# szpiech/garlic

Hardware: NVIDIA B200
Metric: individual_windows_per_sec (higher is better)
Workload: dtype f64

## Files before the change

garlic_b200/csrc/bound.cuh:

```cuda
#pragma once
#include "common.cuh"
#include "walk.cuh"

namespace garlic {

constexpr int kBoundShift = 8;
constexpr int kBoundStoreShift = 2;
constexpr int kPiece = 256;
constexpr int kBoundMinW = 16;
constexpr int kBoundPartialW = 32;
constexpr int kBoundMaxC2 = 13;
constexpr int kBoundGeomMaxW = 209;
constexpr int kPlanSegMax = 16;

GHD int bound_geom_w(int W) { return W > kBoundGeomMaxW ? kBoundGeomMaxW : W; }
GHD int bound_c2(int W) { return (bound_geom_w(W) + 14) >> 4; }
GHD int bound_c1(int W) { const int c = (bound_geom_w(W) - 16) >> 4; return c > 0 ? c : 0; }
GHD int bound_lag(int W) { return bound_c2(W) - bound_c1(W); }
GHD bool bound_partial(int W) { return W < kBoundPartialW; }
GHD uint32_t bound_low_mask(int W) { const int r = (bound_geom_w(W) - 16) & 15; return r ? ((1u << (2 * r)) - 1u) & 0x55555555u : 0u; }

GHD uint4 bound_hw_entry(const double* lut, long long q, long long L, int* invalid)
{
    const double scale = (double)(1 << kBoundShift);
    double D[16], dmax = 0.0, chet = -1e300;
    uint32_t mo = 0u;
    for (int i = 0; i < 16; ++i) {
        const long long s = q * 16 + i;
        const double* e = lut + s * 4;
        const double base = e[0] < e[2] ? e[0] : e[2];
        D[i] = fabs(e[0] - e[2]);
        if (!(D[i] >= 0.0) || D[i] > 1e6) { D[i] = 0.0; if (s < L) *invalid = 1; }
        if (e[2] > e[0]) mo |= 1u << (2 * i);
        if (D[i] > dmax) dmax = D[i];
        if (s < L) {
            const double dh = e[1] - base;
            if (dh > chet) chet = dh;
            if (e[3] - base > 0.0) *invalid = 1;
            if (!(dh <= 0.0)) *invalid = 1;
        }
    }
    uint32_t step = dmax > 0.0 ? (uint32_t)ceil(dmax / 3.0 * scale) + 1u : 0u;
    if (step > 0xffffu) { step = 0xffffu; *invalid = 1; }
    uint32_t p0 = 0u, p1 = 0u;
    for (int i = 0; i < 16; ++i) {
        int lev = 0;
        if (D[i] > 0.0) {
            lev = (int)ceil(D[i] * scale / (double)step);
            if (lev < 1) lev = 1;
            if (lev > 3) lev = 3;
        }
        if (lev & 1) p0 |= 1u << (2 * i);
        if (lev & 2) p1 |= 1u << (2 * i);
    }
    uint32_t ch = 0u;
    if (chet > -1e299 && chet < 0.0) { const double m = floor(-chet * scale); ch = m > 65535.0 ? 0xffffu : (uint32_t)m; }
    uint4 o;
    o.x = mo | (p0 << 1); o.y = p1; o.z = step | (ch << 16); o.w = 0u;
    return o;
}

GHD int bound_block_max(const double* lut, long long k, int W)
{
    const int Wg = bound_geom_w(W);
    const long long s0 = k * 16;
    double b = 0.0;
    for (int i = 0; i < Wg; ++i) { const double* e = lut + (s0 + i) * 4; b += e[0] < e[2] ? e[0] : e[2]; }
    for (int i = Wg; i < W; ++i) { const double* e = lut + (s0 + i) * 4; b += e[0] < e[2] ? e[2] : e[0]; }
    double bmax = b;
    for (int j = 1; j < 16; ++j) {
        const double* eo = lut + (s0 + j - 1) * 4;
        const double* ei = lut + (s0 + j - 1 + W) * 4;
        b -= (eo[0] < eo[2] ? eo[0] : eo[2]);
        if (W > Wg) {
            const double* em = lut + (s0 + j - 1 + Wg) * 4;
            b -= (em[0] < em[2] ? em[2] : em[0]);
            b += (em[0] < em[2] ? em[0] : em[2]);
            b += (ei[0] < ei[2] ? ei[2] : ei[0]);
        } else {
            b += (ei[0] < ei[2] ? ei[0] : ei[2]);
        }
        if (b > bmax) bmax = b;
    }
    const double v = ceil(bmax * (double)(1 << kBoundShift)) + 2.0;
    return v > 1.0e9 ? 1000000000 : (v < -1.0e9 ? -1000000000 : (int)v);
}

struct BoundState {
    uint32_t PH[16], PR[16];
    uint32_t ph, pr;
    uint32_t top1, top2, low1;
    int pm_all, pm_tail;
};

GHD void bound_reset(BoundState& S)
{
#ifdef __CUDA_ARCH__
#pragma unroll
#endif
    for (int i = 0; i < 16; ++i) { S.PH[i] = 0u; S.PR[i] = 0u; }
    S.ph = 0u; S.pr = 0u;
    S.top1 = 0u; S.top2 = 0u; S.low1 = 0u;
    S.pm_all = -0x40000000; S.pm_tail = -0x40000000;
}

template <int C2, int LAG, bool PARTIAL = false>
GHD void bound_step(BoundState& S, uint32_t h, const uint4& t, const int I, const uint32_t low_mask = 0u)
{
    const uint32_t M = 0x55555555u;
    const uint32_t s = h >> 1;
    const uint32_t het = h & ~s & M;
    const uint32_t x = ~h & ~(s ^ t.x);
    const int n0 = popc32(x & (t.x >> 1) & M), n1 = popc32(x & t.y), nh = popc32(het);
    S.pr += (uint32_t)(n0 + 2 * n1) * (t.z & 0xffffu);
    S.PR[I] = S.pr;
    int ub;
    if (!PARTIAL) {
        S.ph += (uint32_t)nh * (t.z >> 16);
        S.PH[I] = S.ph;
        ub = (int)t.w + (int)(S.pr - S.PR[(I - C2 - 1) & 15]) + (int)(S.PH[(I - C2) & 15] - S.PH[(I - LAG) & 15]);
    } else {
        const uint32_t ch = t.z >> 16;
        const uint32_t top = ((het >> 30) & 1u) * ch, low = (uint32_t)popc32(het & low_mask) * ch;
        S.PH[I] = S.ph + (uint32_t)nh * ch - top;
        S.ph += (uint32_t)nh * ch;
        const uint32_t top_lag = LAG == 1 ? S.top1 : S.top2;
        const uint32_t low_next = LAG == 1 ? low : S.low1;
        const uint32_t core = (S.PH[(I - LAG) & 15] + top_lag) - S.PH[(I - C2) & 15] + low_next;
        ub = (int)t.w + (int)(S.pr - S.PR[(I - C2 - 1) & 15]) - (int)core;
        S.top2 = S.top1; S.top1 = top; S.low1 = low;
    }
    S.pm_all = ub > S.pm_all ? ub : S.pm_all;
    if (((I - C2) & 15) >= 16 - C2) S.pm_tail = ub > S.pm_tail ? ub : S.pm_tail;
}

GHD uint32_t bound_pack(int pm_all, int pm_tail)
{
    int a = (pm_all + (1 << kBoundStoreShift) - 1) >> kBoundStoreShift, b = (pm_tail + (1 << kBoundStoreShift) - 1) >> kBoundStoreShift;
    a = a > 32767 ? 32767 : (a < -32768 ? -32768 : a);
    b = b > 32767 ? 32767 : (b < -32768 ? -32768 : b);
    return ((uint32_t)a & 0xffffu) | ((uint32_t)b << 16);
}

GHD int bound_cut_store(double cutoff, double tol, int* ok)
{
    const double c = floor((cutoff - tol) * (double)(1 << kBoundShift)) - 2.0;
    *ok = (c > -8.0e6 && c < 8.0e6);
    if (!*ok) return 0;
    const int s = (int)c >> kBoundStoreShift;
    if (s > 32000 || s < -32000) *ok = 0;
    return s;
}

GHD bool bound_item_candidate(const uint32_t* pmax, int64_t stride, int ind, const Item& it, int cut_store, int c2)
{
    const int p_own = it.own_lo >> 8, p_hi = (it.own_hi - 1) >> 8, p_w0 = it.w0 >> 8;
    bool c = false;
    for (int p = (p_w0 < p_own ? p_w0 + 1 : p_own); p <= p_hi; ++p) c |= (int)(int16_t)(pmax[(int64_t)p * stride + ind] & 0xffffu) >= cut_store;
    if (p_w0 < p_own) {
        const uint32_t v = pmax[(int64_t)p_w0 * stride + ind];
        const bool tail_covers = it.w0 >= 256 * (p_w0 + 1) - 16 * c2;
        c |= (int)(int16_t)(tail_covers ? (v >> 16) : (v & 0xffffu)) >= cut_store;
    }
    return c;
}

GHD void plan_half(const int* src, long long L, long long q, uint4* head, uint4* segs)
{
    const long long d0 = q * 16;
    int n = 0;
    if (d0 < L) { const long long r = L - d0; n = r < 16 ? (int)r : 16; }
    uint4 hd;
    hd.w = n < 16 ? (0xffffffffu << (2 * n)) : 0u;
    hd.z = 0u;
    if (n == 16) {
        const int d = src[d0 + 15] - src[d0] - 15;
        if (d >= 0 && d <= 3) {
            uint32_t z = (uint32_t)(2 * (src[d0] & 15));
            int k = 0;
            for (int i = 0; i < 15; ++i)
                for (int g = src[d0 + i + 1] - src[d0 + i] - 1; g > 0; --g) z |= (uint32_t)(i + 1) << (8 * ++k);
            hd.x = 0x100u | ((uint32_t)d << 4); hd.y = (uint32_t)(src[d0] >> 4); hd.z = z;
            hd.w = d ? ((1u << (2u * ((z >> 8) & 255u))) - 1u) : 0xffffffffu;
            *head = hd;
            return;
        }
    }
    int ns = 0, i = 0, last = -1;
    while (i < n) {
        const int s0 = src[d0 + i];
        int len = 1;
        while (i + len < n && src[d0 + i + len] == s0 + len && ((s0 + len) >> 4) == (s0 >> 4)) ++len;
        uint4 sg;
        sg.x = (uint32_t)(s0 >> 4); sg.y = (uint32_t)(2 * (s0 & 15));
        sg.z = len >= 16 ? 0xffffffffu : ((1u << (2 * len)) - 1u);
        sg.w = (uint32_t)(2 * i);
        segs[ns++] = sg;
        last = s0 >> 4;
        i += len;
    }
    hd.x = (uint32_t)ns; hd.y = (uint32_t)last;
    *head = hd;
}

GHD uint32_t plan_fast_code(const uint4& hd, int a_base, int I)
{
    if (!(hd.x & 0x100u) || ((hd.x >> 4) & 15u) > 1u) return 0xffffu;
    const int rel = 32 * ((int)hd.y - a_base - I) + (int)(hd.z & 255u);
    if (rel < 0 || rel >= 96) return 0xffffu;
    const uint32_t p = ((hd.x >> 4) & 15u) ? ((hd.z >> 8) & 255u) : 16u;
    return (uint32_t)(rel >> 5) | ((uint32_t)(rel & 31) << 2) | ((2u * p) << 8);
}
GHD uint32_t plan_fast_apply(uint32_t code, uint32_t r0, uint32_t r1, uint32_t r2, uint32_t r3, uint32_t r4)
{
    const uint32_t k = code & 3u, sh = (code >> 2) & 31u, p2 = (code >> 8) & 255u;
    const uint32_t x0 = k == 0u ? r0 : (k == 1u ? r1 : r2), x1 = k == 0u ? r1 : (k == 1u ? r2 : r3), x2 = k == 0u ? r2 : (k == 1u ? r3 : r4);
    const uint32_t lo = sh ? ((x0 >> sh) | (x1 << (32u - sh))) : x0, hi = sh ? ((x1 >> sh) | (x2 << (32u - sh))) : x1;
    const uint32_t m = p2 >= 32u ? 0xffffffffu : ((1u << p2) - 1u);
    return (lo & m) | (((lo >> 2) | (hi << 30)) & ~m);
}
GHD bool plan_need1(const uint4& hd) { return ((hd.z & 255u) != 0u) || ((hd.x >> 4) & 15u); }
GHD bool plan_need2(const uint4& hd) { return ((hd.z & 255u) >> 1) + 15u + ((hd.x >> 4) & 15u) >= 32u; }
GHD uint32_t plan_window(const uint4& hd, uint32_t x0, uint32_t x1, uint32_t x2)
{
    const uint32_t sh = hd.z & 255u;
    uint32_t lo = sh ? ((x0 >> sh) | (x1 << (32u - sh))) : x0;
    uint32_t d = (hd.x >> 4) & 15u;
    if (d) {
        uint32_t hi = sh ? ((x1 >> sh) | (x2 << (32u - sh))) : x1;
        uint32_t z = hd.z >> 8;
        for (; d; --d, z >>= 8) {
            const uint32_t m = (1u << (2u * (z & 255u))) - 1u;
            const uint32_t slo = (lo >> 2) | (hi << 30);
            hi >>= 2;
            lo = (lo & m) | (slo & ~m);
        }
    }
    return lo;
}

}
```

garlic_b200/csrc/capi.cu:

```cuda
#include <cuda_runtime.h>
#include <nccl.h>
#include <algorithm>
#include <chrono>
#include <cmath>
#include <cstdio>
#include <cstring>
#include <map>
#include <unistd.h>
#include <string>
#include <vector>

#include "../../include/garlic_b200.h"
#include "common.cuh"
#include "kernels.h"
#include "wlod.h"
#include "segments.h"
#include "bound.cuh"

using namespace garlic;

namespace {
constexpr int kPad = 4096 + 64;
constexpr int kMaxW = 4096;
constexpr unsigned kBreakCap = 1u << 20, kBreakFirst = 4096;

}

struct garlic_gpu {
    int device = 0;
    cudaStream_t stream = nullptr;
    std::string err;
    uint64_t launches = 0;
    int n_ind = 0, ind_offset = 0, n_chr = 0;
    int64_t L0 = 0, L = 0;
    std::vector<int64_t> chr_off0, chr_off;
    std::vector<int32_t> pos0, pos, src, cen;
    std::vector<double> gpos;
    std::vector<Stretch> stretches;
    bool stretches_pending = false;
    uint8_t* brk_pin = nullptr;
    cudaEvent_t ev_tables = nullptr;
    bool have_geno0 = false, filtered = false, tables = false, have_gl = false, have_ld = false;
    int gl_type = GARLIC_GL_ERROR;
    double error = -1, mu = 1e-9;
    int max_gap = 200000, M = 7, ld_W = 0;
    double amax = 0;
    double fmin = 0.5;
    int* d_corr = nullptr;
    int missing_char = '0';
    uint8_t* d_alleles = nullptr;
    unsigned long long* d_key = nullptr;
    uint64_t *d_geno0 = nullptr, *d_geno = nullptr;
    int64_t row_words0 = 0, row_words = 0;
    int* d_counts = nullptr;
    double *d_gl0 = nullptr, *d_gl = nullptr;
    int64_t gl_stride = 0;
    double *d_freq0 = nullptr, *d_freq = nullptr, *d_lut = nullptr, *d_gpos = nullptr;
    double *d_nomut = nullptr, *d_norec = nullptr, *d_wlut = nullptr, *d_invld = nullptr, *d_homf = nullptr;
    char* d_text = nullptr;
    long long* d_textoff = nullptr;
    int* d_nonblank = nullptr;
    int2* d_hard = nullptr;
    StitchScratch stitch_scratch;
    std::vector<RohRec> recs_buf, ambs_buf, merged_buf, tmp_buf;
    uint64_t* d_ldplanes = nullptr;
    double* d_ldpairs = nullptr;
    uint8_t* d_keep = nullptr;
    int *d_src = nullptr, *d_pos0 = nullptr, *d_chr_of0 = nullptr, *d_pos = nullptr, *d_chr_of = nullptr,
        *d_chr_start = nullptr, *d_chr_param = nullptr;
    RohRec *d_out = nullptr, *d_amb = nullptr, *d_sorted = nullptr;
    unsigned* d_hist = nullptr;
    unsigned* d_kept = nullptr;
    size_t last_final = 0;
    std::vector<Segment> p2_segs;
    std::vector<Item> p2_items;
    Item* d_items_p2 = nullptr;
    int p2_W = 0, p2_tile = 0, p2_chunk = 0;
    uint64_t tables_gen = 0, p2_gen = 0;
    size_t sorted_cap = 0;
    unsigned out_cap = 0, amb_cap = 0;
    unsigned* d_cnt = nullptr;
    Item* d_items = nullptr;
    double* d_dump = nullptr;
    size_t items_cap = 0;
    int* d_indlist = nullptr;
    size_t indlist_cap = 0;
    double stats[8] = {0, 0, 0, 0, 0, 0, 0, 0};
    int64_t stats_items = 0;
    int* d_scan = nullptr;
    int* d_breaks = nullptr;
    uint32_t* d_badbits = nullptr;
    int* d_thin = nullptr;
    bool geno_pending = false;
    uint4 *d_plan_head = nullptr, *d_plan_seg = nullptr;
    int2* d_plan_rng = nullptr;
    uint4* d_bhw = nullptr;
    uint16_t* d_plan_fast = nullptr;
    int* d_bflag = nullptr;
    int bound_tables_W = 0;
    uint32_t* d_pmax = nullptr;
    int64_t pmax_stride = 0;
    int n_pieces = 0, bound_W = 0;
    int* d_cand_list = nullptr;
    unsigned* d_cand_cnt = nullptr;
    int2* d_units = nullptr;
    unsigned* d_nunits = nullptr;
    size_t zero_cap = 0, zero_n = 0;
    cudaEvent_t ev_sq0 = nullptr, ev_sq1 = nullptr;
    bool sq_timed = false;
    int item_pieces = 1;
    bool prune = true;
    bool precounted = false;
    bool phased = false;
    bool wlod_mma = true;
    ncclComm_t comm = nullptr;
    int comm_rank = 0, comm_world = 1;
    bool counts_reduced = false, counts_hi_reduced = false;
    bool counts_nccl_mem = false;
    uint8_t* xslab = nullptr;
    void* xpeer[kXchgMaxRanks] = {nullptr};
    size_t x_off_counts = 0, x_off_freq = 0, x_off_keep = 0;
    bool xchg_tried = false, xchg_ok = false;
    unsigned xchg_seq = 0;
    ncclWindow_t counts_win = nullptr;
    bool counts_win_tried = false;
    double* d_gather = nullptr;
    const double* kde_src = nullptr;
    int64_t kde_src_n = 0;
    double *d_kde = nullptr, *d_kde_in = nullptr;
    cudaEvent_t ev2 = nullptr;
    cudaStream_t copy_stream = nullptr;
    cudaStream_t aux_stream = nullptr;
    cudaEvent_t ev_aux_in = nullptr, ev_aux_out = nullptr;
    cudaEvent_t ev_copy = nullptr;
    bool tl_on = false;
    std::vector<cudaEvent_t> tl_ev;
    std::vector<const char*> tl_name;
    std::vector<double> tl_host;
    bool out_pending = false;
    uint8_t* pin = nullptr;
    size_t pin_cap = 0;
    std::map<void*, size_t> cap;
    cudaEvent_t ev0 = nullptr, ev1 = nullptr;
};

struct Laps {
    bool on;
    int rank = 0;
    const char* name;
    std::chrono::steady_clock::time_point t0;
    std::string out;
    explicit Laps(const char* n) : on(getenv("GARLIC_TIMING") != nullptr), name(n), t0(std::chrono::steady_clock::now()) {}
    void lap(const char* what)
    {
        if (!on) return;
        const auto t1 = std::chrono::steady_clock::now();
        char b[96];
        snprintf(b, sizeof b, " %s=%.3f", what, std::chrono::duration<double, std::milli>(t1 - t0).count());
        out += b;
        t0 = t1;
    }
    ~Laps() { if (on) fprintf(stderr, "[garlic_b200 r%d] %s:%s ms\n", rank, name, out.c_str()); }
};

static void tl_mark(garlic_gpu* h, const char* name)
{
    if (!h->tl_on) return;
    if (h->tl_ev.size() >= 4096) return;
    cudaEvent_t e;
    cudaEventCreate(&e);
    cudaEventRecord(e, h->stream);
    h->tl_ev.push_back(e);
    h->tl_name.push_back(name);
    h->tl_host.push_back(std::chrono::duration<double, std::milli>(std::chrono::steady_clock::now().time_since_epoch()).count());
}
static void tl_dump(garlic_gpu* h)
{
    if (!h->tl_on || h->tl_ev.empty()) return;
    cudaStreamSynchronize(h->stream);
    const size_t n = h->tl_ev.size(), first = n > 120 ? n - 120 : 0;
    for (size_t i = first; i < n; ++i) {
        float g = 0;
        cudaEventElapsedTime(&g, h->tl_ev[first], h->tl_ev[i]);
        fprintf(stderr, "[timeline r%d] %-28s host %9.3f  stream %9.3f ms\n", h->comm_rank, h->tl_name[i], h->tl_host[i] - h->tl_host[first], g);
    }
    for (cudaEvent_t e : h->tl_ev) cudaEventDestroy(e);
    h->tl_ev.clear();
}

#define CK(call)                                                                              \
    do {                                                                                      \
        cudaError_t e_ = (call);                                                              \
        if (e_ != cudaSuccess) {                                                              \
            h->err = std::string(#call) + ": " + cudaGetErrorString(e_);                      \
            return 1;                                                                         \
        }                                                                                     \
    } while (0)
#define LAUNCH(call) do { CK(call); h->launches++; } while (0)
#define FAIL(msg) do { h->err = (msg); return 1; } while (0)

template <typename T>
static int dev_alloc(garlic_gpu* h, T** p, size_t n)
{
    if (n == 0) n = 1;
    const size_t bytes = n * sizeof(T);
    auto it = h->cap.find((void*)p);
    if (*p && it != h->cap.end() && it->second >= bytes) return 0;
    if (*p) { cudaFree(*p); *p = nullptr; }
    CK(cudaMalloc((void**)p, bytes));
    h->cap[(void*)p] = bytes;
    return 0;
}
template <typename T>
static void dev_free(T*& p) { if (p) cudaFree(p); p = nullptr; }

static int pin_alloc(garlic_gpu* h, size_t bytes)
{
    if (h->pin && h->pin_cap >= bytes) return 0;
    if (h->pin) { cudaFreeHost(h->pin); h->pin = nullptr; h->pin_cap = 0; }
    CK(cudaMallocHost((void**)&h->pin, bytes));
    h->pin_cap = bytes;
    return 0;
}

static double lod_bound(const garlic_gpu* h)
{
    const double n_total = 2.0 * ((double)h->n_ind + 1.0) * (double)std::max(1, h->comm_world);
    double fmin = 1.0 / n_total;
    if (h->fmin > 0 && h->fmin < fmin) fmin = h->fmin;
    const double emin = h->have_gl ? 1e-16 : ((h->error > 0 && h->error < 1) ? h->error : 1e-16);
    return std::max(-std::log10(emin), -std::log10(fmin)) + 1.0;
}

#define NCK(call)                                                                             \
    do {                                                                                      \
        ncclResult_t r_ = (call);                                                             \
        if (r_ != ncclSuccess) {                                                              \
            h->err = std::string(#call) + ": " + ncclGetErrorString(r_);                      \
            return 1;                                                                         \
        }                                                                                     \
    } while (0)

static int reduce_counts(garlic_gpu* h, bool hi)
{
    if (!h->comm) return 0;
    if (!h->counts_win_tried && h->counts_nccl_mem) {
        h->counts_win_tried = true;
        if (getenv("GARLIC_NCCL_WINDOW") != nullptr) {
            if (ncclCommWindowRegister(h->comm, h->d_counts, (size_t)4 * h->L0 * sizeof(int), &h->counts_win, NCCL_WIN_COLL_SYMMETRIC) != ncclSuccess)
                h->counts_win = nullptr;
        }
    }
    if (!h->counts_reduced) {
        NCK(ncclAllReduce(h->d_counts, h->d_counts, (size_t)2 * h->L0, ncclInt32, ncclSum, h->comm, h->stream));
        h->counts_reduced = true;
    }
    if (hi && !h->counts_hi_reduced) {
        NCK(ncclAllReduce(h->d_counts + 2 * h->L0, h->d_counts + 2 * h->L0, (size_t)2 * h->L0, ncclInt32, ncclSum, h->comm, h->stream));
        h->counts_hi_reduced = true;
    }
    return 0;
}

static void free_counts(garlic_gpu* h)
{
    if (!h->d_counts) return;
    if (h->xchg_ok) return;
    if (h->counts_win && h->comm) ncclCommWindowDeregister(h->comm, h->counts_win);
    h->counts_win = nullptr; h->counts_win_tried = false;
    if (h->counts_nccl_mem) ncclMemFree(h->d_counts); else cudaFree(h->d_counts);
    h->d_counts = nullptr; h->counts_nccl_mem = false;
    h->cap.erase((void*)&h->d_counts);
}

static int alloc_counts(garlic_gpu* h, size_t n)
{
    const size_t bytes = n * sizeof(int);
    auto it = h->cap.find((void*)&h->d_counts);
    if (h->d_counts && it != h->cap.end() && it->second == bytes) return 0;
    free_counts(h);
    void* p = nullptr;
    if (getenv("GARLIC_NCCL_WINDOW") != nullptr && ncclMemAlloc(&p, bytes) == ncclSuccess && p) {
        h->d_counts = static_cast<int*>(p);
        h->counts_nccl_mem = true;
    } else {
        cudaGetLastError();
        CK(cudaMalloc((void**)&h->d_counts, bytes));
    }
    h->cap[(void*)&h->d_counts] = bytes;
    return 0;
}

static void xchg_teardown(garlic_gpu* h)
{
    if (!h->xslab) { h->xchg_tried = false; h->xchg_ok = false; return; }
    cudaStreamSynchronize(h->stream);
    for (int p = 0; p < kXchgMaxRanks; ++p) {
        if (h->xpeer[p] && h->xpeer[p] != (void*)h->xslab) cudaIpcCloseMemHandle(h->xpeer[p]);
        h->xpeer[p] = nullptr;
    }
    if (h->xchg_ok) {
        h->d_counts = nullptr; h->d_freq0 = nullptr; h->d_keep = nullptr;
        h->cap.erase((void*)&h->d_counts); h->cap.erase((void*)&h->d_freq0); h->cap.erase((void*)&h->d_keep);
    }
    cudaFree(h->xslab);
    h->xslab = nullptr;
    h->xchg_tried = false; h->xchg_ok = false; h->xchg_seq = 0;
}

static int ensure_xchg(garlic_gpu* h)
{
    if (h->xchg_tried) return 0;
    h->xchg_tried = true;
    h->xchg_ok = false;
    if (!h->comm || h->comm_world < 2 || h->comm_world > kXchgMaxRanks || h->counts_nccl_mem) return 0;
    if (getenv("GARLIC_NO_XCHG") != nullptr) return 0;
    const int N = h->comm_world;
    const size_t L0 = (size_t)h->L0;
    h->x_off_counts = 256;
    h->x_off_freq = (h->x_off_counts + 16 * L0 + 255) & ~(size_t)255;
    h->x_off_keep = h->x_off_freq + 8 * L0;
    const size_t total = ((h->x_off_keep + L0 + 255) & ~(size_t)255);
    struct Rec { cudaIpcMemHandle_t hdl; int pid; int ok; long long L0; char pad[128 - sizeof(cudaIpcMemHandle_t) - 16]; };
    static_assert(sizeof(Rec) == 128, "exchange record is 128 bytes");
    Rec mine;
    memset(&mine, 0, sizeof(mine));
    mine.pid = (int)getpid(); mine.L0 = h->L0; mine.ok = 1;
    if (cudaMalloc((void**)&h->xslab, total) != cudaSuccess) { cudaGetLastError(); h->xslab = nullptr; mine.ok = 0; }
    if (mine.ok) {
        cudaMemsetAsync(h->xslab, 0, 256, h->stream);
        cudaStreamSynchronize(h->stream);
        if (cudaIpcGetMemHandle(&mine.hdl, h->xslab) != cudaSuccess) { cudaGetLastError(); mine.ok = 0; }
    }
    Rec* d_rec = nullptr;
    std::vector<Rec> all(N);
    CK(cudaMalloc((void**)&d_rec, (size_t)(N + 1) * sizeof(Rec)));
    CK(cudaMemcpyAsync(d_rec + N, &mine, sizeof(Rec), cudaMemcpyHostToDevice, h->stream));
    NCK(ncclAllGather(d_rec + N, d_rec, sizeof(Rec), ncclUint8, h->comm, h->stream));
    CK(cudaMemcpyAsync(all.data(), d_rec, (size_t)N * sizeof(Rec), cudaMemcpyDeviceToHost, h->stream));
    CK(cudaStreamSynchronize(h->stream));
    int ok = 1;
    for (int p = 0; p < N; ++p) {
        if (!all[p].ok || all[p].L0 != h->L0) ok = 0;
        if (p != h->comm_rank && all[p].pid == mine.pid) ok = 0;
    }
    for (int p = 0; p < N && ok; ++p) {
        if (p == h->comm_rank) { h->xpeer[p] = h->xslab; continue; }
        void* ptr = nullptr;
        if (cudaIpcOpenMemHandle(&ptr, all[p].hdl, cudaIpcMemLazyEnablePeerAccess) != cudaSuccess) { cudaGetLastError(); ok = 0; break; }
        h->xpeer[p] = ptr;
    }
    int* d_ok = reinterpret_cast<int*>(d_rec);
    CK(cudaMemcpyAsync(d_ok, &ok, sizeof(int), cudaMemcpyHostToDevice, h->stream));
    NCK(ncclAllReduce(d_ok, d_ok, 1, ncclInt32, ncclMin, h->comm, h->stream));
    CK(cudaMemcpyAsync(&ok, d_ok, sizeof(int), cudaMemcpyDeviceToHost, h->stream));
    CK(cudaStreamSynchronize(h->stream));
    cudaFree(d_rec);
    if (!ok) {
        for (int p = 0; p < N; ++p) {
            if (h->xpeer[p] && h->xpeer[p] != (void*)h->xslab) cudaIpcCloseMemHandle(h->xpeer[p]);
            h->xpeer[p] = nullptr;
        }
        if (h->xslab) cudaFree(h->xslab);
        h->xslab = nullptr;
        return 0;
    }
    int* nc = reinterpret_cast<int*>(h->xslab + h->x_off_counts);
    if (h->d_counts) CK(cudaMemcpyAsync(nc, h->d_counts, 16 * L0, cudaMemcpyDeviceToDevice, h->stream));
    else CK(cudaMemsetAsync(nc, 0, 16 * L0, h->stream));
    CK(cudaStreamSynchronize(h->stream));
    free_counts(h);
    if (h->d_freq0) { cudaFree(h->d_freq0); h->d_freq0 = nullptr; }
    if (h->d_keep) { cudaFree(h->d_keep); h->d_keep = nullptr; }
    h->d_counts = nc;
    h->d_freq0 = reinterpret_cast<double*>(h->xslab + h->x_off_freq);
    h->d_keep = h->xslab + h->x_off_keep;
    h->cap[(void*)&h->d_counts] = 16 * L0;
    h->cap[(void*)&h->d_freq0] = 8 * L0;
    h->cap[(void*)&h->d_keep] = L0;
    h->xchg_ok = true;
// ... 236 lines not shown
    if (h->comm) NCK(ncclAllReduce(h->d_key, h->d_key, (size_t)h->L0, ncclUint64, ncclMin, h->comm, h->stream));
    CK(cudaMemsetAsync(h->d_counts, 0, (size_t)4 * h->L0 * sizeof(int), h->stream));
    const int64_t chunk = 1 << 20;
    for (int64_t s0 = 0; s0 < h->L0; s0 += chunk) {
        const int n = (int)std::min<int64_t>(chunk, h->L0 - s0);
        LAUNCH(launch_code_alleles(h->d_alleles + (size_t)s0 * h->n_ind * 2, n, h->n_ind, missing, h->d_key + s0, s0,
                                   h->d_geno0, h->row_words0, h->d_counts, h->L0, h->stream));
    }
    CK(cudaStreamSynchronize(h->stream));
    h->have_geno0 = true;
    return 0;
}

static int put_packed_common(garlic_gpu* h, const void* rows, int64_t stride, cudaMemcpyKind kind)
{
    CK(cudaSetDevice(h->device));
    if (!h->L0) FAIL("put_packed: call set_shape first");
    const int64_t need = (h->L0 + 3) / 4;
    if (stride < need) FAIL("put_packed: row stride smaller than ceil(n_loci/4)");
    h->precounted = false;
    if (kind == cudaMemcpyHostToDevice && h->n_ind >= 256 && h->d_counts) {
        const int n_slices = 8;
        const int per = ((h->n_ind + n_slices - 1) / n_slices + 15) / 16 * 16;
        CK(cudaMemsetAsync(h->d_counts, 0, (size_t)4 * h->L0 * sizeof(int), h->stream));
        CK(cudaEventRecord(h->ev_copy, h->stream));
        CK(cudaStreamWaitEvent(h->copy_stream, h->ev_copy, 0));
        for (int r0 = 0; r0 < h->n_ind; r0 += per) {
            const int n = std::min(per, h->n_ind - r0);
            uint64_t* dst = h->d_geno0 + (size_t)r0 * h->row_words0;
            CK(cudaMemcpy2DAsync(dst, (size_t)h->row_words0 * 8, (const char*)rows + (size_t)r0 * stride, (size_t)stride, (size_t)need,
                                 (size_t)n, kind, h->copy_stream));
            CK(cudaEventRecord(h->ev_copy, h->copy_stream));
            CK(cudaStreamWaitEvent(h->stream, h->ev_copy, 0));
            LAUNCH(launch_count_packed(dst, h->row_words0, n, h->L0, h->d_counts, h->stream));
        }
        CK(cudaStreamSynchronize(h->copy_stream));
        h->precounted = true;
        h->counts_reduced = false; h->counts_hi_reduced = false;
        h->have_geno0 = true;
        return 0;
    }
    CK(cudaMemcpy2DAsync(h->d_geno0, (size_t)h->row_words0 * 8, rows, (size_t)stride, (size_t)need, (size_t)h->n_ind, kind, h->stream));
    CK(cudaStreamSynchronize(h->stream));
    h->have_geno0 = true;
    return 0;
}

int garlic_gpu_put_packed(garlic_gpu_t* h, const uint8_t* rows, int64_t row_stride_bytes)
{
    return put_packed_common(h, rows, row_stride_bytes, cudaMemcpyHostToDevice);
}
int garlic_gpu_put_packed_dev(garlic_gpu_t* h, const void* rows_dev, int64_t row_stride_bytes)
{
    return put_packed_common(h, rows_dev, row_stride_bytes, cudaMemcpyDeviceToDevice);
}

__global__ void add_corr_kernel(int* counts, long long L0, const int* na, const int* tot)
{
    for (long long s = blockIdx.x * (long long)blockDim.x + threadIdx.x; s < L0; s += (long long)gridDim.x * blockDim.x) {
        if (na) counts[s] += na[s];
        if (tot) counts[L0 + s] += tot[s];
    }
}

int garlic_gpu_count_packed(garlic_gpu_t* h, const int32_t* nalleles_corr, const int32_t* total_corr)
{
    CK(cudaSetDevice(h->device));
    if (!h->have_geno0) FAIL("count_packed: no genotypes loaded");
    tl_mark(h, "count_packed:in");
    h->counts_reduced = false; h->counts_hi_reduced = false;
    if (h->precounted) {
        h->precounted = false;
    } else {
        CK(cudaMemsetAsync(h->d_counts, 0, (size_t)4 * h->L0 * sizeof(int), h->stream));
        LAUNCH(launch_count_packed(h->d_geno0, h->row_words0, h->n_ind, h->L0, h->d_counts, h->stream));
    }
    if (nalleles_corr || total_corr) {
        if (dev_alloc(h, &h->d_corr, (size_t)2 * h->L0)) return 1;
        int *d_a = nalleles_corr ? h->d_corr : nullptr, *d_t = total_corr ? h->d_corr + h->L0 : nullptr;
        if (d_a) CK(cudaMemcpyAsync(d_a, nalleles_corr, h->L0 * sizeof(int), cudaMemcpyHostToDevice, h->stream));
        if (d_t) CK(cudaMemcpyAsync(d_t, total_corr, h->L0 * sizeof(int), cudaMemcpyHostToDevice, h->stream));
        add_corr_kernel<<<(unsigned)std::min<int64_t>((h->L0 + 255) / 256, 148 * 16), 256, 0, h->stream>>>(h->d_counts, h->L0, d_a, d_t);
        CK(cudaGetLastError());
        h->launches++;
        CK(cudaStreamSynchronize(h->stream));
    }
    if (h->xchg_ok) return 0;
    return reduce_counts(h, false);
}

void* garlic_gpu_counts_dev(garlic_gpu_t* h) { return h ? (void*)h->d_counts : nullptr; }

int garlic_gpu_get_counts(garlic_gpu_t* h, int32_t* na, int32_t* tot, int32_t* hom, int32_t* nm)
{
    CK(cudaSetDevice(h->device));
    CK(cudaStreamSynchronize(h->stream));
    int32_t* dst[4] = {na, tot, hom, nm};
    for (int c = 0; c < 4; ++c)
        if (dst[c]) CK(cudaMemcpy(dst[c], h->d_counts + (size_t)c * h->L0, h->L0 * sizeof(int), cudaMemcpyDeviceToHost));
    return 0;
}

int garlic_gpu_get_one_allele(garlic_gpu_t* h, uint8_t* allele, char missing)
{
    CK(cudaSetDevice(h->device));
    if (!h->d_key) FAIL("get_one_allele: alleles were not ingested on this handle");
    std::vector<unsigned long long> k(h->L0);
    CK(cudaStreamSynchronize(h->stream));
    CK(cudaMemcpy(k.data(), h->d_key, h->L0 * sizeof(unsigned long long), cudaMemcpyDeviceToHost));
    for (int64_t s = 0; s < h->L0; ++s) allele[s] = (k[s] == ~0ull) ? (uint8_t)missing : (uint8_t)(k[s] & 0xff);
    return 0;
}

static int put_gl_common(garlic_gpu* h, const void* v, int gl_type, cudaMemcpyKind kind)
{
    CK(cudaSetDevice(h->device));
    if (!h->L0) FAIL("put_gl: call set_shape first");
    if (gl_type < -1 || gl_type > 2) FAIL("put_gl: bad gl_type");
    if (dev_alloc(h, &h->d_gl0, (size_t)h->n_ind * h->L0)) return 1;
    CK(cudaMemcpyAsync(h->d_gl0, v, (size_t)h->n_ind * h->L0 * sizeof(double), kind, h->stream));
    CK(cudaStreamSynchronize(h->stream));
    h->gl_type = gl_type;
    h->have_gl = true;
    return 0;
}
int garlic_gpu_put_tgls_text(garlic_gpu_t* h, const char* text, const int64_t* line_off, int64_t snp0, int n_snp,
                             int gl_type, int32_t* n_tokens)
{
    CK(cudaSetDevice(h->device));
    if (!h->L0) FAIL("put_tgls_text: call set_shape first");
    if (gl_type < -1 || gl_type > 2) FAIL("put_tgls_text: bad gl_type");
    if (snp0 < 0 || n_snp < 0 || snp0 + n_snp > h->L0) FAIL("put_tgls_text: bad SNP range");
    if (n_snp == 0) return 0;
    const int64_t bytes = line_off[n_snp] - line_off[0];
    if (bytes < 0) FAIL("put_tgls_text: line offsets must ascend");
    if (dev_alloc(h, &h->d_gl0, (size_t)h->n_ind * h->L0)) return 1;
    if (dev_alloc(h, &h->d_text, (size_t)bytes + 16)) return 1;
    if (dev_alloc(h, &h->d_textoff, (size_t)n_snp + 1)) return 1;
    if (dev_alloc(h, &h->d_nonblank, (size_t)n_snp)) return 1;
    const unsigned hard_cap = 1u << 16;
    if (dev_alloc(h, &h->d_hard, (size_t)hard_cap + 1)) return 1;
    unsigned* d_hard_n = reinterpret_cast<unsigned*>(h->d_hard + hard_cap);
    std::vector<long long> rel(n_snp + 1);
    for (int i = 0; i <= n_snp; ++i) rel[i] = (long long)(line_off[i] - line_off[0]);
    const char* base = text + line_off[0];
    CK(cudaMemcpyAsync(h->d_text, base, (size_t)bytes, cudaMemcpyHostToDevice, h->stream));
    CK(cudaMemcpyAsync(h->d_textoff, rel.data(), rel.size() * sizeof(long long), cudaMemcpyHostToDevice, h->stream));
    CK(cudaMemsetAsync(d_hard_n, 0, sizeof(unsigned), h->stream));
    LAUNCH(launch_tokenize_tgls(h->d_text, h->d_textoff, n_snp, h->n_ind, h->ind_offset, h->d_gl0, h->L0, snp0, h->d_nonblank,
                                h->d_hard, d_hard_n, hard_cap, h->stream));
    std::vector<int32_t> ntok_local;
    if (!n_tokens) { ntok_local.resize(n_snp); n_tokens = ntok_local.data(); }
    unsigned n_hard = 0;
    CK(cudaMemcpyAsync(n_tokens, h->d_nonblank, (size_t)n_snp * sizeof(int), cudaMemcpyDeviceToHost, h->stream));
    CK(cudaMemcpyAsync(&n_hard, d_hard_n, sizeof(unsigned), cudaMemcpyDeviceToHost, h->stream));
    CK(cudaStreamSynchronize(h->stream));
    if (n_hard) {
        auto token_at = [&](int l, int k) -> const char* {
            const char* p = base + rel[l];
            const char* e = base + rel[l + 1];
            for (int t = 0;; ++t) {
                while (p < e && (*p == ' ' || *p == '\t' || *p == '\r' || *p == '\n')) ++p;
                if (p >= e) return nullptr;
                if (t == k) return p;
                while (p < e && !(*p == ' ' || *p == '\t' || *p == '\r' || *p == '\n')) ++p;
            }
        };
        auto convert = [&](const char* p, int l) -> double {
            const char* e = base + rel[l + 1];
            const char* q = p;
            while (q < e && !(*q == ' ' || *q == '\t' || *q == '\r' || *q == '\n')) ++q;
            const std::string tok(p, q);
            return strtod(tok.c_str(), nullptr);
        };
        std::vector<int2> list;
        if (n_hard <= hard_cap) {
            list.resize(n_hard);
            CK(cudaMemcpy(list.data(), h->d_hard, n_hard * sizeof(int2), cudaMemcpyDeviceToHost));
        } else {
            for (int l = 0; l < n_snp; ++l)
                for (int k = h->ind_offset; k < h->ind_offset + h->n_ind; ++k) list.push_back(make_int2(l, k));
        }
        std::sort(list.begin(), list.end(), [](const int2& a, const int2& b) { return a.x != b.x ? a.x < b.x : a.y < b.y; });
        for (const int2& t : list) {
            const char* p = token_at(t.x, t.y);
            if (!p) continue;
            const double v = convert(p, t.x);
            CK(cudaMemcpyAsync(h->d_gl0 + (size_t)(t.y - h->ind_offset) * h->L0 + snp0 + t.x, &v, sizeof(double), cudaMemcpyHostToDevice, h->stream));
            CK(cudaStreamSynchronize(h->stream));
        }
    }
    h->gl_type = gl_type;
    h->have_gl = true;
    return 0;
}

int garlic_gpu_get_gl(garlic_gpu_t* h, double* values)
{
    CK(cudaSetDevice(h->device));
    if (!h->have_gl || !h->d_gl0) FAIL("get_gl: no likelihoods loaded");
    CK(cudaStreamSynchronize(h->stream));
    CK(cudaMemcpy(values, h->d_gl0, (size_t)h->n_ind * h->L0 * sizeof(double), cudaMemcpyDeviceToHost));
    return 0;
}

int garlic_gpu_put_gl(garlic_gpu_t* h, const double* values, int gl_type) { return put_gl_common(h, values, gl_type, cudaMemcpyHostToDevice); }
int garlic_gpu_put_gl_dev(garlic_gpu_t* h, const void* values_dev, int gl_type) { return put_gl_common(h, values_dev, gl_type, cudaMemcpyDeviceToDevice); }

int garlic_gpu_filter(garlic_gpu_t* h, int oob, const int32_t* chr_param, const double* freq_override,
                      double* freq_out, uint8_t* keep_out, int64_t* n_kept)
{
    CK(cudaSetDevice(h->device));
    if (!h->have_geno0) FAIL("filter: no genotypes loaded");
    if (oob && !chr_param) FAIL("filter: oob filtering needs chr_param");
    const int64_t L0 = h->L0;
    Laps laps("filter");
    laps.rank = h->comm_rank;
    if (finish_outputs(h)) return 1;
    tl_mark(h, "filter:in");
    if (!freq_override) h->fmin = 0.5;
    bool freq_direct = false, keep_direct = false, copies_in_flight = false;
    if (dev_alloc(h, &h->d_freq0, (size_t)L0)) return 1;
    if (dev_alloc(h, &h->d_keep, (size_t)L0)) return 1;
    if (oob) {
        if (dev_alloc(h, &h->d_chr_param, (size_t)4 * h->n_chr)) return 1;
        CK(cudaMemcpyAsync(h->d_chr_param, chr_param, 4 * h->n_chr * sizeof(int), cudaMemcpyHostToDevice, h->stream));
    }
    const int n_blocks = (int)((L0 + 1023) / 1024);
    const size_t off_keep = (size_t)L0 * 8, off_meta = (off_keep + (size_t)L0 + 63) & ~(size_t)63;
    if (pin_alloc(h, off_meta + (size_t)(h->n_chr + 2) * 4 + 64)) return 1;
    double* freq0 = reinterpret_cast<double*>(h->pin);
    uint8_t* keep = h->pin + off_keep;
    int32_t* meta = reinterpret_cast<int32_t*>(h->pin + off_meta);
    if (freq_override) {
        h->fmin = 0.5;
        for (int64_t s = 0; s < L0; ++s) {
            const double f = freq_override[s];
            bool k = (f > 0 && f < 1);
            if (k) h->fmin = std::min(h->fmin, std::min(f, 1.0 - f));
            if (oob) {
                int c = (int)(std::upper_bound(h->chr_off0.begin(), h->chr_off0.end(), s) - h->chr_off0.begin()) - 1;
                const int32_t* cp = chr_param + 4 * c;
                const int p = h->pos0[s];
                k = k && !(p < cp[0]) && !(p > cp[1]) && !(p > cp[2] && p < cp[3]);
            }
            freq0[s] = f; keep[s] = k;
        }
        CK(cudaMemcpyAsync(h->d_freq0, freq0, L0 * sizeof(double), cudaMemcpyHostToDevice, h->stream));
        CK(cudaMemcpyAsync(h->d_keep, keep, L0, cudaMemcpyHostToDevice, h->stream));
    } else {
        if (h->comm && !h->xchg_tried && ensure_xchg(h)) return 1;
        if (h->xchg_ok && !h->counts_reduced) {
            XchgParams X;
            memset(&X, 0, sizeof(X));
            for (int p = 0; p < h->comm_world; ++p) {
                uint8_t* base = static_cast<uint8_t*>(h->xpeer[p]);
                X.flags[p] = reinterpret_cast<unsigned*>(base);
                X.counts[p] = reinterpret_cast<int*>(base + h->x_off_counts);
                X.freq[p] = reinterpret_cast<double*>(base + h->x_off_freq);
                X.keep[p] = base + h->x_off_keep;
            }
            X.n = h->comm_world; X.rank = h->comm_rank; X.seq = ++h->xchg_seq; X.L0 = L0;
            X.pos = h->d_pos0; X.chr_of = h->d_chr_of0; X.chr_param = h->d_chr_param; X.oob = oob;
            X.done_counter = reinterpret_cast<unsigned*>(h->xslab) + 48;
            LAUNCH(launch_xchg_freq_keep(X, h->stream));
            h->counts_reduced = true;
        } else {
            if (reduce_counts(h, false)) return 1;
            LAUNCH(launch_freq_keep(h->d_counts, L0, h->d_pos0, h->d_chr_of0, h->d_chr_param, oob, h->d_freq0, h->d_keep, h->stream));
        }
        freq_direct = freq_out && is_pinned(freq_out);
        keep_direct = keep_out && is_pinned(keep_out);
        copies_in_flight = freq_out || keep_out;
    }
    if (dev_alloc(h, &h->d_src, (size_t)L0)) return 1;
    if (dev_alloc(h, &h->d_scan, (size_t)n_blocks + h->n_chr + 8)) return 1;
    int* d_total = h->d_scan + n_blocks;
    int* d_chr_off_kept = d_total + 1;
    CK(launch_keep_scan(h->d_keep, L0, h->d_chr_of0, h->n_chr, h->d_scan, d_total, h->d_src, d_chr_off_kept, h->stream));
    h->launches += 3;
    CK(cudaMemcpyAsync(meta, d_total, (size_t)(h->n_chr + 2) * sizeof(int), cudaMemcpyDeviceToHost, h->stream));
    if (copies_in_flight) {
        CK(cudaEventRecord(h->ev_copy, h->stream));
        CK(cudaStreamWaitEvent(h->copy_stream, h->ev_copy, 0));
        if (freq_out) CK(cudaMemcpyAsync(freq_direct ? freq_out : freq0, h->d_freq0, L0 * sizeof(double), cudaMemcpyDeviceToHost, h->copy_stream));
        if (keep_out) CK(cudaMemcpyAsync(keep_direct ? keep_out : keep, h->d_keep, L0, cudaMemcpyDeviceToHost, h->copy_stream));
    }
    CK(cudaStreamSynchronize(h->stream));
    laps.lap("freq_keep+scan");
    tl_mark(h, "filter:after-sync");
    if (freq_override) {
        if (freq_out) memcpy(freq_out, freq0, L0 * sizeof(double));
        if (keep_out) memcpy(keep_out, keep, L0);
    }
    const int64_t L = meta[0];
    h->chr_off.assign(h->n_chr + 1, 0);
    for (int c = 0; c <= h->n_chr; ++c) h->chr_off[c] = meta[1 + c];
    h->src.clear();
    h->pos.clear();
    h->L = L;
    if (n_kept) *n_kept = L;
    if (L < 1) FAIL("filter: no polymorphic loci left");
    h->row_words = (((L + kPad + 31) >> 5) + 3) & ~(int64_t)1;
    const bool fresh = h->cap.find((void*)&h->d_geno) == h->cap.end() || !h->d_geno ||
                       h->cap[(void*)&h->d_geno] < (size_t)h->n_ind * h->row_words * 8;
    if (dev_alloc(h, &h->d_geno, (size_t)h->n_ind * h->row_words)) return 1;
    if (fresh) CK(cudaMemsetAsync(h->d_geno, 0xff, (size_t)h->n_ind * h->row_words * 8, h->stream));
    h->n_pieces = (int)((L + kPiece - 1) / kPiece);
    {
        const long long n_q = 16ll * (h->n_pieces + 4);
        if (dev_alloc(h, &h->d_plan_head, (size_t)n_q)) return 1;
        if (dev_alloc(h, &h->d_plan_seg, (size_t)n_q * kPlanSegMax)) return 1;
        if (dev_alloc(h, &h->d_plan_rng, (size_t)h->n_pieces + 4)) return 1;
        if (dev_alloc(h, &h->d_plan_fast, (size_t)n_q)) return 1;
        LAUNCH(launch_plan(h->d_src, d_total, n_q, h->d_plan_head, h->d_plan_seg, h->d_plan_fast, h->d_plan_rng, h->stream));
    }
    h->geno_pending = true; h->bound_W = 0; h->bound_tables_W = 0;
    if (dev_alloc(h, &h->d_freq, (size_t)L + kPad)) return 1;
    CK(cudaMemsetAsync(h->d_freq, 0, (size_t)(L + kPad) * sizeof(double), h->stream));
    LAUNCH(launch_gather_f64(h->d_freq0, h->d_src, L, h->d_freq, h->stream));
    if (h->have_gl) {
        h->gl_stride = L + kPad;
        if (dev_alloc(h, &h->d_gl, (size_t)((h->n_ind + 31) / 32) * 32 * h->gl_stride)) return 1;
        LAUNCH(launch_compact_gl(h->d_gl0, L0, h->d_src, L, h->d_geno0, h->row_words0, h->d_freq0, h->d_gl, h->gl_stride, h->n_ind,
                                 h->gl_type, h->stream));
    }
    std::vector<int> chr_start(h->n_chr);
    for (int c = 0; c < h->n_chr; ++c) chr_start[c] = (int)h->chr_off[c];
    if (dev_alloc(h, &h->d_pos, (size_t)L)) return 1;
    if (dev_alloc(h, &h->d_chr_of, (size_t)L)) return 1;
    if (dev_alloc(h, &h->d_chr_start, (size_t)h->n_chr)) return 1;
    LAUNCH(launch_gather_i32(h->d_pos0, h->d_src, L, h->d_pos, h->stream));
    LAUNCH(launch_gather_i32(h->d_chr_of0, h->d_src, L, h->d_chr_of, h->stream));
    CK(cudaMemcpyAsync(h->d_chr_start, chr_start.data(), h->n_chr * sizeof(int), cudaMemcpyHostToDevice, h->stream));
    laps.lap("enqueue");
    if (copies_in_flight) {
        const bool all_direct = (!freq_out || freq_direct) && (!keep_out || keep_direct);
        if (all_direct) {
            h->out_pending = true;
        } else {
            CK(cudaStreamSynchronize(h->copy_stream));
            if (freq_out && !freq_direct) memcpy(freq_out, freq0, L0 * sizeof(double));
            if (keep_out && !keep_direct) memcpy(keep_out, keep, L0);
        }
        laps.lap("freq/keep d2h");
    }
    h->filtered = true; h->tables = false; h->have_ld = false;
    tl_mark(h, "filter:out");
    return 0;
}

int64_t garlic_gpu_n_kept(const garlic_gpu_t* h) { return h ? h->L : 0; }

int garlic_gpu_get_genotypes(garlic_gpu_t* h, int filtered, uint8_t* rows, int64_t row_stride_bytes)
{
    CK(cudaSetDevice(h->device));
    if (filtered ? !h->filtered : !h->have_geno0) FAIL("get_genotypes: nothing loaded");
    const int64_t n = filtered ? h->L : h->L0;
    const int64_t need = (n + 3) / 4;
    if (row_stride_bytes < need) FAIL("get_genotypes: row stride too small");
    if (filtered && ensure_geno(h, 0)) return 1;
    CK(cudaStreamSynchronize(h->stream));
    CK(cudaMemcpy2D(rows, (size_t)row_stride_bytes, filtered ? h->d_geno : h->d_geno0,
                    (size_t)(filtered ? h->row_words : h->row_words0) * 8, (size_t)need, (size_t)h->n_ind, cudaMemcpyDeviceToHost));
    return 0;
}

int garlic_gpu_get_kept_index(garlic_gpu_t* h, int32_t* src_index)
{
    if (!h->filtered) FAIL("get_kept_index: call filter first");
    if (fetch_src(h)) return 1;
    memcpy(src_index, h->src.data(), h->L * sizeof(int32_t));
    return 0;
}

int garlic_gpu_set_tables(garlic_gpu_t* h, double error, int max_gap, const int32_t* centromeres, const double* gpos)
{
    CK(cudaSetDevice(h->device));
    if (!h->filtered) FAIL("set_tables: call filter first");
    h->error = error; h->max_gap = max_gap;
    Laps laps("set_tables");
    laps.rank = h->comm_rank;
    tl_mark(h, "set_tables:in");
    h->cen.assign(2 * h->n_chr, 0);
    if (centromeres) h->cen.assign(centromeres, centromeres + 2 * h->n_chr);
    const int64_t L = h->L;
    if (dev_alloc(h, &h->d_lut, (size_t)(L + kPad) * 4)) return 1;
    CK(cudaMemsetAsync(h->d_lut, 0, (size_t)(L + kPad) * 4 * sizeof(double), h->stream));
    LAUNCH(launch_build_lut(h->d_freq, L, error, h->d_lut, h->stream));
    h->gpos.clear();
    if (gpos) {
        h->gpos.assign(gpos, gpos + L);
        if (dev_alloc(h, &h->d_gpos, (size_t)L)) return 1;
        CK(cudaMemcpyAsync(h->d_gpos, gpos, L * sizeof(double), cudaMemcpyHostToDevice, h->stream));
    }
    h->amax = lod_bound(h);
    {
        if (dev_alloc(h, &h->d_breaks, (size_t)kBreakCap + 2 * h->n_chr + 4)) return 1;
        int* d_cen = h->d_breaks + kBreakCap;
        unsigned* d_n = reinterpret_cast<unsigned*>(d_cen + 2 * h->n_chr);
        CK(cudaMemcpyAsync(d_cen, h->cen.data(), 2 * h->n_chr * sizeof(int), cudaMemcpyHostToDevice, h->stream));
        CK(cudaMemsetAsync(d_n, 0, sizeof(unsigned), h->stream));
        if (dev_alloc(h, &h->d_badbits, (size_t)((L + 31) >> 5) + 4)) return 1;
        LAUNCH(launch_bad_pairs(h->d_pos, h->d_chr_of, d_cen, max_gap, L, h->d_breaks, d_n, kBreakCap, h->d_badbits, h->stream));
        if (!h->brk_pin) CK(cudaMallocHost((void**)&h->brk_pin, 64 + kBreakFirst * sizeof(int)));
        CK(cudaMemcpyAsync(h->brk_pin, d_n, sizeof(unsigned), cudaMemcpyDeviceToHost, h->stream));
        CK(cudaMemcpyAsync(h->brk_pin + 64, h->d_breaks, kBreakFirst * sizeof(int), cudaMemcpyDeviceToHost, h->stream));
        CK(cudaEventRecord(h->ev_tables, h->stream));
        h->stretches_pending = true;
        h->stretches.clear();
    }
    laps.lap("enqueue");
    tl_mark(h, "set_tables:out");
    h->tables = true; h->have_ld = false; h->bound_W = 0; h->bound_tables_W = 0; h->tables_gen++;
    return 0;
}

int garlic_gpu_set_lut(garlic_gpu_t* h, const double* lut)
{
    CK(cudaSetDevice(h->device));
    if (!h->tables) FAIL("set_lut: call set_tables first");
    CK(cudaMemcpy(h->d_lut, lut, (size_t)h->L * 4 * sizeof(double), cudaMemcpyHostToDevice));
    double m = 0;
    for (int64_t i = 0; i < h->L * 4; ++i) { const double a = std::fabs(lut[i]); if (a > m && std::isfinite(a)) m = a; }
    h->amax = std::max(lod_bound(h), m + 1.0);
    dev_free(h->d_wlut);
    h->bound_W = 0; h->bound_tables_W = 0;
    return 0;
}

int garlic_gpu_get_lut(garlic_gpu_t* h, double* lut)
{
    CK(cudaSetDevice(h->device));
    if (!h->tables) FAIL("get_lut: call set_tables first");
    CK(cudaStreamSynchronize(h->stream));
    CK(cudaMemcpy(lut, h->d_lut, (size_t)h->L * 4 * sizeof(double), cudaMemcpyDeviceToHost));
    return 0;
}

int garlic_gpu_get_hom_freq(garlic_gpu_t* h, double* hom_freq)
{
    CK(cudaSetDevice(h->device));
    if (!h->filtered) FAIL("get_hom_freq: call filter first");
    std::vector<int> hom(h->L0), nm(h->L0);
    if (reduce_counts(h, true)) return 1;
    if (garlic_gpu_get_counts(h, nullptr, nullptr, hom.data(), nm.data())) return 1;
    if (fetch_src(h)) return 1;
    for (int64_t d = 0; d < h->L; ++d) {
        double total = nm[h->src[d]], fh = hom[h->src[d]];
        fh /= total;
        hom_freq[d] = fh;
    }
    return 0;
}

int garlic_gpu_set_prune(garlic_gpu_t* h, int on)
{
    h->prune = on != 0;
    return 0;
}

int garlic_gpu_set_phased(garlic_gpu_t* h, int phased)
{
    h->phased = phased != 0;
    h->have_ld = false;
    return 0;
}

int garlic_gpu_set_wlod(garlic_gpu_t* h, double mu, int M)
{
    h->mu = mu; h->M = M;
    dev_free(h->d_wlut);
    return 0;
}

}

static int ensure_stretches(garlic_gpu* h)
{
    if (!h->stretches_pending) return 0;
    CK(cudaEventSynchronize(h->ev_tables));
    const unsigned nb = *reinterpret_cast<const unsigned*>(h->brk_pin);
    const int* first_host = reinterpret_cast<const int*>(h->brk_pin + 64);
    if (nb > kBreakCap) FAIL("set_tables: more than 2^20 gaps; raise --max-gap");
    std::vector<int> breaks(first_host, first_host + std::min(nb, kBreakFirst));
    if (nb > kBreakFirst) {
        breaks.resize(nb);
        CK(cudaStreamSynchronize(h->stream));
        CK(cudaMemcpy(breaks.data() + kBreakFirst, h->d_breaks + kBreakFirst, (nb - kBreakFirst) * sizeof(int), cudaMemcpyDeviceToHost));
    }
    std::sort(breaks.begin(), breaks.end());
    h->stretches.clear();
    size_t bi = 0;
    for (int c = 0; c < h->n_chr; ++c) {
        int a = (int)h->chr_off[c];
        const int hi = (int)h->chr_off[c + 1];
        while (bi < breaks.size() && breaks[bi] < hi) {
            if (breaks[bi] > a) h->stretches.push_back({c, a, breaks[bi]});
            a = breaks[bi++];
        }
        if (hi > a) h->stretches.push_back({c, a, hi});
    }
    h->stretches_pending = false;
    return 0;
}

static int ensure_zero_block(garlic_gpu* h)
{
    const size_t n = 8 + 2 * ((size_t)h->n_ind + 1);
    if (h->zero_cap < n) {
        if (h->d_cnt) cudaFree(h->d_cnt);
        h->d_cnt = nullptr;
        CK(cudaMalloc((void**)&h->d_cnt, n * sizeof(unsigned)));
        CK(cudaMemsetAsync(h->d_cnt, 0, n * sizeof(unsigned), h->stream));
        h->zero_cap = n;
    }
    h->d_nunits = h->d_cnt + 4;
    h->d_hist = h->d_cnt + 8;
    h->d_kept = h->d_hist + h->n_ind + 1;
    h->zero_n = n;
    return 0;
}

static int upload_items(garlic_gpu* h, const std::vector<Item>& items)
{
    if (items.size() > h->items_cap) {
        if (dev_alloc(h, &h->d_items, items.size() + 1024)) return 1;
        h->items_cap = items.size() + 1024;
    }
    if (!items.empty()) CK(cudaMemcpyAsync(h->d_items, items.data(), items.size() * sizeof(Item), cudaMemcpyHostToDevice, h->stream));
    return 0;
}

static int upload_indlist(garlic_gpu* h, const int32_t* list, int n, cudaStream_t st = nullptr)
{
    if (!st) st = h->stream;
    if ((size_t)n > h->indlist_cap) {
        if (dev_alloc(h, &h->d_indlist, (size_t)n + 1024)) return 1;
        h->indlist_cap = (size_t)n + 1024;
    }
    CK(cudaMemcpyAsync(h->d_indlist, list, n * sizeof(int), cudaMemcpyHostToDevice, st));
    return 0;
}

static WalkParams base_params(const garlic_gpu* h, int W)
{
    WalkParams P;
    memset(&P, 0, sizeof(P));
    P.geno = h->d_geno; P.row_words = h->row_words;
    P.lut = h->d_lut; P.gl = h->have_gl ? h->d_gl : nullptr; P.freq = h->d_freq; P.gl_stride = h->gl_stride;
    P.ind_list = nullptr; P.n_lanes = h->n_ind; P.W = W; P.thr = 1; P.cutoff = 0; P.tol = 0;
    P.out = h->d_out; P.out_count = h->d_cnt; P.out_cap = h->out_cap; P.amb = h->d_amb; P.amb_cap = h->amb_cap;
    P.hist = nullptr;
    P.dump = nullptr; P.dump_stride = 0; P.dump_step = 1;
    return P;
}

static int ensure_weighted(garlic_gpu* h, int W);
static int launch_any_walk(garlic_gpu* h, const WalkParams& P, const Item* items, int n_items, int weighted, bool roh, bool dump,
                           int tile_snps, const CandList& cl = CandList())
{
    if (weighted) {
        WlodParams Q;
        Q.base = P; Q.wlut = h->d_wlut; Q.invld = h->d_invld; Q.nomut = h->d_nomut; Q.norec = h->d_norec;
        if (P.tol > 0 && roh && !dump && h->wlod_mma && P.W >= kWlodMmaMinW) LAUNCH(launch_wlod_mma(Q, items, n_items, h->have_gl, h->stream));
        else LAUNCH(launch_wlod_walk(Q, items, n_items, h->have_gl, roh, dump, h->stream));
    } else {
        LAUNCH(launch_walk(P, items, n_items, h->have_gl, roh, dump, tile_snps <= kTileSnpsMax ? tile_snps : 0, cl, h->stream));
    }
    return 0;
}

static bool can_bound(const garlic_gpu* h, int W)
{
    return h->prune && h->tables && !h->have_gl && W >= kBoundMinW && W <= 1280;
}

static int ensure_bound_tables(garlic_gpu* h, int W)
{
    if (h->bound_tables_W == W) return 0;
    const long long n_hw = 16ll * (h->n_pieces + 4);
    if (dev_alloc(h, &h->d_bhw, (size_t)n_hw)) return 1;
    if (dev_alloc(h, &h->d_bflag, (size_t)4)) return 1;
    CK(cudaMemsetAsync(h->d_bflag, 0, 4 * sizeof(int), h->stream));
    LAUNCH(launch_bound_tables(h->d_lut, h->L + kPad, n_hw, h->L, W, h->d_bhw, h->d_bflag, h->stream));
    h->bound_tables_W = W;
    return 0;
}

static SqueezeParams squeeze_params(garlic_gpu* h, bool squeeze, int W)
{
    SqueezeParams Q;
    memset(&Q, 0, sizeof(Q));
    Q.gin = squeeze ? h->d_geno0 : h->d_geno;
    Q.in_words = squeeze ? h->row_words0 : h->row_words;
    Q.gout = h->d_geno; Q.out_words = h->row_words;
    Q.plan_head = h->d_plan_head; Q.plan_seg = h->d_plan_seg; Q.piece_rng = h->d_plan_rng;
    Q.plan_fast = reinterpret_cast<const uint32_t*>(h->d_plan_fast); Q.src = h->d_src; Q.n_kept = h->d_scan + (int)((h->L0 + 1023) / 1024);
    Q.n_ind = h->n_ind;
    Q.hw = h->d_bhw;
    Q.lag = bound_lag(W);
    Q.partial = (W > 0 && bound_partial(W)) ? 1 : 0;
    Q.low_mask = W > 0 ? bound_low_mask(W) : 0u;
    Q.pmax = h->d_pmax; Q.pmax_stride = h->pmax_stride;
    Q.n_pieces = h->n_pieces;
    return Q;
}

static int alloc_pmax(garlic_gpu* h)
{
    h->pmax_stride = ((int64_t)h->n_ind + 31) & ~(int64_t)31;
    return dev_alloc(h, &h->d_pmax, (size_t)h->n_pieces * h->pmax_stride);
}

static int ensure_geno(garlic_gpu* h, int W_hint)
{
    if (!h->geno_pending) return 0;
    int c2 = 0;
    if (W_hint > 0 && can_bound(h, W_hint)) {
        if (ensure_bound_tables(h, W_hint)) return 1;
        if (alloc_pmax(h)) return 1;
        c2 = bound_c2(W_hint);
    }
    const SqueezeParams Q = squeeze_params(h, true, W_hint);
    CK(cudaEventRecord(h->ev_sq0, h->stream));
    LAUNCH(launch_squeeze_bound(Q, true, c2, h->stream));
    CK(cudaEventRecord(h->ev_sq1, h->stream));
    h->sq_timed = true;
    h->geno_pending = false;
    if (c2) h->bound_W = W_hint;
    return 0;
}

static int prepare_p2_items(garlic_gpu* h, int W)
{
    if (h->p2_gen == h->tables_gen && h->p2_W == W) return 0;
    if (ensure_stretches(h)) return 1;
    segments_from_stretches(h->stretches, W, h->p2_segs);
    build_items_aligned(h->chr_off, W, h->p2_segs, kPiece * h->item_pieces, h->p2_items);
    h->p2_chunk = 0;
    for (const Item& it : h->p2_items) h->p2_chunk = std::max(h->p2_chunk, it.own_hi - it.own_lo);
    h->p2_tile = items_tile_snps(h->p2_items, W);
    if (dev_alloc(h, &h->d_items_p2, h->p2_items.size() + 1)) return 1;
    if (!h->p2_items.empty())
        CK(cudaMemcpyAsync(h->d_items_p2, h->p2_items.data(), h->p2_items.size() * sizeof(Item), cudaMemcpyHostToDevice, h->stream));
    h->p2_gen = h->tables_gen; h->p2_W = W;
    return 0;
}

static int ensure_bound(garlic_gpu* h, int W)
{
    if (ensure_geno(h, W)) return 1;
    if (h->bound_W == W) return 0;
    if (ensure_bound_tables(h, W)) return 1;
    if (alloc_pmax(h)) return 1;
    const SqueezeParams Q = squeeze_params(h, false, W);
    CK(cudaEventRecord(h->ev_sq0, h->stream));
    LAUNCH(launch_squeeze_bound(Q, false, bound_c2(W), h->stream));
    CK(cudaEventRecord(h->ev_sq1, h->stream));
    h->sq_timed = true;
    h->bound_W = W;
    return 0;
}

static bool side_pass1(const garlic_gpu* h, int weighted, int exact, int step)
{
    static const bool off = getenv("GARLIC_NO_SIDE_PASS1") != nullptr;
    return !off && !weighted && !exact && step >= 8 && !h->have_gl && h->have_geno0 && h->aux_stream != nullptr;
}
static int begin_side(garlic_gpu* h)
{
    CK(cudaEventRecord(h->ev_aux_in, h->stream));
    CK(cudaStreamWaitEvent(h->aux_stream, h->ev_aux_in, 0));
    return 0;
}
static int end_side(garlic_gpu* h)
{
    CK(cudaEventRecord(h->ev_aux_out, h->aux_stream));
    CK(cudaStreamWaitEvent(h->stream, h->ev_aux_out, 0));
    return 0;
}

extern "C" {

int64_t garlic_gpu_window_slots(garlic_gpu_t* h, int step)
{
    if (!h || !h->filtered || step < 1) return -1;
    int64_t n = 0;
    for (int c = 0; c < h->n_chr; ++c) n += (h->chr_off[c + 1] - h->chr_off[c] + step - 1) / step;
    return n;
}

static int windows_common(garlic_gpu_t* h, int winsize, int step, int weighted, const int32_t* individuals, int n,
                          int exact, double* out, void** out_dev);

int garlic_gpu_windows(garlic_gpu_t* h, int winsize, int step, int weighted, const int32_t* individuals, int n,
                       int exact, double* out)
{
    return windows_common(h, winsize, step, weighted, individuals, n, exact, out, nullptr);
}

int garlic_gpu_windows_dev(garlic_gpu_t* h, int winsize, int step, int weighted, const int32_t* individuals, int n,
                           int exact, void** out_dev)
{
    if (!out_dev) return 1;
    return windows_common(h, winsize, step, weighted, individuals, n, exact, nullptr, out_dev);
}

int garlic_gpu_windows_gather(garlic_gpu_t* h, int winsize, int step, int weighted, const int32_t* individuals, int n,
                              int rows_per_rank, int exact, double* out)
{
    if (n > rows_per_rank) FAIL("windows_gather: more individuals than rows_per_rank");
    const int64_t slots = garlic_gpu_window_slots(h, step);
    if (slots < 0) FAIL("windows_gather: call filter first");
    void* dptr = nullptr;
    if (n > 0 && windows_common(h, winsize, step, weighted, individuals, n, exact, nullptr, &dptr)) return 1;
    CK(cudaSetDevice(h->device));
    const bool side = h->filtered && h->tables && side_pass1(h, weighted, exact, step);
    cudaStream_t ws = side ? h->aux_stream : h->stream;
    if (side && n == 0 && begin_side(h)) return 1;
    const size_t blk = (size_t)rows_per_rank * slots;
    if (dev_alloc(h, &h->d_gather, blk * (h->comm_world + 1))) return 1;
    double* send = h->d_gather + blk * h->comm_world;
    LAUNCH(launch_fill_f64(send, blk, kMissing, ws));
    if (n > 0) CK(cudaMemcpyAsync(send, dptr, (size_t)n * slots * sizeof(double), cudaMemcpyDeviceToDevice, ws));
    if (h->comm) NCK(ncclAllGather(send, h->d_gather, blk, ncclDouble, h->comm, ws));
    else CK(cudaMemcpyAsync(h->d_gather, send, blk * sizeof(double), cudaMemcpyDeviceToDevice, ws));
    h->kde_src = h->d_gather; h->kde_src_n = (int64_t)(blk * h->comm_world);
    if (!out) return side ? end_side(h) : 0;
    const size_t bytes = blk * h->comm_world * sizeof(double);
    const bool direct = is_pinned(out);
    const bool staged = !direct && bytes <= ((size_t)64 << 20) && !pin_alloc(h, bytes);
    CK(cudaMemcpyAsync(direct ? (void*)out : (staged ? (void*)h->pin : (void*)out), h->d_gather, bytes, cudaMemcpyDeviceToHost, ws));
    CK(cudaStreamSynchronize(ws));
    if (side && end_side(h)) return 1;
    if (finish_outputs(h)) return 1;
    if (staged) memcpy(out, h->pin, bytes);
    return 0;
}

static int windows_common(garlic_gpu_t* h, int winsize, int step, int weighted, const int32_t* individuals, int n,
                          int exact, double* out, void** out_dev)
{
    CK(cudaSetDevice(h->device));
    if (!h->tables) FAIL("windows: call set_tables first");
    if (winsize < 2 || winsize > kMaxW) FAIL("windows: winsize out of range [2,4096]");
    if (step < 1) FAIL("windows: step must be >= 1");
    tl_mark(h, "windows:in");
    if (weighted && ensure_weighted(h, winsize)) return 1;
    const int W = winsize;
    const int n_lanes = individuals ? n : h->n_ind;
    if (individuals)
        for (int i = 0; i < n; ++i) if (individuals[i] < 0 || individuals[i] >= h->n_ind) FAIL("windows: individual index out of range");
    const int64_t slots = garlic_gpu_window_slots(h, step);
    const bool direct = !weighted && !exact && step >= 8;
    const bool side = direct && side_pass1(h, weighted, exact, step);
    cudaStream_t ws = h->stream;
    int rc = 0;
    double* d_dump = nullptr;
    if (direct) {
        if (!side && ensure_geno(h, winsize)) return 1;
        if (individuals && upload_indlist(h, individuals, n)) return 1;
        if (dev_alloc(h, &h->d_dump, (size_t)n_lanes * slots)) return 1;
        d_dump = h->d_dump;
        LAUNCH(launch_fill_f64(d_dump, (size_t)n_lanes * slots, kMissing, h->stream));
        std::vector<int2> meta(h->n_chr);
        int base = 0;
        for (int c = 0; c < h->n_chr; ++c) {
            meta[c].x = (int)h->chr_off[c]; meta[c].y = base;
            base += (int)((h->chr_off[c + 1] - h->chr_off[c] + step - 1) / step);
        }
        if (dev_alloc(h, &h->d_thin, (size_t)2 * h->n_chr + 8)) return 1;
        int2* d_meta = reinterpret_cast<int2*>(h->d_thin);
        CK(cudaMemcpyAsync(d_meta, meta.data(), meta.size() * sizeof(int2), cudaMemcpyHostToDevice, h->stream));
        LAUNCH(launch_thin_windows(side ? h->d_geno0 : h->d_geno, side ? h->row_words0 : h->row_words, h->d_lut,
                                   individuals ? h->d_indlist : nullptr, n_lanes, h->d_badbits, h->L, d_meta, h->n_chr, slots, step, W,
                                   d_dump, slots, h->have_gl ? h->d_gl : nullptr, h->gl_stride, side ? h->d_src : nullptr, h->stream));
        if (side) {
            if (begin_side(h)) return 1;
            ws = h->aux_stream;
            if (ensure_geno(h, winsize)) return 1;
        }
        tl_mark(h, "windows:squeeze-enqueued");
        if (h->bound_W == W && prepare_p2_items(h, W)) return 1;
    } else {
        if (ensure_geno(h, weighted ? 0 : winsize)) return 1;
        if (individuals && upload_indlist(h, individuals, n)) return 1;
        std::vector<Segment> segs;
        std::vector<Item> items;
        if (ensure_stretches(h)) return 1;
        segments_from_stretches(h->stretches, W, segs);
        if (dev_alloc(h, &h->d_dump, (size_t)n_lanes * slots)) return 1;
        d_dump = h->d_dump;
        LAUNCH(launch_fill_f64(d_dump, (size_t)n_lanes * slots, kMissing, h->stream));
        int chunk = 0;
        if (weighted) chunk = std::max(64, pick_chunk(h->L, W, n_lanes, 0) / 8);
        else if (!exact) chunk = pick_chunk(h->L, W, n_lanes, h->have_gl ? 0 : kTileSnpsMax);
        build_items(h->chr_off, W, segs, chunk, step, items);
        if (upload_items(h, items)) return 1;
        WalkParams P = base_params(h, W);
        P.ind_list = individuals ? h->d_indlist : nullptr;
        P.n_lanes = n_lanes;
        P.cutoff = 0; P.thr = 1; P.tol = 0;
        P.dump = d_dump; P.dump_stride = slots; P.dump_step = step;
        CK(cudaMemsetAsync(h->d_cnt, 0, 4 * sizeof(unsigned), h->stream));
        rc = launch_any_walk(h, P, h->d_items, (int)items.size(), weighted, false, true, items_tile_snps(items, W));
    }
    if (!rc) { h->kde_src = d_dump; h->kde_src_n = (int64_t)n_lanes * slots; }
    tl_mark(h, "windows:enqueued");
    if (!rc && finish_outputs(h)) rc = 1;
    if (!rc && out_dev) {
        *out_dev = d_dump;
        cudaError_t e = cudaStreamSynchronize(ws);
        if (e != cudaSuccess) { h->err = std::string("windows: ") + cudaGetErrorString(e); rc = 1; }
    } else if (!rc) {
        const size_t bytes = (size_t)n_lanes * slots * sizeof(double);
        const bool staged = !is_pinned(out) && bytes <= ((size_t)64 << 20) && !pin_alloc(h, bytes);
        cudaError_t e = cudaMemcpyAsync(staged ? (void*)h->pin : (void*)out, d_dump, bytes, cudaMemcpyDeviceToHost, ws);
        if (e == cudaSuccess) e = cudaStreamSynchronize(ws);
        if (e != cudaSuccess) { h->err = std::string("windows: ") + cudaGetErrorString(e); rc = 1; }
        else if (staged) memcpy(out, h->pin, bytes);
    }
    tl_mark(h, "windows:out");
    return rc;
}

int garlic_gpu_kde(garlic_gpu_t* h, const double* values, int64_t n_values, int m_targets, double* x, double* y,
                   int64_t* n_used, double* bandwidth)
{
    CK(cudaSetDevice(h->device));
    if (m_targets < 2 || m_targets > 1024) FAIL("kde: number of targets out of range [2,1024]");
    if (!x || !y) FAIL("kde: null output");
    const double* src = h->kde_src;
    int64_t n = h->kde_src_n;
    if (values) {
        if (n_values < 1) FAIL("kde: no values");
        if (dev_alloc(h, &h->d_kde_in, (size_t)n_values)) return 1;
        CK(cudaMemcpyAsync(h->d_kde_in, values, (size_t)n_values * sizeof(double), cudaMemcpyHostToDevice, h->stream));
        src = h->d_kde_in; n = n_values;
    }
    if (!src || n < 1) FAIL("kde: no window matrix on the device (call garlic_gpu_windows first, or pass values)");
    if (dev_alloc(h, &h->d_kde, kde_scratch_doubles(m_targets))) return 1;
    double* d_res = nullptr;
    int launches = 0;
    CK(launch_kde(src, (long long)n, m_targets, h->d_kde, &d_res, &launches, h->stream));
    h->launches += launches;
    const size_t bytes = (size_t)(8 + 2 * m_targets) * sizeof(double);
    if (pin_alloc(h, bytes)) return 1;
    CK(cudaMemcpyAsync(h->pin, d_res, bytes, cudaMemcpyDeviceToHost, h->stream));
    CK(cudaStreamSynchronize(h->stream));
    if (finish_outputs(h)) return 1;
    const double* r = reinterpret_cast<const double*>(h->pin);
    if (n_used) *n_used = (int64_t)r[0];
    if (bandwidth) *bandwidth = r[5];
    if (r[0] < 2) FAIL("kde: fewer than two valid window values");
    memcpy(x, r + 8, (size_t)m_targets * sizeof(double));
    memcpy(y, r + 8 + m_targets, (size_t)m_targets * sizeof(double));
    return 0;
}

int garlic_gpu_call_roh(garlic_gpu_t* h, int winsize, double cutoff, double overlap_frac, int weighted, int exact,
                        garlic_roh_t* out, int64_t cap, int64_t* count)
{
    CK(cudaSetDevice(h->device));
    if (!h->tables) FAIL("call_roh: call set_tables first");
    if (winsize < 2 || winsize > kMaxW) FAIL("call_roh: winsize out of range [2,4096]");
    if (!(cutoff > kMissing)) FAIL("call_roh: LOD cutoff must be greater than the MISSING sentinel (-9999)");
    if (weighted && ensure_weighted(h, winsize)) return 1;
    const int W = winsize;
    Laps laps("call_roh");
    laps.rank = h->comm_rank;
    tl_mark(h, "call_roh:in");
    int cut_ok = 0;
    bound_cut_store(cutoff, 1.0, &cut_ok);
    bool prune = !exact && !weighted && can_bound(h, W) && cut_ok;
    if (ensure_geno(h, prune ? W : 0)) return 1;
    double thr_d = overlap_frac * W;
    thr_d = (thr_d >= 1) ? thr_d : 1;
    thr_d = (thr_d <= W) ? thr_d : W;
    const int thr = (int)std::ceil(thr_d);

    std::vector<Segment> segs;
    std::vector<Item> items;
    if (ensure_stretches(h)) return 1;
    segments_from_stretches(h->stretches, W, segs);
    int chunk = 0;
    if (weighted) chunk = (!exact && h->wlod_mma && W >= kWlodMmaMinW) ? std::max(256, pick_chunk(h->L, W, h->n_ind, 0) / 2)
                                                                      : std::max(64, pick_chunk(h->L, W, h->n_ind, 0) / 8);
    else if (!exact) chunk = pick_chunk(h->L, W, h->n_ind, h->have_gl ? 0 : kTileSnpsMax);
    if (prune) {
        if (prepare_p2_items(h, W)) return 1;
        prune = h->p2_tile <= kTileSnpsMax && (int64_t)h->p2_items.size() * h->n_ind < (1ll << 31);
        if (prune) chunk = h->p2_chunk;
    }
    const Item* d_its = h->d_items;
    const std::vector<Item>* its = &items;
    if (prune) {
        d_its = h->d_items_p2; its = &h->p2_items;
    } else {
        build_items(h->chr_off, W, segs, chunk, 0, items);
        if (upload_items(h, items)) return 1;
        d_its = h->d_items;
    }
    int64_t n_win = 0;
    for (const Segment& s : segs) n_win += s.we - s.ws;
    int64_t units = 0;
    for (int c = 0; c < h->n_chr; ++c) units += std::max<int64_t>(0, h->chr_off[c + 1] - h->chr_off[c] - W + 1);
    units *= h->n_ind;

    if (!h->d_out) {
        h->out_cap = 1u << 22;
        if (dev_alloc(h, &h->d_out, h->out_cap)) return 1;
        h->amb_cap = 1u << 16;
        if (dev_alloc(h, &h->d_amb, h->amb_cap)) return 1;
    }
    laps.lap("items");
    std::vector<RohRec>&recs = h->recs_buf, &ambs = h->ambs_buf;
    recs.clear(); ambs.clear();
    size_t n_stage = 0;
    bool done = false;
    float ms = 0, ms_select = 0;
    bool pruned = false;
    double n_cand = -1.0;
    for (int attempt = 0; attempt < 3; ++attempt) {
        WalkParams P = base_params(h, W);
        P.cutoff = cutoff; P.thr = thr;
        if (!exact && !weighted) {
            int64_t longest = 0;
            for (const Segment& s : segs) longest = std::max<int64_t>(longest, s.we - s.ws);
            P.tol = (double)(longest + chunk + 3 * W) * 2.220446049250313e-16 * (W + 1) * h->amax;
        }
        if (!exact && weighted && h->wlod_mma && W >= kWlodMmaMinW) {
            P.tol = (double)(W + 8) * 2.0 * 2.220446049250313e-16 * W * h->amax;
        }
        if (ensure_zero_block(h)) return 1;
        CK(cudaMemsetAsync(h->d_cnt, 0, h->zero_n * sizeof(unsigned), h->stream));
        P.out_count = h->d_cnt;
        const int tile_snps = prune ? h->p2_tile : items_tile_snps(*its, W);
        const bool prune_now = prune && !exact;
        const int n_its = (int)its->size();
        CandList cl;
        unsigned unit_cap = 0;
        CK(cudaEventRecord(h->ev0, h->stream));
        if (prune_now) {
            if (ensure_bound(h, W)) return 1;
            int ok = 0;
            const int cut_store = bound_cut_store(cutoff, P.tol, &ok);
            const int per_item = (h->n_ind + kUnitThreads - 1) / kUnitThreads;
            unit_cap = (unsigned)std::min<int64_t>((int64_t)n_its * per_item, 1ll << 28);
            if (dev_alloc(h, &h->d_cand_list, (size_t)n_its * h->n_ind)) return 1;
            if (dev_alloc(h, &h->d_cand_cnt, (size_t)n_its + 1)) return 1;
            if (dev_alloc(h, &h->d_units, (size_t)unit_cap)) return 1;
            LAUNCH(launch_select(d_its, n_its, h->d_pmax, h->pmax_stride, h->n_ind, cut_store, h->d_bflag,
                                 h->d_cand_list, h->n_ind, h->d_cand_cnt, h->d_units, h->d_nunits, unit_cap, kUnitThreads, bound_c2(W), h->stream));
            cl.list = h->d_cand_list; cl.cnt = h->d_cand_cnt; cl.stride = h->n_ind;
        }
        CK(cudaEventRecord(h->ev2, h->stream));
        if (dev_alloc(h, &h->d_sorted, (size_t)h->out_cap)) return 1;
        P.hist = h->d_hist;
        if (prune_now && !bound_partial(W)) LAUNCH(launch_walk_units(P, d_its, h->d_units, h->d_nunits, unit_cap, tile_snps, cl, h->stream));
        else if (prune_now) LAUNCH(launch_walk(P, d_its, n_its, false, true, false, tile_snps, cl, h->stream));
        else if (launch_any_walk(h, P, d_its, n_its, weighted, true, false, tile_snps)) return 1;
        CK(cudaEventRecord(h->ev1, h->stream));
        LAUNCH(launch_bucket_by_individual(h->d_out, h->d_cnt, h->out_cap, h->d_hist, h->n_ind, h->d_sorted, thr, h->d_kept,
                                           h->d_cnt + 2, h->stream));
        const size_t guess = std::min<size_t>(h->out_cap, std::max<size_t>(4096, h->last_final + h->last_final / 4));
        const size_t amb_guess = 256;
        if (pin_alloc(h, 64 + (guess + std::max<size_t>(amb_guess, h->amb_cap)) * sizeof(RohRec))) return 1;
        unsigned* cnt = reinterpret_cast<unsigned*>(h->pin);
        RohRec* stage = reinterpret_cast<RohRec*>(h->pin + 64);
        CK(cudaMemcpyAsync(cnt, h->d_cnt, 4 * sizeof(unsigned), cudaMemcpyDeviceToHost, h->stream));
        cnt[4] = 0; cnt[5] = 0;
        if (prune_now) CK(cudaMemcpyAsync(cnt + 4, h->d_nunits, 2 * sizeof(unsigned), cudaMemcpyDeviceToHost, h->stream));
        CK(cudaMemcpyAsync(stage, h->d_out, guess * sizeof(RohRec), cudaMemcpyDeviceToHost, h->stream));
        CK(cudaMemcpyAsync(stage + guess, h->d_amb, amb_guess * sizeof(RohRec), cudaMemcpyDeviceToHost, h->stream));
        tl_mark(h, "call_roh:enqueued");
        CK(cudaStreamSynchronize(h->stream));
        if (finish_outputs(h)) return 1;
        tl_mark(h, "call_roh:synced");
        CK(cudaEventElapsedTime(&ms, h->ev0, h->ev1));
        CK(cudaEventElapsedTime(&ms_select, h->ev0, h->ev2));
        pruned = prune_now;
        n_cand = prune_now ? (double)cnt[5] : -1.0;
        const unsigned n_raw = cnt[0], n_amb = cnt[1], n_fin = cnt[2];
        if (n_raw > h->out_cap) {
            h->out_cap = n_raw + n_raw / 4 + 1024;
            if (dev_alloc(h, &h->d_out, h->out_cap)) return 1;
            continue;
        }
        if (n_amb > h->amb_cap) {
            exact = 1; prune = false;
            build_items(h->chr_off, W, segs, 0, 0, items);
            if (upload_items(h, items)) return 1;
            d_its = h->d_items; its = &items;
            continue;
        }
        recs.resize(n_fin);
        ambs.resize(n_amb);
        if (n_fin) memcpy(recs.data(), stage, std::min<size_t>(n_fin, guess) * sizeof(RohRec));
        if (n_fin > guess) CK(cudaMemcpy(recs.data() + guess, h->d_out + guess, (n_fin - guess) * sizeof(RohRec), cudaMemcpyDeviceToHost));
        if (n_amb) memcpy(ambs.data(), stage + guess, std::min<size_t>(n_amb, amb_guess) * sizeof(RohRec));
        if (n_amb > amb_guess) CK(cudaMemcpy(ambs.data() + amb_guess, h->d_amb + amb_guess, (n_amb - amb_guess) * sizeof(RohRec), cudaMemcpyDeviceToHost));
        n_stage = n_raw;
        h->last_final = n_fin;
        done = true;
        break;
    }
    if (!done) FAIL("call_roh: record buffers still overflowing after three attempts");
    laps.lap("kernel+d2h");
    int64_t n_amb_pairs = 0;
    if (!ambs.empty()) {
        std::map<int, std::vector<int>> by_seg;
        for (const RohRec& a : ambs) by_seg[a.tag].push_back(a.ind);
        std::vector<RohRec> fixed;
        for (auto& kv : by_seg) {
            std::vector<int>& inds = kv.second;
            std::sort(inds.begin(), inds.end());
            inds.erase(std::unique(inds.begin(), inds.end()), inds.end());
            n_amb_pairs += (int64_t)inds.size();
            std::vector<Segment> one(1, segs[kv.first]);
            std::vector<Item> its;
            build_items(h->chr_off, W, one, 0, 0, its);
            its[0].seg = kv.first;
            if (upload_items(h, its)) return 1;
            if (upload_indlist(h, inds.data(), (int)inds.size())) return 1;
            WalkParams P = base_params(h, W);
            P.cutoff = cutoff; P.thr = thr; P.tol = 0;
            P.ind_list = h->d_indlist; P.n_lanes = (int)inds.size();
            CK(cudaMemsetAsync(h->d_cnt, 0, 4 * sizeof(unsigned), h->stream));
            if (launch_any_walk(h, P, h->d_items, 1, weighted, true, false, items_tile_snps(its, W))) return 1;
            unsigned cnt[4];
            CK(cudaMemcpyAsync(cnt, h->d_cnt, sizeof(cnt), cudaMemcpyDeviceToHost, h->stream));
            CK(cudaStreamSynchronize(h->stream));
            if (cnt[0] > h->out_cap) FAIL("call_roh: ROH buffer overflow during exact re-evaluation");
            const size_t base = fixed.size();
            fixed.resize(base + cnt[0]);
            if (cnt[0]) CK(cudaMemcpy(fixed.data() + base, h->d_out, cnt[0] * sizeof(RohRec), cudaMemcpyDeviceToHost));
            recs.erase(std::remove_if(recs.begin(), recs.end(), [&](const RohRec& r) {
                return (r.tag >> 2) == kv.first && std::binary_search(inds.begin(), inds.end(), r.ind);
            }), recs.end());
        }
        recs.insert(recs.end(), fixed.begin(), fixed.end());
    }
    laps.lap("ambiguous");
    std::vector<RohRec>& merged = ambs.empty() ? recs : h->merged_buf;
    if (!ambs.empty()) stitch_runs(recs, thr, merged, &h->stitch_scratch);
    laps.lap("stitch");
    if (laps.on) fprintf(stderr, "[garlic_b200] call_roh: %zu raw records, %zu ambiguous pairs, %zu runs after stitching\n", n_stage, ambs.size(), merged.size());
    const int64_t n_out = (int64_t)merged.size();
    for (int64_t r = 0; r < n_out && r < cap && out; ++r) {
        out[r].ind = merged[r].ind;
        out[r].chr = segs[merged[r].tag >> 2].chr;
        out[r].start_idx = merged[r].a;
        out[r].stop_idx = merged[r].b;
    }
    if (count) *count = n_out;
    h->stats[0] = (double)its->size();
    h->stats[1] = (double)units;
    h->stats[2] = (double)n_amb_pairs;
    h->stats[3] = ms;
    h->stats[4] = ms_select;
    h->stats[5] = pruned ? n_cand : -1;
    h->stats[6] = (double)its->size() * h->n_ind;
    h->stats_items = 0;
    laps.lap("out");
    tl_mark(h, "call_roh:out");
    return 0;
}

int garlic_gpu_last_stats(garlic_gpu_t* h, double* s)
{
    if (h->stats_items > 0) {
        unsigned nu[2] = {0, 0};
        CK(cudaSetDevice(h->device));
        CK(cudaStreamSynchronize(h->stream));
        CK(cudaMemcpy(nu, h->d_nunits, sizeof(nu), cudaMemcpyDeviceToHost));
        h->stats[5] = (double)nu[1];
        h->stats_items = 0;
    }
    if (h->sq_timed) {
        float ms = 0;
        CK(cudaSetDevice(h->device));
        CK(cudaEventSynchronize(h->ev_sq1));
        CK(cudaEventElapsedTime(&ms, h->ev_sq0, h->ev_sq1));
        h->stats[7] = ms;
    }
    for (int i = 0; i < 8; ++i) s[i] = h->stats[i];
    return 0;
}

int garlic_gpu_get_piece_bounds(garlic_gpu_t* h, int winsize, uint32_t* out, int64_t cap_entries, int64_t* n_pieces)
{
    CK(cudaSetDevice(h->device));
    if (!h->tables) FAIL("get_piece_bounds: call set_tables first");
    if (!can_bound(h, winsize)) FAIL("get_piece_bounds: no bound for this mode / window size (unweighted table mode, winsize >= 16)");
    if (ensure_bound(h, winsize)) return 1;
    if (n_pieces) *n_pieces = h->n_pieces;
    if ((int64_t)h->n_pieces * h->n_ind > cap_entries) FAIL("get_piece_bounds: output buffer too small");
    CK(cudaStreamSynchronize(h->stream));
    CK(cudaMemcpy2D(out, (size_t)h->n_ind * 4, h->d_pmax, (size_t)h->pmax_stride * 4, (size_t)h->n_ind * 4, (size_t)h->n_pieces,
                    cudaMemcpyDeviceToHost));
    return 0;
}

int garlic_gpu_ld_band(garlic_gpu_t* h, int winsize, const int32_t* ld_individuals, int n_ld, double* out_ld)
{
    CK(cudaSetDevice(h->device));
    if (!h->tables) FAIL("ld_band: call set_tables first");
    if (winsize < 2 || winsize > kMaxW) FAIL("ld_band: winsize out of range [2,4096]");
    if (ensure_geno(h, 0)) return 1;
    const int64_t L = h->L;
    const int W = winsize;
    int n_total = h->n_ind;
    if (h->comm) {
        int* d_n = reinterpret_cast<int*>(h->d_cnt);
        CK(cudaMemcpyAsync(d_n, &h->n_ind, sizeof(int), cudaMemcpyHostToDevice, h->stream));
        NCK(ncclAllReduce(d_n, d_n, 1, ncclInt32, ncclSum, h->comm, h->stream));
        CK(cudaMemcpyAsync(&n_total, d_n, sizeof(int), cudaMemcpyDeviceToHost, h->stream));
        CK(cudaStreamSynchronize(h->stream));
    }
    std::vector<int> all;
    if (!ld_individuals) {
        all.resize(n_total);
        for (int i = 0; i < n_total; ++i) all[i] = i;
        ld_individuals = all.data(); n_ld = n_total;
    }
    for (int i = 0; i < n_ld; ++i)
        if (ld_individuals[i] < 0 || ld_individuals[i] >= n_total) {
            h->err = "ld_band: individual index " + std::to_string(ld_individuals[i]) + " out of range [0, " + std::to_string(n_total) + ")";
            return 1;
        }
    if (upload_indlist(h, ld_individuals, n_ld)) return 1;
    Laps laps("ld_band");
    if (reduce_counts(h, true)) return 1;
    if (dev_alloc(h, &h->d_homf, (size_t)L)) return 1;
    LAUNCH(launch_hom_freq(h->d_counts, h->L0, h->d_src, L, h->d_homf, h->stream));
    if (dev_alloc(h, &h->d_invld, (size_t)(L + kPad) * inv_stride(W))) return 1;
    CK(cudaMemsetAsync(h->d_invld, 0, (size_t)(L + kPad) * inv_stride(W) * sizeof(double), h->stream));
    LdPhase ph;
    if (h->phased) {
        if (!h->d_alleles || !h->d_key) FAIL("ld_band: --phased needs the allele characters (put_alleles / put_tped_text), not pre-packed genotypes");
        ph.alleles = h->d_alleles; ph.key = h->d_key; ph.src = h->d_src; ph.missing = h->missing_char; ph.freq = h->d_freq;
    }
    if (dev_alloc(h, &h->d_ldplanes, ld_planes_words(L, n_ld, h->phased))) return 1;
    if (dev_alloc(h, &h->d_ldpairs, ld_pairs_doubles(L, W))) return 1;
    double* d_ld = nullptr;
    if (out_ld) CK(cudaMalloc(&d_ld, (size_t)L * W * sizeof(double)));
    laps.lap("alloc");
    int launches = 0;
    cudaError_t e = launch_ld_band(h->d_geno, h->row_words, h->d_indlist, n_ld, h->d_homf, h->d_chr_of, h->d_chr_start,
                                   h->n_chr, L, W, h->d_invld, d_ld, h->stream, &launches, h->comm,
                                   h->comm ? h->ind_offset : 0, h->n_ind, h->d_ldplanes, h->d_ldpairs, ph);
    h->launches += launches + 1;
    if (e != cudaSuccess) { if (d_ld) cudaFree(d_ld); h->err = std::string("ld_band: ") + cudaGetErrorString(e); return 1; }
    if (out_ld) {
        e = cudaMemcpyAsync(out_ld, d_ld, (size_t)L * W * sizeof(double), cudaMemcpyDeviceToHost, h->stream);
        if (e == cudaSuccess) e = cudaStreamSynchronize(h->stream);
        cudaFree(d_ld);
        if (e != cudaSuccess) { h->err = std::string("ld_band: ") + cudaGetErrorString(e); return 1; }
    }
    CK(cudaStreamSynchronize(h->stream));
    laps.lap("kernels");
    h->have_ld = true; h->ld_W = W;
    return 0;
}

}

static int ensure_weighted(garlic_gpu* h, int W)
{
    if (h->gpos.empty()) FAIL("weighted: genetic positions were not given to set_tables");
    if (!h->have_ld || h->ld_W != W) FAIL("weighted: call ld_band with this window size first");
    if (!h->d_wlut) {
        const int64_t L = h->L;
        if (dev_alloc(h, &h->d_nomut, (size_t)L + kPad)) return 1;
        if (dev_alloc(h, &h->d_norec, (size_t)L + kPad)) return 1;
        CK(cudaMemsetAsync(h->d_nomut, 0, (size_t)(L + kPad) * sizeof(double), h->stream));
        CK(cudaMemsetAsync(h->d_norec, 0, (size_t)(L + kPad) * sizeof(double), h->stream));
        LAUNCH(launch_wlod_weights(h->d_pos, h->d_gpos, h->d_chr_of, h->d_chr_start, L, h->mu, h->M, h->d_nomut, h->d_norec, h->stream));
        if (dev_alloc(h, &h->d_wlut, (size_t)(L + kPad) * 4)) return 1;
        CK(cudaMemsetAsync(h->d_wlut, 0, (size_t)(L + kPad) * 4 * sizeof(double), h->stream));
        LAUNCH(launch_build_wlut(h->d_lut, h->d_nomut, h->d_norec, L, h->d_wlut, h->stream));
    }
    return 0;
}
```

garlic_b200/csrc/kernels.cu:

```cuda
#include <cuda_runtime.h>
#include <stdlib.h>
#include <stdint.h>
#include <algorithm>
#include "common.cuh"
#include "walk.cuh"
#include "kernels.h"

namespace garlic {

__device__ __forceinline__ uint32_t smem_u32(const void* p) { return (uint32_t)__cvta_generic_to_shared(p); }
__device__ __forceinline__ void mbar_init(uint64_t* bar, int count)
{
    asm volatile("mbarrier.init.shared::cta.b64 [%0], %1;" ::"r"(smem_u32(bar)), "r"(count) : "memory");
    asm volatile("fence.mbarrier_init.release.cluster;" ::: "memory");
}
__device__ __forceinline__ void mbar_expect_tx(uint64_t* bar, uint32_t bytes)
{
    asm volatile("mbarrier.arrive.expect_tx.shared::cta.b64 _, [%0], %1;" ::"r"(smem_u32(bar)), "r"(bytes) : "memory");
}
__device__ __forceinline__ void tma_load_1d(void* dst_smem, const void* src, uint32_t bytes, uint64_t* bar)
{
    asm volatile("cp.async.bulk.shared::cluster.global.mbarrier::complete_tx::bytes [%0], [%1], %2, [%3];"
                 ::"r"(smem_u32(dst_smem)), "l"(src), "r"(bytes), "r"(smem_u32(bar)) : "memory");
}
__device__ __forceinline__ void mbar_wait(uint64_t* bar, uint32_t parity)
{
    asm volatile(
        "{\n"
        ".reg .pred p;\n"
        "WAIT_LOOP:\n"
        "mbarrier.try_wait.parity.shared::cta.b64 p, [%0], %1;\n"
        "@p bra WAIT_DONE;\n"
        "bra WAIT_LOOP;\n"
        "WAIT_DONE:\n"
        "}\n" ::"r"(smem_u32(bar)), "r"(parity) : "memory");
}

template <int SRC, bool ROH, bool DUMP, bool TILE>
__global__ void __launch_bounds__(kWalkThreads, TILE ? 4 : 2)
walk_kernel(const WalkParams P, const Item* __restrict__ items, int n_items, int n_groups, int tile_bytes,
            const int* __restrict__ cand_list, const unsigned* __restrict__ cand_cnt, int cand_stride)
{
    extern __shared__ __align__(128) unsigned char walk_smem[];
    unsigned char* tile_s = walk_smem;
    uint32_t* ring_smem = reinterpret_cast<uint32_t*>(walk_smem + (TILE ? tile_bytes : 0));
    const int NW = ((P.W + 31) >> 5) + 1;
    uint64_t* bar = reinterpret_cast<uint64_t*>(ring_smem + NW * blockDim.x);
    const int warp = threadIdx.x >> 5, lane = threadIdx.x & 31;
    const int gpb = blockDim.x >> 5;
    const int gblocks = (n_groups + gpb - 1) / gpb;
    const long long total = (long long)n_items * gblocks;
    if (TILE) {
        if (threadIdx.x == 0) mbar_init(bar, 1);
        __syncthreads();
    }
    uint32_t phase = 0;
    for (long long u = blockIdx.x; u < total; u += gridDim.x) {
        const int item = (int)(u / gblocks);
        const int group = (int)(u % gblocks) * gpb + warp;
        int n_lanes = P.n_lanes;
        const int* list = nullptr;
        if (cand_list) {
            n_lanes = (int)cand_cnt[item];
            list = cand_list + (int64_t)item * cand_stride;
            if ((int)(u % gblocks) * gpb * 32 >= n_lanes) continue;
        }
        const Item it = items[item];
        const char* tile = reinterpret_cast<const char*>(P.lut);
        int tile_lo = 0;
        if (TILE) {
            const int nblk = (it.own_hi - 1 - it.w0 + 31) >> 5;
            const uint32_t bytes = (uint32_t)(32 * nblk + P.W) * 32u;
            if (threadIdx.x == 0) {
                mbar_expect_tx(bar, bytes);
                tma_load_1d(tile_s, P.lut + (int64_t)it.w0 * 4, bytes, bar);
            }
            mbar_wait(bar, phase);
            phase ^= 1u;
            tile = reinterpret_cast<const char*>(tile_s);
            tile_lo = it.w0;
        }
        if (group * 32 < n_lanes) {
            const int k = group * 32 + lane;
            const bool active = k < n_lanes;
            const int kk = active ? k : n_lanes - 1;
            walk_item<SRC, ROH, DUMP>(P, it, kk, active, ring_smem + threadIdx.x, blockDim.x, tile, tile_lo,
                                      list ? list[kk] : -1);
        }
        if (TILE) __syncthreads();
    }
}

__global__ void __launch_bounds__(kUnitThreads, 16)
walk_units_kernel(const WalkParams P, const Item* __restrict__ items, const int2* __restrict__ units,
                  const unsigned* __restrict__ n_units, unsigned unit_cap, int tile_bytes, const int* __restrict__ cand_list,
                  const unsigned* __restrict__ cand_cnt, int cand_stride)
{
    extern __shared__ __align__(128) unsigned char walk_smem[];
    unsigned char* tile_s = walk_smem;
    uint32_t* ring_smem = reinterpret_cast<uint32_t*>(walk_smem + tile_bytes);
    const int NW = ((P.W + 31) >> 5) + 1;
    uint64_t* bar = reinterpret_cast<uint64_t*>(ring_smem + NW * kUnitThreads);
    const int warp = threadIdx.x >> 5, lane = threadIdx.x & 31;
    if (threadIdx.x == 0) mbar_init(bar, 1);
    __syncthreads();
    unsigned nu = *n_units;
    nu = nu < unit_cap ? nu : unit_cap;
    uint32_t phase = 0;
    for (unsigned u = blockIdx.x; u < nu; u += gridDim.x) {
        const int2 un = units[u];
        const Item it = items[un.x];
        int n_lanes = (int)cand_cnt[un.x] - un.y;
        n_lanes = n_lanes < kUnitThreads ? n_lanes : kUnitThreads;
        const int* list = cand_list + (int64_t)un.x * cand_stride + un.y;
        const int nblk = (it.own_hi - 1 - it.w0 + 31) >> 5;
        const uint32_t bytes = (uint32_t)(32 * nblk + P.W) * 32u;
        if (threadIdx.x == 0) {
            mbar_expect_tx(bar, bytes);
            tma_load_1d(tile_s, P.lut + (int64_t)it.w0 * 4, bytes, bar);
        }
        mbar_wait(bar, phase);
        phase ^= 1u;
        if (warp * 32 < n_lanes) {
            const int k = warp * 32 + lane;
            const bool active = k < n_lanes;
            const int kk = active ? k : n_lanes - 1;
            walk_item<0, true, false>(P, it, kk, active, ring_smem + threadIdx.x, kUnitThreads,
                                      reinterpret_cast<const char*>(tile_s), it.w0, list[kk]);
        }
        __syncthreads();
    }
}

cudaError_t launch_walk_units(const WalkParams& P, const Item* items, const int2* units, const unsigned* n_units,
                              unsigned unit_cap, int tile_snps, const CandList& cl, cudaStream_t st)
{
    const int NW = ((P.W + 31) >> 5) + 1;
    const int tile_bytes = tile_snps * 32;
    const size_t smem = (size_t)tile_bytes + (size_t)NW * kUnitThreads * sizeof(uint32_t) + 16;
    if (smem > 48 * 1024) {
        cudaError_t e = cudaFuncSetAttribute(walk_units_kernel, cudaFuncAttributeMaxDynamicSharedMemorySize, (int)smem);
        if (e != cudaSuccess) return e;
    }
    int per_sm = (int)((227 * 1024) / (smem + 1024));
    per_sm = per_sm > 16 ? 16 : (per_sm < 1 ? 1 : per_sm);
    walk_units_kernel<<<148 * per_sm, kUnitThreads, smem, st>>>(P, items, units, n_units, unit_cap, tile_bytes, cl.list, cl.cnt,
                                                               cl.stride);
    return cudaGetLastError();
}

template <int SRC, bool ROH, bool DUMP>
static cudaError_t launch_walk_t(const WalkParams& P, const Item* items, int n_items, int tile_snps, const CandList& cl,
                                 cudaStream_t st)
{
    if (n_items == 0 || P.n_lanes == 0) return cudaSuccess;
    const int threads = kWalkThreads;
    const int n_groups = (P.n_lanes + 31) / 32;
    const int gpb = threads / 32;
    const long long total = (long long)n_items * ((n_groups + gpb - 1) / gpb);
    const int NW = ((P.W + 31) >> 5) + 1;
    const bool tile = (SRC == 0) && tile_snps > 0;
    const int tile_bytes = tile ? tile_snps * 32 : 0;
    const size_t smem = (size_t)tile_bytes + (size_t)NW * threads * sizeof(uint32_t) + 16;
    int dev = 0, sms = 148;
    cudaGetDevice(&dev);
    cudaDeviceGetAttribute(&sms, cudaDevAttrMultiProcessorCount, dev);
    long long grid = total;
    const long long cap = (long long)sms * 4 * 16;
    if (grid > cap) grid = cap;
    if (tile) {
        auto kern = walk_kernel<SRC, ROH, DUMP, true>;
        if (smem > 48 * 1024) {
            cudaError_t e = cudaFuncSetAttribute(kern, cudaFuncAttributeMaxDynamicSharedMemorySize, (int)smem);
            if (e != cudaSuccess) return e;
        }
        kern<<<(unsigned)grid, threads, smem, st>>>(P, items, n_items, n_groups, tile_bytes, cl.list, cl.cnt, cl.stride);
    } else {
        auto kern = walk_kernel<SRC, ROH, DUMP, false>;
        if (smem > 48 * 1024) {
            cudaError_t e = cudaFuncSetAttribute(kern, cudaFuncAttributeMaxDynamicSharedMemorySize, (int)smem);
            if (e != cudaSuccess) return e;
        }
        kern<<<(unsigned)grid, threads, smem, st>>>(P, items, n_items, n_groups, 0, cl.list, cl.cnt, cl.stride);
    }
    return cudaGetLastError();
}

constexpr int kGlPiece = 16;
constexpr int kGlPieceBytes = kGlPiece * kGlLanes * 8;

__device__ __forceinline__ void fence_proxy_async()
{
    asm volatile("fence.proxy.async.shared::cta;" ::: "memory");
}

template <bool CHK>
__global__ void __launch_bounds__(32)
gl_walk_kernel(const WalkParams P, const Item* __restrict__ items, int n_items, int n_groups, int NS)
{
    extern __shared__ __align__(128) unsigned char gl_smem[];
    const int lane = threadIdx.x;
    const int W = P.W;
    const int NW = ((W + 31) >> 5) + 1;
    const double* ring = reinterpret_cast<const double*>(gl_smem);
    uint32_t* fring = reinterpret_cast<uint32_t*>(gl_smem + (size_t)NS * kGlPieceBytes) + lane;
    uint64_t* bars = reinterpret_cast<uint64_t*>(gl_smem + (size_t)NS * kGlPieceBytes + (size_t)NW * 128);
    if (lane == 0) for (int s = 0; s < NS; ++s) mbar_init(&bars[s], 1);
    __syncwarp();
    const int R = NS * kGlPiece;
    uint64_t par = 0;
    const double cut_hi = CHK ? P.cutoff + P.tol : P.cutoff, cut_lo = P.cutoff - P.tol;
    const int r = (32 - (W & 31)) & 31;
    const long long total = (long long)n_items * n_groups;
    for (long long u = blockIdx.x; u < total; u += gridDim.x) {
        const int item = (int)(u / n_groups), group = (int)(u % n_groups);
        const Item it = items[item];
        const int ind = group * 32 + lane;
        const bool active = ind < P.n_lanes;
        const unsigned char* slab = reinterpret_cast<const unsigned char*>(P.gl + ((int64_t)group * P.gl_stride + it.w0) * kGlLanes);
        const int M = it.own_hi - 1 - it.w0;
        const int nblk = (M + 31) >> 5;
        const int NQ = (W + 32 * nblk + kGlPiece - 1) / kGlPiece;
        int issued = 0, waited = 0;
        int islot = 0, wslot = 0;
        auto issue_upto = [&](int qmax) {
            const int hi = qmax + 1 < NQ ? qmax + 1 : NQ;
            if (hi <= issued) return;
            __syncwarp();
            if (lane == 0) fence_proxy_async();
            for (; issued < hi; ++issued) {
                if (lane == 0) {
                    mbar_expect_tx(&bars[islot], kGlPieceBytes);
                    tma_load_1d(gl_smem + (size_t)islot * kGlPieceBytes, slab + (size_t)issued * kGlPieceBytes, kGlPieceBytes,
                                &bars[islot]);
                }
                if (++islot == NS) islot = 0;
            }
        };
        auto wait_upto = [&](int q) {
            for (; waited <= q; ++waited) {
                mbar_wait(&bars[wslot], (uint32_t)(par >> wslot) & 1u);
                par ^= 1ull << wslot;
                if (++wslot == NS) wslot = 0;
            }
        };
        issue_upto(NS - 1);
        double win = 0.0;
        for (int q = 0; q * kGlPiece < W; ++q) {
            wait_upto(q);
            const int n = W - q * kGlPiece < kGlPiece ? W - q * kGlPiece : kGlPiece;
            const double* p = ring + (size_t)q * kGlPiece * kGlLanes + lane;
            for (int i = 0; i < n; ++i) win += p[i * kGlLanes];
        }
        LaneState S;
        S.win = win; S.run_start = -1; S.fw = 0; S.ambig = false;
        const bool f0 = win >= cut_hi;
        if (CHK) S.ambig = (f0 != (win >= cut_lo));
        S.cov = (int)f0;
        S.hist = (uint32_t)f0 << 31;
        if (it.w0 >= it.own_lo && S.cov >= P.thr) S.run_start = it.w0;
        if (W > 32) {
            for (int w = 0; w < NW; ++w) fring[w * 32] = 0;
            fring[0] = (uint32_t)f0 << 31;
        }
        int wr = 1 % NW;
        int tblk = it.w0 + 1;
        int pin = W % R, pout = 0;
        for (int j = 0; j < nblk; ++j, tblk += 32) {
            wait_upto((W + 32 * j + 31) / kGlPiece);
            const int kwrap = R - pin;
            const double* p_in = ring + (size_t)pin * kGlLanes + lane;
            const double* p_in2 = p_in - (size_t)R * kGlLanes;
            const double* p_out = ring + (size_t)pout * kGlLanes + lane;
            uint32_t vm = 0xffffffffu;
            const int nv = it.we - tblk;
            if (nv < 32) vm = nv <= 0 ? 0u : ((1u << nv) - 1u);
            uint32_t fhi = 0, flo = 0;
            double d[32], o[CHK ? 1 : 32];
            if (kwrap >= 32) {
#pragma unroll
                for (int k = 0; k < 32; ++k) {
                    if (CHK) d[k] = p_in[k * kGlLanes] - p_out[k * kGlLanes];
                    else { d[k] = p_in[k * kGlLanes]; o[k] = p_out[k * kGlLanes]; }
                }
            } else {
#pragma unroll
                for (int k = 0; k < 32; ++k) {
                    const double a_in = (k < kwrap ? p_in : p_in2)[k * kGlLanes];
                    if (CHK) d[k] = a_in - p_out[k * kGlLanes];
                    else { d[k] = a_in; o[k] = p_out[k * kGlLanes]; }
                }
            }
            if (CHK) {
#pragma unroll
                for (int k = 0; k < 32; ++k) {
                    win = win + d[k];
                    d[k] = win;
                    if (win >= cut_lo) flo |= 1u << k;
                }
                if (__any_sync(0xffffffffu, flo != 0u)) {
#pragma unroll
                    for (int k = 0; k < 32; ++k) if (d[k] >= cut_hi) fhi |= 1u << k;
                }
            } else {
#pragma unroll
                for (int k = 0; k < 32; ++k) {
                    win = (win - o[k]) + d[k];
                    if (win >= cut_hi) fhi |= 1u << k;
                }
            }
            S.win = win;
            fhi &= vm;
            if (CHK) { flo &= vm; S.ambig |= (fhi != flo); }
            uint32_t ow = 0;
            if (W > 32) {
                int r0 = wr + 1; if (r0 >= NW) r0 -= NW;
                int r1 = r0 + 1; if (r1 >= NW) r1 -= NW;
                const uint32_t w0_ = fring[r0 * 32], w1_ = fring[r1 * 32];
                ow = r ? ((w0_ >> r) | (w1_ << (32 - r))) : w0_;
            }
            const bool full = (tblk + 31 < it.we) && (tblk >= it.own_lo) && (tblk + 31 < it.own_hi);
            if (full) cover_block<true>(P, it, S, ind, active, fhi, ow, tblk);
            else cover_block<false>(P, it, S, ind, active, fhi, ow, tblk);
            if (W > 32) {
                fring[wr * 32] = S.fw;
                if (++wr >= NW) wr = 0;
            }
            pin += 32; if (pin >= R) pin -= R;
            pout += 32; if (pout >= R) pout -= R;
            issue_upto(2 * j + 1 + NS);
        }
        if (S.run_start >= 0) emit_run(P, it, ind, active, S.run_start, it.own_hi - 1);
        if (CHK && S.ambig && active) {
            const unsigned p = atomicAdd(P.out_count + 1, 1u);
            if (p < P.amb_cap) {
                RohRec rr;
                rr.ind = ind; rr.a = 0; rr.b = 0; rr.tag = it.seg;
                P.amb[p] = rr;
            }
        }
        wait_upto(NQ - 1);
        __syncwarp();
    }
}

__device__ __forceinline__ void seq_wait(const volatile int* p, int v)
{
    while (*p < v) { }
    __threadfence_block();
}
__device__ __forceinline__ void seq_post(volatile int* p, int v, int lane)
{
    __threadfence_block();
    __syncwarp();
    if (lane == 0) *p = v;
}

__global__ void __launch_bounds__(128)
gl_relay_kernel(const WalkParams P, const Item* __restrict__ items, int n_items, int n_groups, int NS)
{
    extern __shared__ __align__(128) unsigned char gl_smem[];
    const int lane = threadIdx.x & 31, warp = threadIdx.x >> 5, K = blockDim.x >> 5;
    const int W = P.W;
    const int NW = ((W + 31) >> 5) + 1;
    const double* ring = reinterpret_cast<const double*>(gl_smem);
    unsigned char* aux = gl_smem + (size_t)NS * kGlPieceBytes;
    uint32_t* fring = reinterpret_cast<uint32_t*>(aux) + lane;
    uint64_t* bars = reinterpret_cast<uint64_t*>(aux + (size_t)NW * 128);
    double* sbase = reinterpret_cast<double*>(aux + (size_t)NW * 128 + 512) + lane;
    int* scov = reinterpret_cast<int*>(aux + (size_t)NW * 128 + 512 + 256) + lane;
    volatile int* seq = reinterpret_cast<volatile int*>(aux + (size_t)NW * 128 + 512 + 256 + 384);
    if (threadIdx.x == 0) for (int s = 0; s < NS; ++s) mbar_init(&bars[s], 1);
    __syncthreads();
    const int R = NS * kGlPiece;
    uint64_t par = 0;
    const double cut_hi = P.cutoff + P.tol, cut_lo = P.cutoff - P.tol;
    const int r = (32 - (W & 31)) & 31;
    const long long total = (long long)n_items * n_groups;
    for (long long u = blockIdx.x; u < total; u += gridDim.x) {
        const int item = (int)(u / n_groups), group = (int)(u % n_groups);
        const Item it = items[item];
        const int ind = group * 32 + lane;
        const bool active = ind < P.n_lanes;
        const unsigned char* slab = reinterpret_cast<const unsigned char*>(P.gl + ((int64_t)group * P.gl_stride + it.w0) * kGlLanes);
        const int M = it.own_hi - 1 - it.w0;
        const int nblk = (M + 31) >> 5;
        const int NQ = (W + 32 * nblk + kGlPiece - 1) / kGlPiece;
        __syncthreads();
        if (threadIdx.x == 0) { seq[0] = -1; seq[1] = -1; }
        __syncthreads();
        int waited = 0, wslot = 0;
        auto wait_upto = [&](int q) {
            for (; waited <= q; ++waited) {
                mbar_wait(&bars[wslot], (uint32_t)(par >> wslot) & 1u);
                par ^= 1ull << wslot;
                if (++wslot == NS) wslot = 0;
            }
        };
        auto issue = [&](int q0, int q1) {
            if (q1 > NQ) q1 = NQ;
            if (q0 >= q1) return;
            __syncwarp();
            if (lane == 0) {
                fence_proxy_async();
                int sl = q0 % NS;
                for (int q = q0; q < q1; ++q) {
                    mbar_expect_tx(&bars[sl], kGlPieceBytes);
                    tma_load_1d(gl_smem + (size_t)sl * kGlPieceBytes, slab + (size_t)q * kGlPieceBytes, kGlPieceBytes, &bars[sl]);
                    if (++sl == NS) sl = 0;
                }
            }
        };
        if (warp == 0) issue(0, NS);
        wait_upto((W + 31) / kGlPiece < NQ ? (W + 31) / kGlPiece : NQ - 1);
        bool ambig = false;
        if (warp == 0) {
            double win = 0.0;
            for (int q = 0; q * kGlPiece < W; ++q) {
                const int n = W - q * kGlPiece < kGlPiece ? W - q * kGlPiece : kGlPiece;
                const double* p = ring + (size_t)q * kGlPiece * kGlLanes + lane;
                for (int i = 0; i < n; ++i) win += p[i * kGlLanes];
            }
            const bool f0 = win >= cut_hi;
            ambig = (f0 != (win >= cut_lo));
            const int cov0 = (int)f0;
            sbase[0] = win;
            scov[0] = cov0;
            scov[32] = (it.w0 >= it.own_lo && cov0 >= P.thr) ? it.w0 : -1;
            scov[64] = (int)((uint32_t)f0 << 31);
            if (W > 32) {
                for (int w = 0; w < NW; ++w) fring[w * 32] = 0;
                fring[0] = (uint32_t)f0 << 31;
            }
            seq_post(&seq[0], 0, lane);
            seq_post(&seq[1], 0, lane);
        }
        __syncthreads();
        int wr = (1 + warp) % NW;
        int pin = (W + 32 * warp) % R, pout = (32 * warp) % R;
        for (int j = warp; j < nblk; j += K) {
            const int tblk = it.w0 + 1 + 32 * j;
            wait_upto((W + 32 * j + 31) / kGlPiece);
            const int kwrap = R - pin;
            const double* p_in = ring + (size_t)pin * kGlLanes + lane;
            const double* p_in2 = p_in - (size_t)R * kGlLanes;
            const double* p_out = ring + (size_t)pout * kGlLanes + lane;
            double d[32];
            if (kwrap >= 32) {
#pragma unroll
                for (int k = 0; k < 32; ++k) d[k] = p_in[k * kGlLanes] - p_out[k * kGlLanes];
// ... 956 lines not shown
```

garlic_b200/csrc/kernels.h:

```cpp
#pragma once
#include <cuda_runtime.h>
#include <stdint.h>
#include "common.cuh"

namespace garlic {

constexpr int kWalkThreads = 256;
constexpr int kTileSnpsMax = 1536;
constexpr int kUnitThreads = 64;

struct CandList {
    const int* list = nullptr;
    const unsigned* cnt = nullptr;
    int stride = 0;
};

cudaError_t launch_walk(const WalkParams& P, const Item* items, int n_items, bool gl_mode, bool roh,
                        bool dump, int tile_snps, const CandList& cl, cudaStream_t st);
cudaError_t launch_walk_units(const WalkParams& P, const Item* items, const int2* units, const unsigned* n_units,
                              unsigned unit_cap, int tile_snps, const CandList& cl, cudaStream_t st);

struct SqueezeParams {
    const uint64_t* gin;
    int64_t in_words;
    uint64_t* gout;
    int64_t out_words;
    const uint4* plan_head;
    const uint4* plan_seg;
    const uint32_t* plan_fast;
    const int2* piece_rng;
    const int* src;
    const int* n_kept;
    int n_ind;
    const uint4* hw;
    int lag;
    int partial;
    uint32_t low_mask;
    uint32_t* pmax;
    int64_t pmax_stride;
    int n_pieces, pieces_per_task, n_col_tasks;
};
cudaError_t launch_bound_tables(const double* lut, long long n_tab, long long n_hw, long long L, int W, uint4* hw, int* invalid, cudaStream_t st);
cudaError_t launch_plan(const int* src, const int* n_kept, long long n_q, uint4* head, uint4* segs, uint16_t* fast,
                        int2* piece_rng, cudaStream_t st);
cudaError_t launch_squeeze_bound(SqueezeParams P, bool squeeze, int c2, cudaStream_t st);
cudaError_t launch_select(const Item* items, int n_items, const uint32_t* pmax, int64_t stride, int n_ind, int cut_store,
                          const int* invalid, int* cand_list, int cand_stride, unsigned* cand_cnt, int2* units, unsigned* n_units,
                          unsigned unit_cap, int lanes_per_unit, int c2, cudaStream_t st);
cudaError_t launch_thin_windows(const uint64_t* geno, int64_t row_words, const double* lut, const int* ind_list, int n_lanes,
                                const uint32_t* bad_bits, long long L, const int2* meta, int n_chr, long long n_slots, int step, int W,
                                double* dump, int64_t dump_stride, const double* gl, int64_t gl_stride, const int* src, cudaStream_t st);
cudaError_t launch_fill_f64(double* p, size_t n, double v, cudaStream_t st);
cudaError_t launch_bucket_by_individual(RohRec* in, const unsigned* count, unsigned cap, unsigned* hist, int n_ind,
                                        RohRec* out, int thr, unsigned* kept, unsigned* total, cudaStream_t st);
cudaError_t launch_tokenize_tped(const char* text, const long long* off, int n_snp, int n_ind, int ind_lo, uint8_t* alleles,
                                 int* nonblank, cudaStream_t st);
cudaError_t launch_first_allele(const uint8_t* alleles, int n_snp, int n_ind, int ind_offset, int missing,
                                unsigned long long* key, cudaStream_t st);
cudaError_t launch_code_alleles(const uint8_t* alleles, int n_snp, int n_ind, int missing,
                                const unsigned long long* key, long long snp0, uint64_t* geno,
                                int64_t row_words, int* counts, long long L0, cudaStream_t st);
cudaError_t launch_count_packed(const uint64_t* geno, int64_t row_words, int n_ind, long long L0,
                                int* counts, cudaStream_t st);
cudaError_t launch_freq_keep(const int* counts, long long L0, const int* pos, const int* chr_of,
                             const int* chr_param, int oob, double* freq, uint8_t* keep, cudaStream_t st);
cudaError_t launch_keep_scan(const uint8_t* keep, long long L0, const int* chr_of0, int n_chr, int* block_counts,
                             int* total, int* src, int* chr_off_kept, cudaStream_t st);
cudaError_t launch_bad_pairs(const int* pos, const int* chr_of, const int* cen, int max_gap, long long L, int* list,
                             unsigned* count, unsigned cap, uint32_t* bad_bits, cudaStream_t st);
cudaError_t launch_gather_i32(const int* in, const int* src, long long L, int* out, cudaStream_t st);
cudaError_t launch_compact_gl(const double* in, int64_t in_stride, const int* src, long long L, const uint64_t* geno0,
                              int64_t row_words0, const double* freq0, double* out, int64_t out_stride, int n_ind, int type,
                              cudaStream_t st);
cudaError_t launch_gather_f64(const double* in, const int* src, long long L, double* out, cudaStream_t st);
cudaError_t launch_build_lut(const double* freq, long long L, double error, double* lut, cudaStream_t st);
cudaError_t launch_wlod_weights(const int* pos, const double* gpos, const int* chr_of, const int* chr_start,
                                long long L, double mu, int M, double* nomut, double* norec, cudaStream_t st);
cudaError_t launch_build_wlut(const double* lut, const double* nomut, const double* norec, long long L,
                              double* wlut, cudaStream_t st);
cudaError_t launch_tokenize_tgls(const char* text, const long long* off, int n_snp, int n_ind, int ind_lo, double* out,
                                 int64_t out_stride, long long snp0, int* n_tokens, int2* hard_list, unsigned* hard_count,
                                 unsigned hard_cap, cudaStream_t st);
constexpr int kXchgMaxRanks = 16, kXchgReady = 0, kXchgDone = 16;
struct XchgParams {
    int* counts[kXchgMaxRanks];
    double* freq[kXchgMaxRanks];
    uint8_t* keep[kXchgMaxRanks];
    unsigned* flags[kXchgMaxRanks];
    int n, rank;
    unsigned seq;
    long long L0;
    const int* pos; const int* chr_of; const int* chr_param; int oob;
    unsigned* done_counter;
};
cudaError_t launch_xchg_freq_keep(const XchgParams& P, cudaStream_t st);
size_t kde_scratch_doubles(int m);
cudaError_t launch_kde(const double* v, long long n, int m, double* scratch, double** out, int* launches, cudaStream_t st);

}
```

garlic_b200/csrc/segments.h:

```cpp
#pragma once
#include <algorithm>
#include <cstdint>
#include <vector>
#include "common.cuh"

namespace garlic {

struct Segment { int chr, ws, we; };

inline bool in_gap(int qs, int qe, int ts, int te)
{
    return (ts <= qs && te >= qs) || (ts <= qe && te >= qe) || (ts >= qs && te <= qe);
}

struct Stretch { int chr, a, b; };

inline void build_stretches(const std::vector<int64_t>& chr_off, const std::vector<int32_t>& pos,
                            const std::vector<int32_t>& cen, int max_gap, std::vector<Stretch>& out)
{
    out.clear();
    const int n_chr = (int)chr_off.size() - 1;
    for (int c = 0; c < n_chr; ++c) {
        const int lo = (int)chr_off[c], hi = (int)chr_off[c + 1];
        const int cs = cen[2 * c], ce = cen[2 * c + 1];
        int a = lo;
        for (int i = lo + 1; i <= hi; ++i) {
            bool brk = (i == hi);
            if (!brk) {
                const int p0 = pos[i - 1], p1 = pos[i];
                brk = (p1 - p0 > max_gap) || in_gap(p0, p1, cs, ce);
            }
            if (brk) {
                if (i > a) out.push_back({c, a, i});
                a = i;
            }
        }
    }
}

inline void segments_from_stretches(const std::vector<Stretch>& st, int W, std::vector<Segment>& segs)
{
    segs.clear();
    for (const Stretch& s : st)
        if (s.b - s.a >= W) segs.push_back({s.chr, s.a, s.b - W + 1});
}

inline void build_segments(const std::vector<int64_t>& chr_off, const std::vector<int32_t>& pos,
                           const std::vector<int32_t>& cen, int max_gap, int W, std::vector<Segment>& segs)
{
    std::vector<Stretch> st;
    build_stretches(chr_off, pos, cen, max_gap, st);
    segments_from_stretches(st, W, segs);
}

inline int pick_chunk(int64_t L, int W, int n_lanes, int tile_max)
{
    const int c_tile = (tile_max - 2 * W - 32) / 32 * 32;
    if (c_tile >= 256) return c_tile;
    const int n_groups = (n_lanes + 31) / 32;
    const int64_t target_items = std::max<int64_t>(1, (148 * 16 * 4 + n_groups - 1) / n_groups);
    int64_t ch = L / target_items;
    const int64_t lo = std::max(256, 8 * W);
    ch = std::max<int64_t>(lo, std::min<int64_t>(ch, 8192));
    return (int)((ch + 31) / 32 * 32);
}

inline int items_tile_snps(const std::vector<Item>& items, int W)
{
    int m = 0;
    for (const Item& it : items) m = std::max(m, 32 * ((it.own_hi - 1 - it.w0 + 31) >> 5) + W);
    return m;
}

inline void build_items(const std::vector<int64_t>& chr_off, int W, const std::vector<Segment>& segs, int chunk,
                        int step, std::vector<Item>& items)
{
    items.clear();
    const int n_chr = (int)chr_off.size() - 1;
    std::vector<int> thin_base(n_chr + 1, 0);
    for (int c = 0; c < n_chr; ++c) {
        const int Lc = (int)(chr_off[c + 1] - chr_off[c]);
        thin_base[c + 1] = thin_base[c] + (step > 0 ? (Lc + step - 1) / step : 0);
    }
    for (size_t si = 0; si < segs.size(); ++si) {
        const Segment& s = segs[si];
        const int a = s.ws, b = s.we + W - 1;
        int n = 1, size = b - a;
        if (chunk > 0 && b - a > chunk) {
            n = (b - a + chunk - 1) / chunk;
            size = std::min(chunk, ((b - a + n - 1) / n + 31) / 32 * 32);
            n = (b - a + size - 1) / size;
        }
        for (int i = 0; i < n; ++i) {
            Item it;
            it.own_lo = a + i * size;
            it.own_hi = std::min(b, it.own_lo + size);
            it.w0 = std::max(a, it.own_lo - W + 1);
            it.we = s.we;
            it.seg = (int)si;
            it.flags = (i > 0 ? 1 : 0) | (i + 1 < n ? 2 : 0);
            it.chr_start = (int)chr_off[s.chr];
            it.thin_base = thin_base[s.chr];
            items.push_back(it);
        }
    }
}

inline void build_items_aligned(const std::vector<int64_t>& chr_off, int W, const std::vector<Segment>& segs, int piece,
                                std::vector<Item>& items)
{
    items.clear();
    std::vector<int> cuts;
    for (size_t si = 0; si < segs.size(); ++si) {
        const Segment& s = segs[si];
        const int a = s.ws, b = s.we + W - 1;
        cuts.clear();
        cuts.push_back(a);
        for (int c = (a / piece + 1) * piece; c < b; c += piece)
            if (c - a >= piece / 4 && b - c >= piece / 4) cuts.push_back(c);
        cuts.push_back(b);
        const int n = (int)cuts.size() - 1;
        for (int i = 0; i < n; ++i) {
            Item it;
            it.own_lo = cuts[i];
            it.own_hi = cuts[i + 1];
            it.w0 = std::max(a, it.own_lo - W + 1);
            it.we = s.we;
            it.seg = (int)si;
            it.flags = (i > 0 ? 1 : 0) | (i + 1 < n ? 2 : 0);
            it.chr_start = (int)chr_off[s.chr];
            it.thin_base = 0;
            items.push_back(it);
        }
    }
}

struct StitchScratch {
    std::vector<uint32_t> first, cur;
    std::vector<std::pair<uint64_t, uint32_t>> key;
};


inline void stitch_runs(std::vector<RohRec>& recs, int thr, std::vector<RohRec>& out, StitchScratch* scratch = nullptr)
{
    StitchScratch local;
    StitchScratch& S = scratch ? *scratch : local;
    int n_ind = 0;
    for (const RohRec& r : recs) n_ind = std::max(n_ind, r.ind + 1);
    std::vector<uint32_t>& first = S.first;
    first.assign(n_ind + 1, 0);
    for (const RohRec& r : recs) first[r.ind + 1]++;
    for (int i = 0; i < n_ind; ++i) first[i + 1] += first[i];
    std::vector<std::pair<uint64_t, uint32_t>>& key = S.key;
    key.resize(recs.size());
    {
        std::vector<uint32_t>& cur = S.cur;
        cur.assign(first.begin(), first.end() - 1);
        for (size_t i = 0; i < recs.size(); ++i)
            key[cur[recs[i].ind]++] = {((uint64_t)(uint32_t)recs[i].ind << 32) | (uint32_t)recs[i].a, (uint32_t)i};
    }
    for (int i = 0; i < n_ind; ++i) {
        const uint32_t lo = first[i], hi = first[i + 1];
        if (hi - lo > 24) std::sort(key.begin() + lo, key.begin() + hi);
        else
            for (uint32_t a = lo + 1; a < hi; ++a) {
                const auto v = key[a];
                uint32_t b = a;
                while (b > lo && key[b - 1] > v) { key[b] = key[b - 1]; --b; }
                key[b] = v;
            }
    }
    out.clear();
    out.reserve(recs.size());
    size_t i = 0;
    while (i < key.size()) {
        RohRec cur = recs[key[i++].second];
        while ((cur.tag & 2) && i < key.size()) {
            const RohRec& nx = recs[key[i].second];
            if (!(nx.ind == cur.ind && (nx.tag & 1) && nx.a == cur.b + 1 && (nx.tag >> 2) == (cur.tag >> 2))) break;
            cur.b = nx.b;
            cur.tag = (cur.tag & ~2) | (nx.tag & 2);
            ++i;
        }
        if (cur.b - cur.a + 1 < thr) continue;
        out.push_back(cur);
    }
}

inline void take_stitched(const RohRec* recs, size_t n, std::vector<RohRec>& out)
{
    out.resize(n);
    RohRec* o = out.data();
    size_t m = 0;
    for (size_t i = 0; i < n; ++i) {
        o[m] = recs[i];
        m += recs[i].ind >= 0;
    }
    out.resize(m);
}

}
```

garlic_b200/csrc/squeeze.cu:

```cuda
#include <cuda_runtime.h>
#include <stdint.h>
#include <algorithm>
#include "common.cuh"
#include "bound.cuh"
#include "kernels.h"

namespace garlic {

namespace {
constexpr int kSqWarps = 4;
constexpr int kSqStages = 4;
constexpr int kSqStageHw = 16, kSqStageShift = 4;
constexpr int kSqRingHw = kSqStages * kSqStageHw;
constexpr int kSqRowBytes = kSqRingHw * 4 + 8;
constexpr int kSqRingBytes = 32 * kSqRowBytes;
constexpr int kSqOutRowBytes = 144;
constexpr int kSqOutBytes = 32 * kSqOutRowBytes;
constexpr int kSqStashBytes = 32 + 256 + 256;
constexpr int kSqWarpBytes = kSqRingBytes + kSqOutBytes + kSqStashBytes;

__device__ __forceinline__ uint32_t sq_smem_u32(const void* p) { return (uint32_t)__cvta_generic_to_shared(p); }
__device__ __forceinline__ void cp_async8(uint32_t dst_smem, const void* src)
{
    asm volatile("cp.async.ca.shared.global [%0], [%1], 8;" ::"r"(dst_smem), "l"(src) : "memory");
}
__device__ __forceinline__ void cp_async_wait_dyn(int pending)
{
    switch (pending) {
        case 0: asm volatile("cp.async.wait_group 0;" ::: "memory"); break;
        case 1: asm volatile("cp.async.wait_group 1;" ::: "memory"); break;
        case 2: asm volatile("cp.async.wait_group 2;" ::: "memory"); break;
        case 3: asm volatile("cp.async.wait_group 3;" ::: "memory"); break;
        case 4: asm volatile("cp.async.wait_group 4;" ::: "memory"); break;
        case 5: asm volatile("cp.async.wait_group 5;" ::: "memory"); break;
        case 6: asm volatile("cp.async.wait_group 6;" ::: "memory"); break;
        default: asm volatile("cp.async.wait_group 7;" ::: "memory"); break;
    }
}
}

constexpr int kBtHw = 128;
namespace {
__device__ __forceinline__ void bt_mbar_init(uint64_t* bar)
{
    asm volatile("mbarrier.init.shared::cta.b64 [%0], 1;" ::"r"(sq_smem_u32(bar)) : "memory");
    asm volatile("fence.mbarrier_init.release.cluster;" ::: "memory");
}
__device__ __forceinline__ void bt_bulk_load(void* dst_smem, const void* src, uint32_t bytes, uint64_t* bar)
{
    asm volatile("mbarrier.arrive.expect_tx.shared::cta.b64 _, [%0], %1;" ::"r"(sq_smem_u32(bar)), "r"(bytes) : "memory");
    asm volatile("cp.async.bulk.shared::cluster.global.mbarrier::complete_tx::bytes [%0], [%1], %2, [%3];"
                 ::"r"(sq_smem_u32(dst_smem)), "l"(src), "r"(bytes), "r"(sq_smem_u32(bar)) : "memory");
}
__device__ __forceinline__ void bt_mbar_wait(uint64_t* bar, uint32_t parity)
{
    asm volatile(
        "{\n"
        ".reg .pred p;\n"
        "BT_WAIT_LOOP:\n"
        "mbarrier.try_wait.parity.shared::cta.b64 p, [%0], %1;\n"
        "@p bra BT_WAIT_DONE;\n"
        "bra BT_WAIT_LOOP;\n"
        "BT_WAIT_DONE:\n"
        "}\n" ::"r"(sq_smem_u32(bar)), "r"(parity) : "memory");
}
}

__global__ void __launch_bounds__(kBtHw)
bound_tables_kernel(const double* __restrict__ lut, long long n_hw, long long L, int W, uint4* __restrict__ hw, int* __restrict__ invalid,
                    int stage_snps, long long n_tab)
{
    extern __shared__ __align__(128) double bt_smem[];
    uint64_t* bar = reinterpret_cast<uint64_t*>(bt_smem + (size_t)stage_snps * 4);
    const int c2 = bound_c2(W);
    if (threadIdx.x == 0) bt_mbar_init(bar);
    __syncthreads();
    uint32_t phase = 0;
    for (long long k0 = (long long)blockIdx.x * kBtHw; k0 < n_hw; k0 += (long long)gridDim.x * kBtHw) {
        const long long kb = k0 >= c2 ? k0 - c2 : 0;
        const long long s_lo = kb * 16;
        __syncthreads();
        const long long have = n_tab - s_lo < stage_snps ? n_tab - s_lo : stage_snps;
        if (threadIdx.x == 0) bt_bulk_load(bt_smem, lut + s_lo * 4, (uint32_t)(have * 32), bar);
        for (long long i = have * 4 + threadIdx.x; i < (long long)stage_snps * 4; i += kBtHw) bt_smem[i] = 0.0;
        bt_mbar_wait(bar, phase);
        phase ^= 1u;
        __syncthreads();
        const long long k = k0 + threadIdx.x;
        if (k < n_hw) {
            const double* tab = bt_smem - s_lo * 4;
            int bad = 0;
            uint4 e = bound_hw_entry(tab, k, L, &bad);
            e.w = k >= c2 ? (uint32_t)bound_block_max(tab, k - c2, W) : 0u;
            hw[k] = e;
            if (bad) atomicOr(invalid, 1);
        }
    }
}

cudaError_t launch_bound_tables(const double* lut, long long n_tab, long long n_hw, long long L, int W, uint4* hw, int* invalid, cudaStream_t st)
{
    if (!n_hw) return cudaSuccess;
    const int c2 = bound_c2(W);
    const int stage_snps = std::max(16 * (kBtHw + c2), 16 * (kBtHw - 1) + 16 + W + 16);
    const size_t smem = (size_t)stage_snps * 32 + 16;
    if (smem > 200 * 1024) return cudaErrorInvalidValue;
    cudaError_t e = cudaFuncSetAttribute(bound_tables_kernel, cudaFuncAttributeMaxDynamicSharedMemorySize, (int)smem);
    if (e != cudaSuccess) return e;
    long long blocks = (n_hw + kBtHw - 1) / kBtHw;
    if (blocks > 148 * 8) blocks = 148 * 8;
    bound_tables_kernel<<<(unsigned)blocks, kBtHw, smem, st>>>(lut, n_hw, L, W, hw, invalid, stage_snps, n_tab);
    return cudaGetLastError();
}

__global__ void plan_kernel(const int* __restrict__ src, const int* __restrict__ n_kept, long long n_q,
                            uint4* __restrict__ head, uint4* __restrict__ segs, uint16_t* __restrict__ fast,
                            int2* __restrict__ piece_rng)
{
    const long long L = *n_kept;
    for (long long q = blockIdx.x * (long long)blockDim.x + threadIdx.x; q < n_q; q += (long long)gridDim.x * blockDim.x) {
        uint4 hd;
        plan_half(src, L, q, &hd, segs + q * kPlanSegMax);
        head[q] = hd;
        const long long d0 = (q & ~15ll) * 16;
        const int a0 = d0 < L ? src[d0] >> 4 : -1;
        const uint32_t code = a0 >= 0 ? plan_fast_code(hd, a0 & ~1, (int)(q & 15)) : 0xffffu;
        fast[q] = (uint16_t)code;
        const unsigned slow = __ballot_sync(__activemask(), code == 0xffffu);
        if ((q & 15) == 0) {
            int2 r = make_int2(-1, 0);
            if (a0 >= 0) {
                const long long d1 = d0 + kPiece - 1 < L ? d0 + kPiece - 1 : L - 1;
                const int a1 = src[d1] >> 4;
                r.x = a0;
                r.y = (int)((unsigned)(a1 - a0 < 0xffff ? a1 - a0 : 0xffff) << 16);
            }
            r.y |= (int)((slow >> (threadIdx.x & 16)) & 0xffffu);
            piece_rng[q >> 4] = r;
        }
    }
}

cudaError_t launch_plan(const int* src, const int* n_kept, long long n_q, uint4* head, uint4* segs, uint16_t* fast,
                        int2* piece_rng, cudaStream_t st)
{
    if (!n_q) return cudaSuccess;
    long long blocks = (n_q + 127) / 128;
    if (blocks > 148 * 16) blocks = 148 * 16;
    plan_kernel<<<(unsigned)blocks, 128, 0, st>>>(src, n_kept, n_q, head, segs, fast, piece_rng);
    return cudaGetLastError();
}

template <bool SQUEEZE, bool BOUND, int C2, int LAG, bool PARTIAL>
__global__ void __launch_bounds__(kSqWarps * 32)
squeeze_bound_kernel(const SqueezeParams P)
{
    extern __shared__ __align__(16) unsigned char sq_smem[];
    const int warp = __shfl_sync(0xffffffffu, (int)(threadIdx.x >> 5), 0);
    const int lane = threadIdx.x & 31;
    unsigned char* ring_s = sq_smem + (size_t)warp * kSqWarpBytes;
    unsigned char* out_s = ring_s + kSqRingBytes;
    const uint32_t* my_ring = reinterpret_cast<const uint32_t*>(ring_s + lane * kSqRowBytes);
    const uint2* my_ring64 = reinterpret_cast<const uint2*>(ring_s + lane * kSqRowBytes);
    uint32_t* my_out = reinterpret_cast<uint32_t*>(out_s + lane * kSqOutRowBytes);
    uint32_t* sh_fast = reinterpret_cast<uint32_t*>(out_s + kSqOutBytes);
    uint4* sh_tab = reinterpret_cast<uint4*>(sh_fast + 8);
    uint4* sh_head = sh_tab + 16;
    const int c4 = lane & 7, rsel4 = lane >> 3;
    const uint32_t ring_u32 = sq_smem_u32(ring_s);
    const int n_rg = (P.n_ind + 31) >> 5;
    const long long n_kept = SQUEEZE ? (long long)*P.n_kept : 0;
    const long long n_out_words = SQUEEZE ? (n_kept + 31) >> 5 : 0;
    const long long n_tasks = (long long)n_rg * P.n_col_tasks;
    for (long long task = (long long)blockIdx.x * kSqWarps + warp; task < n_tasks; task += (long long)gridDim.x * kSqWarps) {
        const int rg = (int)(task % n_rg), ct = (int)(task / n_rg);
        const int pc_lo = ct * P.pieces_per_task;
        const int pc_hi = min(P.n_pieces, pc_lo + P.pieces_per_task);
        const int row = rg * 32 + lane;
        const bool active = row < P.n_ind;
        const uint32_t* grow32 = reinterpret_cast<const uint32_t*>(P.gin + (int64_t)(active ? row : P.n_ind - 1) * P.in_words);
        int issued = 0;
        const uint64_t* cp_src[8];
#pragma unroll
        for (int i = 0; i < 8; ++i) {
            int gr = rg * 32 + 4 * i + rsel4;
            gr = gr < P.n_ind ? gr : P.n_ind - 1;
            cp_src[i] = P.gin + (int64_t)gr * P.in_words + c4;
        }
        const uint32_t cp_dst = ring_u32 + (uint32_t)(rsel4 * kSqRowBytes + c4 * 8);
        auto issue = [&](int t) {
            const long long w0 = (long long)t * (kSqStageHw / 2);
            if (w0 + kSqStageHw / 2 <= P.in_words) {
                const uint32_t dst = cp_dst + (uint32_t)((t & (kSqStages - 1)) * (kSqStageHw * 4));
#pragma unroll
                for (int i = 0; i < 8; ++i) cp_async8(dst + i * 4 * kSqRowBytes, cp_src[i] + w0);
            }
            asm volatile("cp.async.commit_group;" ::: "memory");
        };
        auto stage_in = [&](int a_lo, int a_hi) -> bool {
            if (a_hi < a_lo) return true;
            const int lo_st = a_lo >> kSqStageShift, hi_st = a_hi >> kSqStageShift;
            if (hi_st - lo_st > 2) return false;
            if (issued < lo_st) {
                asm volatile("cp.async.wait_group 0;" ::: "memory");
                issued = lo_st;
            }
            __syncwarp();
#pragma unroll 1
            while (issued <= lo_st + kSqStages - 1) issue(issued++);
            cp_async_wait_dyn(issued - 1 - hi_st);
            __syncwarp();
            return true;
        };

        BoundState S;
        bound_reset(S);
        uint32_t r_fast = 0u;
        uint4 r_tab = make_uint4(0u, 0u, 0u, 0u);
        int2 r_rng = make_int2(-1, 0);
        const uint4* tab_src = lane < 16 ? P.hw + lane : P.plan_head + (lane - 16);
        const bool tab_on = lane < 16 ? BOUND : SQUEEZE;
        auto fetch = [&](int piece) {
            if (SQUEEZE && lane < 8) r_fast = P.plan_fast[(long long)piece * 8 + lane];
            if (tab_on) r_tab = tab_src[(long long)piece * 16];
            r_rng = SQUEEZE ? P.piece_rng[piece] : make_int2(piece * 16, 15 << 16);
        };
        fetch(pc_lo);
        const int pi_end = BOUND ? pc_hi + 1 : pc_hi;
#pragma unroll 1
        for (int pi = pc_lo; pi < pi_end; ++pi) {
            const long long qb = (long long)pi * 16;
            __syncwarp();
            const int2 rng = r_rng;
            const bool ring_ok = stage_in(rng.x, rng.x < 0 ? -2 : rng.x + (int)((unsigned)rng.y >> 16));
            if (SQUEEZE && lane < 8) sh_fast[lane] = r_fast;
            if (tab_on) sh_tab[lane] = r_tab;
            __syncwarp();
            fetch(pi + 1);
            uint32_t hreg[16];
            uint32_t* dst = my_out + ((pi & 1) << 4);
            if (SQUEEZE) {
                uint32_t w[20];
                const uint32_t u0 = (uint32_t)rng.x >> 1;
#pragma unroll
                for (int j = 0; j < 10; ++j) {
                    const uint2 v = my_ring64[(u0 + j) & (kSqRingHw / 2 - 1)];
                    w[2 * j] = v.x; w[2 * j + 1] = v.y;
                }
#pragma unroll
                for (int I = 0; I < 16; ++I) {
                    const uint32_t cw = sh_fast[I >> 1];
                    const uint32_t b0 = __byte_perm(cw, 0u, (I & 1) ? 0x4442u : 0x4440u);
                    const uint32_t p2 = __byte_perm(cw, 0u, (I & 1) ? 0x4443u : 0x4441u);
                    const uint32_t k = b0 & 3u, sh = b0 >> 2;
                    const uint32_t x0 = k == 0u ? w[I] : (k == 1u ? w[I + 1] : w[I + 2]);
                    const uint32_t x1 = k == 0u ? w[I + 1] : (k == 1u ? w[I + 2] : w[I + 3]);
                    const uint32_t x2 = k == 0u ? w[I + 2] : (k == 1u ? w[I + 3] : w[I + 4]);
                    const uint32_t lo = __funnelshift_r(x0, x1, sh), hi = __funnelshift_r(x1, x2, sh);
                    const uint32_t m = __funnelshift_lc(0xffffffffu, 0u, p2);
                    hreg[I] = (lo & m) | (__funnelshift_r(lo, hi, 2u) & ~m);
                }
#pragma unroll
                for (int I = 0; I < 16; I += 4) *reinterpret_cast<uint4*>(dst + I) = make_uint4(hreg[I], hreg[I + 1], hreg[I + 2], hreg[I + 3]);
                unsigned slow = ring_ok ? ((unsigned)rng.y & 0xffffu) : 0xffffu;
                if (slow) {
#pragma unroll 1
                    for (; slow; slow &= slow - 1u) {
                        const int I = __ffs((int)slow) - 1;
                        const uint4 hd = sh_head[I];
                        uint32_t h;
                        if (hd.x & 0x100u) {
                            const uint32_t a = hd.y;
                            if (ring_ok) h = plan_window(hd, my_ring[a & (kSqRingHw - 1)], my_ring[(a + 1) & (kSqRingHw - 1)], my_ring[(a + 2) & (kSqRingHw - 1)]);
                            else h = plan_window(hd, grow32[a], plan_need1(hd) ? grow32[a + 1] : 0u, plan_need2(hd) ? grow32[a + 2] : 0u);
                        } else {
                            h = hd.w;
                            const uint4* sg = P.plan_seg + (qb + I) * kPlanSegMax;
                            const int ns = (int)hd.x;
#pragma unroll 1
                            for (int k = 0; k < ns; ++k) {
                                const uint4 g = sg[k];
                                const uint32_t x = ring_ok ? my_ring[g.x & (kSqRingHw - 1)] : grow32[g.x];
                                h |= ((x >> g.y) & g.z) << g.w;
                            }
                        }
                        dst[I] = h;
                    }
                    __syncwarp();
#pragma unroll
                    for (int I = 0; I < 16; ++I) hreg[I] = dst[I];
                }
            } else {
                const uint4* hsrc = reinterpret_cast<const uint4*>(my_ring + (qb & (kSqRingHw - 1)));
#pragma unroll
                for (int I = 0; I < 16; I += 4) { const uint2 v0 = reinterpret_cast<const uint2*>(hsrc)[I >> 1], v1 = reinterpret_cast<const uint2*>(hsrc)[(I >> 1) + 1]; hreg[I] = v0.x; hreg[I + 1] = v0.y; hreg[I + 2] = v1.x; hreg[I + 3] = v1.y; }
            }
            if (BOUND) {
#pragma unroll
                for (int I = 0; I < 16; ++I) {
                    const long long q = qb + I;
                    bound_step<C2, LAG, PARTIAL>(S, hreg[I], sh_tab[I], I, P.low_mask);
                    if (((I - C2) & 15) == 15) {
                        const int piece = (int)((q - C2) >> 4);
                        if (piece >= pc_lo && piece < pc_hi && active)
                            P.pmax[(int64_t)piece * P.pmax_stride + row] = bound_pack(S.pm_all, S.pm_tail);
                        S.pm_all = -0x40000000; S.pm_tail = -0x40000000;
                    }
                }
            }
            if (SQUEEZE && pi < pc_hi && ((pi & 1) || pi == pc_hi - 1)) {
                __syncwarp();
                const long long wd = 16ll * (pi >> 1) + 2 * c4;
                if (2 * c4 < ((pi & 1) ? 16 : 8) && wd < n_out_words) {
                    const unsigned char* sp = out_s + rsel4 * kSqOutRowBytes + c4 * 16;
                    uint64_t* gp = P.gout + (int64_t)(rg * 32 + rsel4) * P.out_words + wd;
                    const int rows = min(32, P.n_ind - rg * 32);
#pragma unroll 4
                    for (int r = rsel4; r < rows; r += 4, sp += 4 * kSqOutRowBytes, gp += 4 * P.out_words)
                        *reinterpret_cast<uint4*>(gp) = *reinterpret_cast<const uint4*>(sp);
                }
                __syncwarp();
            }
        }
        asm volatile("cp.async.wait_group 0;" ::: "memory");
        __syncwarp();
    }
}

template <bool SQUEEZE, bool BOUND, int C2, int LAG, bool PARTIAL>
static cudaError_t launch_sq_t(const SqueezeParams& P, unsigned grid, size_t smem, cudaStream_t st)
{
    auto kern = squeeze_bound_kernel<SQUEEZE, BOUND, C2, LAG, PARTIAL>;
    cudaError_t e = cudaFuncSetAttribute(kern, cudaFuncAttributeMaxDynamicSharedMemorySize, (int)smem);
    if (e != cudaSuccess) return e;
    kern<<<grid, kSqWarps * 32, smem, st>>>(P);
    return cudaGetLastError();
}

template <bool SQUEEZE, int LAG>
static cudaError_t launch_sq_c2(const SqueezeParams& P, int c2, unsigned grid, size_t smem, cudaStream_t st)
{
    switch (c2) {
        case 2: return launch_sq_t<SQUEEZE, true, 2, LAG, false>(P, grid, smem, st);
        case 3: return launch_sq_t<SQUEEZE, true, 3, LAG, false>(P, grid, smem, st);
        case 4: return launch_sq_t<SQUEEZE, true, 4, LAG, false>(P, grid, smem, st);
        case 5: return launch_sq_t<SQUEEZE, true, 5, LAG, false>(P, grid, smem, st);
        case 6: return launch_sq_t<SQUEEZE, true, 6, LAG, false>(P, grid, smem, st);
        case 7: return launch_sq_t<SQUEEZE, true, 7, LAG, false>(P, grid, smem, st);
        case 8: return launch_sq_t<SQUEEZE, true, 8, LAG, false>(P, grid, smem, st);
        case 9: return launch_sq_t<SQUEEZE, true, 9, LAG, false>(P, grid, smem, st);
        case 10: return launch_sq_t<SQUEEZE, true, 10, LAG, false>(P, grid, smem, st);
        case 11: return launch_sq_t<SQUEEZE, true, 11, LAG, false>(P, grid, smem, st);
        case 12: return launch_sq_t<SQUEEZE, true, 12, LAG, false>(P, grid, smem, st);
        case 13: return launch_sq_t<SQUEEZE, true, 13, LAG, false>(P, grid, smem, st);
        default: return cudaErrorInvalidValue;
    }
}

template <bool SQUEEZE>
static cudaError_t launch_sq_partial(const SqueezeParams& P, int c2, unsigned grid, size_t smem, cudaStream_t st)
{
    if (c2 == 1) return launch_sq_t<SQUEEZE, true, 1, 1, true>(P, grid, smem, st);
    if (c2 == 2) return launch_sq_t<SQUEEZE, true, 2, 2, true>(P, grid, smem, st);
    return cudaErrorInvalidValue;
}

int squeeze_pieces_per_task(int n_ind, int n_pieces)
{
    const int n_rg = (n_ind + 31) / 32;
    const int want_tasks = 148 * 16 * 3;
    int n_col = std::max(1, (want_tasks + n_rg - 1) / n_rg);
    int ppt = (n_pieces + n_col - 1) / n_col;
    ppt = std::max(ppt, 16);
    ppt += ppt & 1;
    return ppt;
}

cudaError_t launch_squeeze_bound(SqueezeParams P, bool squeeze, int c2, cudaStream_t st)
{
    if (!P.n_ind || !P.n_pieces) return cudaSuccess;
    P.pieces_per_task = squeeze_pieces_per_task(P.n_ind, P.n_pieces);
    P.n_col_tasks = (P.n_pieces + P.pieces_per_task - 1) / P.pieces_per_task;
    const int n_rg = (P.n_ind + 31) / 32;
    const long long n_tasks = (long long)n_rg * P.n_col_tasks;
    long long grid = (n_tasks + kSqWarps - 1) / kSqWarps;
    if (grid > 148ll * 4 * 8) grid = 148ll * 4 * 8;
    const size_t smem = (size_t)kSqWarps * kSqWarpBytes;
    if (c2 <= 0) {
        if (!squeeze) return cudaErrorInvalidValue;
        return launch_sq_t<true, false, 2, 1, false>(P, (unsigned)grid, smem, st);
    }
    if (P.partial) return squeeze ? launch_sq_partial<true>(P, c2, (unsigned)grid, smem, st) : launch_sq_partial<false>(P, c2, (unsigned)grid, smem, st);
    if (P.lag == 1) return squeeze ? launch_sq_c2<true, 1>(P, c2, (unsigned)grid, smem, st) : launch_sq_c2<false, 1>(P, c2, (unsigned)grid, smem, st);
    if (P.lag == 2) return squeeze ? launch_sq_c2<true, 2>(P, c2, (unsigned)grid, smem, st) : launch_sq_c2<false, 2>(P, c2, (unsigned)grid, smem, st);
    return cudaErrorInvalidValue;
}

__global__ void __launch_bounds__(256)
select_kernel(const Item* __restrict__ items, int n_items, const uint32_t* __restrict__ pmax, int64_t stride, int n_ind,
              int cut_store, const int* __restrict__ invalid, int* __restrict__ cand_list, int cand_stride,
              unsigned* __restrict__ cand_cnt, int2* __restrict__ units, unsigned* __restrict__ n_units, unsigned unit_cap,
              int lanes_per_unit, int c2)
{
    __shared__ int s_n;
    const int lane = threadIdx.x & 31;
    if (*invalid) cut_store = -32768;
    for (int item = blockIdx.x; item < n_items; item += gridDim.x) {
        const Item it = items[item];
        __syncthreads();
        if (threadIdx.x == 0) s_n = 0;
        __syncthreads();
        int* list = cand_list + (int64_t)item * cand_stride;
        const int rounds = (n_ind + 255) >> 8;
        for (int r = 0; r < rounds; ++r) {
            const int ind = r * 256 + threadIdx.x;
            const bool c = ind < n_ind && bound_item_candidate(pmax, stride, ind, it, cut_store, c2);
            const unsigned m = __ballot_sync(0xffffffffu, c);
            if (m) {
                int base = 0;
                if (lane == 0) base = atomicAdd(&s_n, __popc(m));
                base = __shfl_sync(0xffffffffu, base, 0);
                if (c) list[base + __popc(m & ((1u << lane) - 1u))] = ind;
            }
        }
        __syncthreads();
        if (threadIdx.x == 0) {
            const int total = s_n;
            cand_cnt[item] = (unsigned)total;
            const int nu = (total + lanes_per_unit - 1) / lanes_per_unit;
            if (nu) {
                const unsigned b = atomicAdd(n_units, (unsigned)nu);
                for (int u = 0; u < nu; ++u)
                    if (b + u < unit_cap) units[b + u] = make_int2(item, u * lanes_per_unit);
                atomicAdd(n_units + 1, (unsigned)total);
            }
        }
    }
}

cudaError_t launch_select(const Item* items, int n_items, const uint32_t* pmax, int64_t stride, int n_ind, int cut_store,
                          const int* invalid, int* cand_list, int cand_stride, unsigned* cand_cnt, int2* units, unsigned* n_units,
                          unsigned unit_cap, int lanes_per_unit, int c2, cudaStream_t st)
{
    if (!n_items || !n_ind) return cudaSuccess;
    const int grid = n_items < 148 * 8 ? n_items : 148 * 8;
    select_kernel<<<grid, 256, 0, st>>>(items, n_items, pmax, stride, n_ind, cut_store, invalid, cand_list, cand_stride, cand_cnt, units,
                                        n_units, unit_cap, lanes_per_unit, c2);
    return cudaGetLastError();
}

}
```

garlic_b200/csrc/walk.cuh:

```cuda
#pragma once
#include <math.h>
#include "common.cuh"

namespace garlic {

GHD double lod_eval(int g, double f, double e)
{
    if (f == 0 || f == 1 || g == 3) return 0.0;
    double a, na;
    if (g == 0) {
        na = (1 - f) * (1 - f);
        a = (1 - e) * (1 - f) + e * na;
    } else if (g == 1) {
        na = 2 * (f) * (1 - f);
        a = e * na;
    } else {
        na = (f) * (f);
        a = (1 - e) * (f) + e * na;
    }
    return log10(a / na);
}

template <int SRC>
struct LaneCtx {
    const uint64_t* row;
    const char* tile;
    int tile_lo;
    const double* freq;
    const double* glrow;
    GHD double aval(int s, int g) const
    {
        if (SRC == 0) return *reinterpret_cast<const double*>(tile + ((uint32_t)(s - tile_lo) * 32u + (uint32_t)g * 8u));
        return glrow[(int64_t)s * kGlLanes];
    }
};

struct LaneState {
    double win;
    int cov;
    int run_start;
    uint32_t fw;
    uint32_t hist;
    bool ambig;
};

GHD void emit_run(const WalkParams& P, const Item& it, int ind, bool active, int a, int b)
{
    const int ol = (a == it.own_lo) && (it.flags & 1);
    const int orr = (b == it.own_hi - 1) && (it.flags & 2);
    if (!active) return;
    if (!(ol | orr) && (b - a + 1 < P.thr)) return;
#ifdef __CUDA_ARCH__
    unsigned p = atomicAdd(P.out_count, 1u);
#else
    unsigned p = P.out_count[0]++;
#endif
    if (p < P.out_cap) {
        RohRec r;
        r.ind = ind; r.a = a; r.b = b; r.tag = (it.seg << 2) | (orr << 1) | ol;
        P.out[p] = r;
#ifdef __CUDA_ARCH__
        if (P.hist) atomicAdd(P.hist + ind, 1u);
#endif
    }
}

template <bool DUMP>
GHD void dump_window(const WalkParams& P, const Item& it, int k, bool active, int t, double win)
{
    if (!DUMP) return;
    const int d = t - it.chr_start;
    if (active && t >= it.own_lo && (d % P.dump_step) == 0)
        P.dump[(int64_t)k * P.dump_stride + it.thin_base + d / P.dump_step] = win;
}

GHD int popc32(uint32_t x)
{
#ifdef __CUDA_ARCH__
    return __popc(x);
#else
    return __builtin_popcount(x);
#endif
}

GHD int nth_set_bit(uint32_t x, int n)
{
    int pos = 0, c;
    c = popc32(x & 0xffffu); if (n > c) { n -= c; pos += 16; x >>= 16; }
    c = popc32(x & 0xffu);   if (n > c) { n -= c; pos += 8;  x >>= 8; }
    c = popc32(x & 0xfu);    if (n > c) { n -= c; pos += 4;  x >>= 4; }
    c = popc32(x & 0x3u);    if (n > c) { n -= c; pos += 2;  x >>= 2; }
    c = (int)(x & 1u);       if (n > c) { pos += 1; }
    return pos;
}

GHD uint32_t lut_off(uint32_t w, int kk)
{
    return kk >= 2 ? ((w >> (2 * kk - 3)) & 24u) : ((w << (3 - 2 * kk)) & 24u);
}

template <bool FULL>
GHD void cover_block(const WalkParams& P, const Item& it, LaneState& S, int ind, bool active, uint32_t fw, uint32_t ow,
                     int tblk)
{
    const int W = P.W;
    S.fw = fw;

    bool busy = (fw | (uint32_t)S.cov) != 0u;
#ifdef __CUDA_ARCH__
    busy = __any_sync(0xffffffffu, busy);
#endif
    if (!busy) {
        if (W <= 32) S.hist = 0;
        return;
    }
    uint32_t owv = ow;
    if (W <= 32) owv = (W == 32) ? S.hist : ((fw << W) | (S.hist >> (32 - W)));
    const uint32_t d1 = fw & ~owv, d2 = owv & ~fw;
    int cov = S.cov;
    uint32_t cw;
    bool mixed = (d1 != 0u) && (d2 != 0u);
#ifdef __CUDA_ARCH__
    mixed = __any_sync(0xffffffffu, mixed);
#endif
    if (mixed) {
        cw = 0;
#pragma unroll
        for (int k = 0; k < 32; ++k) {
            cov += (int)((d1 >> k) & 1u) - (int)((d2 >> k) & 1u);
            cw |= (uint32_t)(cov >= P.thr) << k;
        }
    } else if (d1) {
        const int n = P.thr - cov, c = popc32(d1);
        cw = n <= 0 ? 0xffffffffu : (n > c ? 0u : (0xffffffffu << nth_set_bit(d1, n)));
        cov += c;
    } else if (d2) {
        const int m = cov - P.thr, c = popc32(d2);
        cw = m < 0 ? 0u : (m >= c ? 0xffffffffu : ((1u << nth_set_bit(d2, m + 1)) - 1u));
        cov -= c;
    } else {
        cw = cov >= P.thr ? 0xffffffffu : 0u;
    }
    S.cov = cov;
    if (W <= 32) S.hist = fw;
    uint32_t em = 0xffffffffu;
    if (!FULL) {
        const int lo = it.own_lo - tblk, hi = it.own_hi - tblk;
        const uint32_t mlo = lo <= 0 ? 0xffffffffu : (lo >= 32 ? 0u : ~((1u << lo) - 1u));
        const uint32_t mhi = hi >= 32 ? 0xffffffffu : (hi <= 0 ? 0u : ((1u << hi) - 1u));
        em = mlo & mhi;
    }
    const uint32_t x = cw & em;
    const uint32_t inr = S.run_start >= 0 ? 1u : 0u;
    uint32_t trans = x ^ ((x << 1) | inr);
    while (trans) {
#ifdef __CUDA_ARCH__
        const int k = __ffs((int)trans) - 1;
#else
        const int k = __builtin_ctz(trans);
#endif
        trans &= trans - 1;
        const int t = tblk + k;
        if ((x >> k) & 1u) S.run_start = t;
        else { emit_run(P, it, ind, active, S.run_start, t - 1); S.run_start = -1; }
    }
}

template <int SRC, bool ROH, bool DUMP, bool FULL, bool CHK>
GHD void walk_block(const WalkParams& P, const Item& it, const LaneCtx<SRC>& C, LaneState& S, int ind,
                    int k_slot, bool active, uint64_t gin, uint64_t gout, int tblk, uint32_t ow)
{
    const int W = P.W;
    const double cut_hi = CHK ? P.cutoff + P.tol : P.cutoff, cut_lo = P.cutoff - P.tol;
    const int s_in0 = tblk + W - 1, s_out0 = tblk - 1;
    uint32_t vm = 0xffffffffu;
    if (!FULL) {
        const int n = it.we - tblk;
        vm = n >= 32 ? 0xffffffffu : (n <= 0 ? 0u : ((1u << n) - 1u));
    }
    uint32_t fhi = 0, flo = 0;
    double win = S.win;
    if (SRC == 0) {
        const uint32_t bi = (uint32_t)(s_in0 - C.tile_lo) * 32u, bo = (uint32_t)(s_out0 - C.tile_lo) * 32u;
        const uint32_t gi0 = (uint32_t)gin, gi1 = (uint32_t)(gin >> 32);
        const uint32_t go0 = (uint32_t)gout, go1 = (uint32_t)(gout >> 32);
#pragma unroll
        for (int k = 0; k < 32; ++k) {
            const uint32_t oi = lut_off(k < 16 ? gi0 : gi1, k & 15), oo = lut_off(k < 16 ? go0 : go1, k & 15);
            const double a_in = *reinterpret_cast<const double*>(C.tile + ((bi | oi) + k * 32));
            const double a_out = *reinterpret_cast<const double*>(C.tile + ((bo | oo) + k * 32));
            if (CHK) win = win + (a_in - a_out);
            else win = (win - a_out) + a_in;
            if (ROH) {
                if (win >= cut_hi) fhi |= 1u << k;
                if (CHK) { if (win >= cut_lo) flo |= 1u << k; }
            }
            if (DUMP) { if ((vm >> k) & 1u) dump_window<DUMP>(P, it, k_slot, active, tblk + k, win); }
        }
    } else {
#pragma unroll 4
        for (int k = 0; k < 32; ++k) {
            const int go = (int)(gout >> (2 * k)) & 3, gi = (int)(gin >> (2 * k)) & 3;
            win = (win - C.aval(s_out0 + k, go)) + C.aval(s_in0 + k, gi);
            if (ROH) {
                if (win >= cut_hi) fhi |= 1u << k;
                if (CHK) { if (win >= cut_lo) flo |= 1u << k; }
            }
            if (DUMP) { if ((vm >> k) & 1u) dump_window<DUMP>(P, it, k_slot, active, tblk + k, win); }
        }
    }
    S.win = win;
    if (!ROH) return;
    fhi &= vm;
    if (CHK) { flo &= vm; S.ambig |= (fhi != flo); }
    cover_block<FULL>(P, it, S, ind, active, fhi, ow, tblk);
}

template <int SRC, bool ROH, bool DUMP>
GHD void walk_item(const WalkParams& P, const Item& it, int k_slot, bool active, uint32_t* ring, int rstride,
                   const char* tile, int tile_lo, int ind_in = -1)
{
    const int W = P.W;
    const int ind = ind_in >= 0 ? ind_in : (P.ind_list ? P.ind_list[k_slot] : k_slot);
    LaneCtx<SRC> C;
    C.row = P.geno + (int64_t)ind * P.row_words;
    C.tile = tile;
    C.tile_lo = tile_lo;
    C.freq = P.freq;
    C.glrow = (SRC == 1) ? gl_lane(P, ind) : nullptr;
    const int NW = ((W + 31) >> 5) + 1;
    const bool chk = P.tol > 0;

    double win = 0.0;
    for (int i = 0; i < W; ++i) {
        const int s = it.w0 + i;
        const int g = (int)(C.row[s >> 5] >> (2 * (s & 31))) & 3;
        win += C.aval(s, g);
    }
    LaneState S;
    S.win = win; S.run_start = -1; S.fw = 0; S.ambig = false;
    const bool f0 = win >= (chk ? P.cutoff + P.tol : P.cutoff);
    if (chk) S.ambig = (f0 != (win >= P.cutoff - P.tol));
    dump_window<DUMP>(P, it, k_slot, active, it.w0, win);
    S.cov = (int)f0;
    S.hist = (uint32_t)f0 << 31;
    if (ROH && it.w0 >= it.own_lo && S.cov >= P.thr) S.run_start = it.w0;
    if (W > 32) {
        for (int w = 0; w < NW; ++w) ring[w * rstride] = 0;
        ring[0] = (uint32_t)f0 << 31;
    }

    const int M = it.own_hi - 1 - it.w0;
    const int sa = 2 * ((it.w0 + W) & 31), sb = 2 * (it.w0 & 31);
    const uint64_t* pa = C.row + ((it.w0 + W) >> 5);
    const uint64_t* pb = C.row + (it.w0 >> 5);
    uint64_t a_lo = pa[0], b_lo = pb[0];
    uint64_t a_hi = pa[1], b_hi = pb[1];
    pa += 2; pb += 2;
    const int r = (32 - (W & 31)) & 31;
    int wr = 1 % NW;
    int tblk = it.w0 + 1;
    for (int m0 = 0; m0 < M; m0 += 32, tblk += 32) {
        const uint64_t a_nx = *pa++, b_nx = *pb++;
        const uint64_t gin = sa ? ((a_lo >> sa) | (a_hi << (64 - sa))) : a_lo;
        const uint64_t gout = sb ? ((b_lo >> sb) | (b_hi << (64 - sb))) : b_lo;
        a_lo = a_hi; b_lo = b_hi; a_hi = a_nx; b_hi = b_nx;
        uint32_t ow = 0;
        if (ROH && W > 32) {
            int r0 = wr + 1; if (r0 >= NW) r0 -= NW;
            int r1 = r0 + 1; if (r1 >= NW) r1 -= NW;
            const uint32_t w0_ = ring[r0 * rstride], w1_ = ring[r1 * rstride];
            ow = r ? ((w0_ >> r) | (w1_ << (32 - r))) : w0_;
        }
        const bool full = (tblk + 31 < it.we) && (tblk >= it.own_lo) && (tblk + 31 < it.own_hi);
        if (chk) {
            if (full) walk_block<SRC, ROH, DUMP, true, true>(P, it, C, S, ind, k_slot, active, gin, gout, tblk, ow);
            else walk_block<SRC, ROH, DUMP, false, true>(P, it, C, S, ind, k_slot, active, gin, gout, tblk, ow);
        } else {
            if (full) walk_block<SRC, ROH, DUMP, true, false>(P, it, C, S, ind, k_slot, active, gin, gout, tblk, ow);
            else walk_block<SRC, ROH, DUMP, false, false>(P, it, C, S, ind, k_slot, active, gin, gout, tblk, ow);
        }
        if (ROH && W > 32) {
            ring[wr * rstride] = S.fw;
            if (++wr >= NW) wr = 0;
        }
    }
    if (ROH && S.run_start >= 0) emit_run(P, it, ind, active, S.run_start, it.own_hi - 1);
    if (chk && S.ambig && active) {
#ifdef __CUDA_ARCH__
        unsigned p = atomicAdd(P.out_count + 1, 1u);
#else
        unsigned p = P.out_count[1]++;
#endif
        if (p < P.amb_cap) {
            RohRec rr;
            rr.ind = ind; rr.a = 0; rr.b = 0; rr.tag = it.seg;
            P.amb[p] = rr;
        }
    }
}

}
```

Before: 1238 billion.

## Defer compacted genotype store; gather raw rows per unit via plan in walk

Skips writing the compacted genotype matrix during the squeeze/bound pass when the pruned units walk can run. The units kernel instead gathers each lane's needed slice of compacted bits from the raw genotype rows into shared memory using the precomputed plan tables. The squeeze kernel gains a STORE template flag with a smaller shared footprint and higher CTA occupancy when no tile is stored. Full compaction is still done lazily for fallback paths such as exact, ambiguous or partial cases. This trades a full-matrix write for per-thread gather work and extra shared memory in the walk kernel, which may reduce its occupancy.

```diff
diff --git a/garlic_b200/csrc/bound.cuh b/garlic_b200/csrc/bound.cuh
--- a/garlic_b200/csrc/bound.cuh
+++ b/garlic_b200/csrc/bound.cuh
@@ -239,4 +239,22 @@
     return lo;
 }
 
-}
+GHD uint32_t plan_gather(const uint4& hd, const uint4* sg, const uint32_t* hin)
+{
+    if (hd.x & 0x100u) return plan_window(hd, hin[hd.y], plan_need1(hd) ? hin[hd.y + 1] : 0u, plan_need2(hd) ? hin[hd.y + 2] : 0u);
+    uint32_t h = hd.w;
+    for (uint32_t k = 0; k < hd.x; ++k) { const uint4 g = sg[k]; h |= ((hin[g.x] >> g.y) & g.z) << g.w; }
+    return h;
+}
+
+GHD void plan_slice(const uint4* head, const uint4* segs, long long L, const uint32_t* hin, long long wlo, int n, uint64_t* out)
+{
+    for (int j = 0; j < n; ++j) {
+        const long long q = 2 * (wlo + j);
+        const uint32_t lo = 16 * q < L ? plan_gather(head[q], segs + q * kPlanSegMax, hin) : 0xffffffffu;
+        const uint32_t hi = 16 * (q + 1) < L ? plan_gather(head[q + 1], segs + (q + 1) * kPlanSegMax, hin) : 0xffffffffu;
+        out[j] = (uint64_t)hi << 32 | lo;
+    }
+}
+
+}
diff --git a/garlic_b200/csrc/capi.cu b/garlic_b200/csrc/capi.cu
--- a/garlic_b200/csrc/capi.cu
+++ b/garlic_b200/csrc/capi.cu
@@ -75,7 +75,7 @@
     std::vector<Segment> p2_segs;
     std::vector<Item> p2_items;
     Item* d_items_p2 = nullptr;
-    int p2_W = 0, p2_tile = 0, p2_chunk = 0;
+    int p2_W = 0, p2_tile = 0, p2_chunk = 0, p2_slice = 0;
     uint64_t tables_gen = 0, p2_gen = 0;
     size_t sorted_cap = 0;
     unsigned out_cap = 0, amb_cap = 0;
@@ -918,10 +918,6 @@
     if (n_kept) *n_kept = L;
     if (L < 1) FAIL("filter: no polymorphic loci left");
     h->row_words = (((L + kPad + 31) >> 5) + 3) & ~(int64_t)1;
-    const bool fresh = h->cap.find((void*)&h->d_geno) == h->cap.end() || !h->d_geno ||
-                       h->cap[(void*)&h->d_geno] < (size_t)h->n_ind * h->row_words * 8;
-    if (dev_alloc(h, &h->d_geno, (size_t)h->n_ind * h->row_words)) return 1;
-    if (fresh) CK(cudaMemsetAsync(h->d_geno, 0xff, (size_t)h->n_ind * h->row_words * 8, h->stream));
     h->n_pieces = (int)((L + kPiece - 1) / kPiece);
     {
         const long long n_q = 16ll * (h->n_pieces + 4);
@@ -1192,6 +1188,12 @@
     return h->prune && h->tables && !h->have_gl && W >= kBoundMinW && W <= 1280;
 }
 
+static bool units_walk(const garlic_gpu* h, int W)
+{
+    const int span = kPiece * h->item_pieces + W - 2;
+    return can_bound(h, W) && !bound_partial(W) && 32 * ((span + 31) / 32) + W <= kTileSnpsMax;
+}
+
 static int ensure_bound_tables(garlic_gpu* h, int W)
 {
     if (h->bound_tables_W == W) return 0;
@@ -1232,15 +1234,19 @@
 static int ensure_geno(garlic_gpu* h, int W_hint)
 {
     if (!h->geno_pending) return 0;
+    const bool fresh = h->cap.find((void*)&h->d_geno) == h->cap.end() || !h->d_geno ||
+                       h->cap[(void*)&h->d_geno] < (size_t)h->n_ind * h->row_words * 8;
+    if (dev_alloc(h, &h->d_geno, (size_t)h->n_ind * h->row_words)) return 1;
+    if (fresh) CK(cudaMemsetAsync(h->d_geno, 0xff, (size_t)h->n_ind * h->row_words * 8, h->stream));
     int c2 = 0;
-    if (W_hint > 0 && can_bound(h, W_hint)) {
+    if (W_hint > 0 && can_bound(h, W_hint) && h->bound_W != W_hint) {
         if (ensure_bound_tables(h, W_hint)) return 1;
         if (alloc_pmax(h)) return 1;
         c2 = bound_c2(W_hint);
     }
     const SqueezeParams Q = squeeze_params(h, true, W_hint);
     CK(cudaEventRecord(h->ev_sq0, h->stream));
-    LAUNCH(launch_squeeze_bound(Q, true, c2, h->stream));
+    LAUNCH(launch_squeeze_bound(Q, true, true, c2, h->stream));
     CK(cudaEventRecord(h->ev_sq1, h->stream));
     h->sq_timed = true;
     h->geno_pending = false;
@@ -1257,6 +1263,7 @@
     h->p2_chunk = 0;
     for (const Item& it : h->p2_items) h->p2_chunk = std::max(h->p2_chunk, it.own_hi - it.own_lo);
     h->p2_tile = items_tile_snps(h->p2_items, W);
+    h->p2_slice = items_slice_words(h->p2_items, W);
     if (dev_alloc(h, &h->d_items_p2, h->p2_items.size() + 1)) return 1;
     if (!h->p2_items.empty())
         CK(cudaMemcpyAsync(h->d_items_p2, h->p2_items.data(), h->p2_items.size() * sizeof(Item), cudaMemcpyHostToDevice, h->stream));
@@ -1266,13 +1273,14 @@
 
 static int ensure_bound(garlic_gpu* h, int W)
 {
-    if (ensure_geno(h, W)) return 1;
     if (h->bound_W == W) return 0;
+    if (h->geno_pending && bound_partial(W)) return ensure_geno(h, W);
     if (ensure_bound_tables(h, W)) return 1;
     if (alloc_pmax(h)) return 1;
-    const SqueezeParams Q = squeeze_params(h, false, W);
+    const bool raw = h->geno_pending;
+    const SqueezeParams Q = squeeze_params(h, raw, W);
     CK(cudaEventRecord(h->ev_sq0, h->stream));
-    LAUNCH(launch_squeeze_bound(Q, false, bound_c2(W), h->stream));
+    LAUNCH(launch_squeeze_bound(Q, raw, false, bound_c2(W), h->stream));
     CK(cudaEventRecord(h->ev_sq1, h->stream));
     h->sq_timed = true;
     h->bound_W = W;
@@ -1395,7 +1403,7 @@
         if (side) {
             if (begin_side(h)) return 1;
             ws = h->aux_stream;
-            if (ensure_geno(h, winsize)) return 1;
+            if (units_walk(h, W) ? ensure_bound(h, W) : ensure_geno(h, winsize)) return 1;
         }
         tl_mark(h, "windows:squeeze-enqueued");
         if (h->bound_W == W && prepare_p2_items(h, W)) return 1;
@@ -1490,7 +1498,7 @@
     int cut_ok = 0;
     bound_cut_store(cutoff, 1.0, &cut_ok);
     bool prune = !exact && !weighted && can_bound(h, W) && cut_ok;
-    if (ensure_geno(h, prune ? W : 0)) return 1;
+    if (prune && units_walk(h, W) ? ensure_bound(h, W) : ensure_geno(h, prune ? W : 0)) return 1;
     double thr_d = overlap_frac * W;
     thr_d = (thr_d >= 1) ? thr_d : 1;
     thr_d = (thr_d <= W) ? thr_d : W;
@@ -1509,6 +1517,7 @@
         prune = h->p2_tile <= kTileSnpsMax && (int64_t)h->p2_items.size() * h->n_ind < (1ll << 31);
         if (prune) chunk = h->p2_chunk;
     }
+    if (!(prune && !bound_partial(W)) && ensure_geno(h, 0)) return 1;
     const Item* d_its = h->d_items;
     const std::vector<Item>* its = &items;
     if (prune) {
@@ -1574,7 +1583,12 @@
         CK(cudaEventRecord(h->ev2, h->stream));
         if (dev_alloc(h, &h->d_sorted, (size_t)h->out_cap)) return 1;
         P.hist = h->d_hist;
-        if (prune_now && !bound_partial(W)) LAUNCH(launch_walk_units(P, d_its, h->d_units, h->d_nunits, unit_cap, tile_snps, cl, h->stream));
+        if (prune_now && !bound_partial(W)) {
+            RawRows R;
+            R.rows = h->geno_pending ? h->d_geno0 : nullptr; R.row_words = h->row_words0;
+            R.head = h->d_plan_head; R.segs = h->d_plan_seg; R.L = h->L;
+            LAUNCH(launch_walk_units(P, R, d_its, h->d_units, h->d_nunits, unit_cap, tile_snps, h->p2_slice, cl, h->stream));
+        }
         else if (prune_now) LAUNCH(launch_walk(P, d_its, n_its, false, true, false, tile_snps, cl, h->stream));
         else if (launch_any_walk(h, P, d_its, n_its, weighted, true, false, tile_snps)) return 1;
         CK(cudaEventRecord(h->ev1, h->stream));
@@ -1606,6 +1620,7 @@
         }
         if (n_amb > h->amb_cap) {
             exact = 1; prune = false;
+            if (ensure_geno(h, 0)) return 1;
             build_items(h->chr_off, W, segs, 0, 0, items);
             if (upload_items(h, items)) return 1;
             d_its = h->d_items; its = &items;
@@ -1626,6 +1641,7 @@
     laps.lap("kernel+d2h");
     int64_t n_amb_pairs = 0;
     if (!ambs.empty()) {
+        if (ensure_geno(h, 0)) return 1;
         std::map<int, std::vector<int>> by_seg;
         for (const RohRec& a : ambs) by_seg[a.tag].push_back(a.ind);
         std::vector<RohRec> fixed;
diff --git a/garlic_b200/csrc/kernels.cu b/garlic_b200/csrc/kernels.cu
--- a/garlic_b200/csrc/kernels.cu
+++ b/garlic_b200/csrc/kernels.cu
@@ -4,6 +4,7 @@
 #include <algorithm>
 #include "common.cuh"
 #include "walk.cuh"
+#include "bound.cuh"
 #include "kernels.h"
 
 namespace garlic {
@@ -92,13 +93,14 @@
 }
 
 __global__ void __launch_bounds__(kUnitThreads, 16)
-walk_units_kernel(const WalkParams P, const Item* __restrict__ items, const int2* __restrict__ units,
-                  const unsigned* __restrict__ n_units, unsigned unit_cap, int tile_bytes, const int* __restrict__ cand_list,
-                  const unsigned* __restrict__ cand_cnt, int cand_stride)
+walk_units_kernel(const WalkParams P, const RawRows R, const Item* __restrict__ items, const int2* __restrict__ units,
+                  const unsigned* __restrict__ n_units, unsigned unit_cap, int tile_bytes, int slice_stride,
+                  const int* __restrict__ cand_list, const unsigned* __restrict__ cand_cnt, int cand_stride)
 {
     extern __shared__ __align__(128) unsigned char walk_smem[];
     unsigned char* tile_s = walk_smem;
-    uint32_t* ring_smem = reinterpret_cast<uint32_t*>(walk_smem + tile_bytes);
+    uint64_t* slice_s = reinterpret_cast<uint64_t*>(walk_smem + tile_bytes) + (size_t)threadIdx.x * slice_stride;
+    uint32_t* ring_smem = reinterpret_cast<uint32_t*>(walk_smem + tile_bytes + (size_t)slice_stride * kUnitThreads * 8);
     const int NW = ((P.W + 31) >> 5) + 1;
     uint64_t* bar = reinterpret_cast<uint64_t*>(ring_smem + NW * kUnitThreads);
     const int warp = threadIdx.x >> 5, lane = threadIdx.x & 31;
@@ -119,33 +121,40 @@
             mbar_expect_tx(bar, bytes);
             tma_load_1d(tile_s, P.lut + (int64_t)it.w0 * 4, bytes, bar);
         }
+        const bool busy = warp * 32 < n_lanes;
+        const int k = warp * 32 + lane;
+        const bool active = k < n_lanes;
+        const int kk = active ? k : n_lanes - 1;
+        const int ind = busy ? list[kk] : 0;
+        const int wlo = it.w0 >> 5;
+        if (busy && R.rows) {
+            const int n_w = ((it.w0 + P.W) >> 5) + nblk + 2 - wlo;
+            plan_slice(R.head, R.segs, R.L, reinterpret_cast<const uint32_t*>(R.rows + (int64_t)ind * R.row_words), wlo, n_w, slice_s);
+        }
         mbar_wait(bar, phase);
         phase ^= 1u;
-        if (warp * 32 < n_lanes) {
-            const int k = warp * 32 + lane;
-            const bool active = k < n_lanes;
-            const int kk = active ? k : n_lanes - 1;
+        if (busy)
             walk_item<0, true, false>(P, it, kk, active, ring_smem + threadIdx.x, kUnitThreads,
-                                      reinterpret_cast<const char*>(tile_s), it.w0, list[kk]);
-        }
-        __syncthreads();
-    }
-}
-
-cudaError_t launch_walk_units(const WalkParams& P, const Item* items, const int2* units, const unsigned* n_units,
-                              unsigned unit_cap, int tile_snps, const CandList& cl, cudaStream_t st)
+                                      reinterpret_cast<const char*>(tile_s), it.w0, ind, R.rows ? slice_s : nullptr, wlo);
+        __syncthreads();
+    }
+}
+
+cudaError_t launch_walk_units(const WalkParams& P, const RawRows& R, const Item* items, const int2* units, const unsigned* n_units,
+                              unsigned unit_cap, int tile_snps, int slice_words, const CandList& cl, cudaStream_t st)
 {
     const int NW = ((P.W + 31) >> 5) + 1;
     const int tile_bytes = tile_snps * 32;
-    const size_t smem = (size_t)tile_bytes + (size_t)NW * kUnitThreads * sizeof(uint32_t) + 16;
+    const int slice_stride = R.rows ? slice_words | 1 : 0;
+    const size_t smem = (size_t)tile_bytes + (size_t)slice_stride * kUnitThreads * 8 + (size_t)NW * kUnitThreads * sizeof(uint32_t) + 16;
     if (smem > 48 * 1024) {
         cudaError_t e = cudaFuncSetAttribute(walk_units_kernel, cudaFuncAttributeMaxDynamicSharedMemorySize, (int)smem);
         if (e != cudaSuccess) return e;
     }
     int per_sm = (int)((227 * 1024) / (smem + 1024));
     per_sm = per_sm > 16 ? 16 : (per_sm < 1 ? 1 : per_sm);
-    walk_units_kernel<<<148 * per_sm, kUnitThreads, smem, st>>>(P, items, units, n_units, unit_cap, tile_bytes, cl.list, cl.cnt,
-                                                               cl.stride);
+    walk_units_kernel<<<148 * per_sm, kUnitThreads, smem, st>>>(P, R, items, units, n_units, unit_cap, tile_bytes, slice_stride,
+                                                               cl.list, cl.cnt, cl.stride);
     return cudaGetLastError();
 }
 
diff --git a/garlic_b200/csrc/kernels.h b/garlic_b200/csrc/kernels.h
--- a/garlic_b200/csrc/kernels.h
+++ b/garlic_b200/csrc/kernels.h
@@ -17,8 +17,15 @@
 
 cudaError_t launch_walk(const WalkParams& P, const Item* items, int n_items, bool gl_mode, bool roh,
                         bool dump, int tile_snps, const CandList& cl, cudaStream_t st);
-cudaError_t launch_walk_units(const WalkParams& P, const Item* items, const int2* units, const unsigned* n_units,
-                              unsigned unit_cap, int tile_snps, const CandList& cl, cudaStream_t st);
+struct RawRows {
+    const uint64_t* rows;
+    int64_t row_words;
+    const uint4* head;
+    const uint4* segs;
+    long long L;
+};
+cudaError_t launch_walk_units(const WalkParams& P, const RawRows& R, const Item* items, const int2* units, const unsigned* n_units,
+                              unsigned unit_cap, int tile_snps, int slice_words, const CandList& cl, cudaStream_t st);
 
 struct SqueezeParams {
     const uint64_t* gin;
@@ -43,7 +50,7 @@
 cudaError_t launch_bound_tables(const double* lut, long long n_tab, long long n_hw, long long L, int W, uint4* hw, int* invalid, cudaStream_t st);
 cudaError_t launch_plan(const int* src, const int* n_kept, long long n_q, uint4* head, uint4* segs, uint16_t* fast,
                         int2* piece_rng, cudaStream_t st);
-cudaError_t launch_squeeze_bound(SqueezeParams P, bool squeeze, int c2, cudaStream_t st);
+cudaError_t launch_squeeze_bound(SqueezeParams P, bool squeeze, bool store, int c2, cudaStream_t st);
 cudaError_t launch_select(const Item* items, int n_items, const uint32_t* pmax, int64_t stride, int n_ind, int cut_store,
                           const int* invalid, int* cand_list, int cand_stride, unsigned* cand_cnt, int2* units, unsigned* n_units,
                           unsigned unit_cap, int lanes_per_unit, int c2, cudaStream_t st);
diff --git a/garlic_b200/csrc/segments.h b/garlic_b200/csrc/segments.h
--- a/garlic_b200/csrc/segments.h
+++ b/garlic_b200/csrc/segments.h
@@ -69,6 +69,14 @@
 {
     int m = 0;
     for (const Item& it : items) m = std::max(m, 32 * ((it.own_hi - 1 - it.w0 + 31) >> 5) + W);
+    return m;
+}
+
+inline int items_slice_words(const std::vector<Item>& items, int W)
+{
+    int m = 0;
+    for (const Item& it : items)
+        m = std::max(m, ((it.w0 + W) >> 5) + ((it.own_hi - 1 - it.w0 + 31) >> 5) + 2 - (it.w0 >> 5));
     return m;
 }
 
diff --git a/garlic_b200/csrc/squeeze.cu b/garlic_b200/csrc/squeeze.cu
--- a/garlic_b200/csrc/squeeze.cu
+++ b/garlic_b200/csrc/squeeze.cu
@@ -18,6 +18,8 @@
 constexpr int kSqOutBytes = 32 * kSqOutRowBytes;
 constexpr int kSqStashBytes = 32 + 256 + 256;
 constexpr int kSqWarpBytes = kSqRingBytes + kSqOutBytes + kSqStashBytes;
+constexpr int kSqWarpBytesNoTile = kSqRingBytes + kSqStashBytes;
+constexpr int kSqCtasPerSm = 4, kSqCtasPerSmNoTile = 5;
 
 __device__ __forceinline__ uint32_t sq_smem_u32(const void* p) { return (uint32_t)__cvta_generic_to_shared(p); }
 __device__ __forceinline__ void cp_async8(uint32_t dst_smem, const void* src)
@@ -151,26 +153,27 @@
     return cudaGetLastError();
 }
 
-template <bool SQUEEZE, bool BOUND, int C2, int LAG, bool PARTIAL>
-__global__ void __launch_bounds__(kSqWarps * 32)
+template <bool SQUEEZE, bool STORE, bool BOUND, int C2, int LAG, bool PARTIAL>
+__global__ void __launch_bounds__(kSqWarps * 32, SQUEEZE && STORE ? 0 : kSqCtasPerSmNoTile)
 squeeze_bound_kernel(const SqueezeParams P)
 {
+    constexpr bool TILE = SQUEEZE && STORE;
     extern __shared__ __align__(16) unsigned char sq_smem[];
     const int warp = __shfl_sync(0xffffffffu, (int)(threadIdx.x >> 5), 0);
     const int lane = threadIdx.x & 31;
-    unsigned char* ring_s = sq_smem + (size_t)warp * kSqWarpBytes;
+    unsigned char* ring_s = sq_smem + (size_t)warp * (TILE ? kSqWarpBytes : kSqWarpBytesNoTile);
     unsigned char* out_s = ring_s + kSqRingBytes;
     const uint32_t* my_ring = reinterpret_cast<const uint32_t*>(ring_s + lane * kSqRowBytes);
     const uint2* my_ring64 = reinterpret_cast<const uint2*>(ring_s + lane * kSqRowBytes);
     uint32_t* my_out = reinterpret_cast<uint32_t*>(out_s + lane * kSqOutRowBytes);
-    uint32_t* sh_fast = reinterpret_cast<uint32_t*>(out_s + kSqOutBytes);
+    uint32_t* sh_fast = reinterpret_cast<uint32_t*>(out_s + (TILE ? kSqOutBytes : 0));
     uint4* sh_tab = reinterpret_cast<uint4*>(sh_fast + 8);
     uint4* sh_head = sh_tab + 16;
     const int c4 = lane & 7, rsel4 = lane >> 3;
     const uint32_t ring_u32 = sq_smem_u32(ring_s);
     const int n_rg = (P.n_ind + 31) >> 5;
-    const long long n_kept = SQUEEZE ? (long long)*P.n_kept : 0;
-    const long long n_out_words = SQUEEZE ? (n_kept + 31) >> 5 : 0;
+    const long long n_kept = TILE ? (long long)*P.n_kept : 0;
+    const long long n_out_words = TILE ? (n_kept + 31) >> 5 : 0;
     const long long n_tasks = (long long)n_rg * P.n_col_tasks;
     for (long long task = (long long)blockIdx.x * kSqWarps + warp; task < n_tasks; task += (long long)gridDim.x * kSqWarps) {
         const int rg = (int)(task % n_rg), ct = (int)(task / n_rg);
@@ -260,8 +263,10 @@
                     const uint32_t m = __funnelshift_lc(0xffffffffu, 0u, p2);
                     hreg[I] = (lo & m) | (__funnelshift_r(lo, hi, 2u) & ~m);
                 }
-#pragma unroll
-                for (int I = 0; I < 16; I += 4) *reinterpret_cast<uint4*>(dst + I) = make_uint4(hreg[I], hreg[I + 1], hreg[I + 2], hreg[I + 3]);
+                if (TILE) {
+#pragma unroll
+                    for (int I = 0; I < 16; I += 4) *reinterpret_cast<uint4*>(dst + I) = make_uint4(hreg[I], hreg[I + 1], hreg[I + 2], hreg[I + 3]);
+                }
                 unsigned slow = ring_ok ? ((unsigned)rng.y & 0xffffu) : 0xffffu;
                 if (slow) {
 #pragma unroll 1
@@ -284,11 +289,18 @@
                                 h |= ((x >> g.y) & g.z) << g.w;
                             }
                         }
-                        dst[I] = h;
+                        if (TILE) {
+                            dst[I] = h;
+                        } else {
+#pragma unroll
+                            for (int J = 0; J < 16; ++J) hreg[J] = J == I ? h : hreg[J];
+                        }
                     }
-                    __syncwarp();
-#pragma unroll
-                    for (int I = 0; I < 16; ++I) hreg[I] = dst[I];
+                    if (TILE) {
+                        __syncwarp();
+#pragma unroll
+                        for (int I = 0; I < 16; ++I) hreg[I] = dst[I];
+                    }
                 }
             } else {
                 const uint4* hsrc = reinterpret_cast<const uint4*>(my_ring + (qb & (kSqRingHw - 1)));
@@ -308,7 +320,7 @@
                     }
                 }
             }
-            if (SQUEEZE && pi < pc_hi && ((pi & 1) || pi == pc_hi - 1)) {
+            if (TILE && pi < pc_hi && ((pi & 1) || pi == pc_hi - 1)) {
                 __syncwarp();
                 const long long wd = 16ll * (pi >> 1) + 2 * c4;
                 if (2 * c4 < ((pi & 1) ? 16 : 8) && wd < n_out_words) {
@@ -327,48 +339,48 @@
     }
 }
 
-template <bool SQUEEZE, bool BOUND, int C2, int LAG, bool PARTIAL>
+template <bool SQUEEZE, bool STORE, bool BOUND, int C2, int LAG, bool PARTIAL>
 static cudaError_t launch_sq_t(const SqueezeParams& P, unsigned grid, size_t smem, cudaStream_t st)
 {
-    auto kern = squeeze_bound_kernel<SQUEEZE, BOUND, C2, LAG, PARTIAL>;
+    auto kern = squeeze_bound_kernel<SQUEEZE, STORE, BOUND, C2, LAG, PARTIAL>;
     cudaError_t e = cudaFuncSetAttribute(kern, cudaFuncAttributeMaxDynamicSharedMemorySize, (int)smem);
     if (e != cudaSuccess) return e;
     kern<<<grid, kSqWarps * 32, smem, st>>>(P);
     return cudaGetLastError();
 }
 
-template <bool SQUEEZE, int LAG>
+template <bool SQUEEZE, bool STORE, int LAG>
 static cudaError_t launch_sq_c2(const SqueezeParams& P, int c2, unsigned grid, size_t smem, cudaStream_t st)
 {
     switch (c2) {
-        case 2: return launch_sq_t<SQUEEZE, true, 2, LAG, false>(P, grid, smem, st);
-        case 3: return launch_sq_t<SQUEEZE, true, 3, LAG, false>(P, grid, smem, st);
-        case 4: return launch_sq_t<SQUEEZE, true, 4, LAG, false>(P, grid, smem, st);
-        case 5: return launch_sq_t<SQUEEZE, true, 5, LAG, false>(P, grid, smem, st);
-        case 6: return launch_sq_t<SQUEEZE, true, 6, LAG, false>(P, grid, smem, st);
-        case 7: return launch_sq_t<SQUEEZE, true, 7, LAG, false>(P, grid, smem, st);
-        case 8: return launch_sq_t<SQUEEZE, true, 8, LAG, false>(P, grid, smem, st);
-        case 9: return launch_sq_t<SQUEEZE, true, 9, LAG, false>(P, grid, smem, st);
-        case 10: return launch_sq_t<SQUEEZE, true, 10, LAG, false>(P, grid, smem, st);
-        case 11: return launch_sq_t<SQUEEZE, true, 11, LAG, false>(P, grid, smem, st);
-        case 12: return launch_sq_t<SQUEEZE, true, 12, LAG, false>(P, grid, smem, st);
-        case 13: return launch_sq_t<SQUEEZE, true, 13, LAG, false>(P, grid, smem, st);
+        case 2: return launch_sq_t<SQUEEZE, STORE, true, 2, LAG, false>(P, grid, smem, st);
+        case 3: return launch_sq_t<SQUEEZE, STORE, true, 3, LAG, false>(P, grid, smem, st);
+        case 4: return launch_sq_t<SQUEEZE, STORE, true, 4, LAG, false>(P, grid, smem, st);
+        case 5: return launch_sq_t<SQUEEZE, STORE, true, 5, LAG, false>(P, grid, smem, st);
+        case 6: return launch_sq_t<SQUEEZE, STORE, true, 6, LAG, false>(P, grid, smem, st);
+        case 7: return launch_sq_t<SQUEEZE, STORE, true, 7, LAG, false>(P, grid, smem, st);
+        case 8: return launch_sq_t<SQUEEZE, STORE, true, 8, LAG, false>(P, grid, smem, st);
+        case 9: return launch_sq_t<SQUEEZE, STORE, true, 9, LAG, false>(P, grid, smem, st);
+        case 10: return launch_sq_t<SQUEEZE, STORE, true, 10, LAG, false>(P, grid, smem, st);
+        case 11: return launch_sq_t<SQUEEZE, STORE, true, 11, LAG, false>(P, grid, smem, st);
+        case 12: return launch_sq_t<SQUEEZE, STORE, true, 12, LAG, false>(P, grid, smem, st);
+        case 13: return launch_sq_t<SQUEEZE, STORE, true, 13, LAG, false>(P, grid, smem, st);
         default: return cudaErrorInvalidValue;
     }
 }
 
-template <bool SQUEEZE>
+template <bool SQUEEZE, bool STORE>
 static cudaError_t launch_sq_partial(const SqueezeParams& P, int c2, unsigned grid, size_t smem, cudaStream_t st)
 {
-    if (c2 == 1) return launch_sq_t<SQUEEZE, true, 1, 1, true>(P, grid, smem, st);
-    if (c2 == 2) return launch_sq_t<SQUEEZE, true, 2, 2, true>(P, grid, smem, st);
+    if (c2 == 1) return launch_sq_t<SQUEEZE, STORE, true, 1, 1, true>(P, grid, smem, st);
+    if (c2 == 2) return launch_sq_t<SQUEEZE, STORE, true, 2, 2, true>(P, grid, smem, st);
     return cudaErrorInvalidValue;
 }
 
-int squeeze_pieces_per_task(int n_ind, int n_pieces)
+int squeeze_pieces_per_task(int n_ind, int n_pieces, int warps_per_sm)
 {
     const int n_rg = (n_ind + 31) / 32;
-    const int want_tasks = 148 * 16 * 3;
+    const int want_tasks = 148 * warps_per_sm * 3;
     int n_col = std::max(1, (want_tasks + n_rg - 1) / n_rg);
     int ppt = (n_pieces + n_col - 1) / n_col;
     ppt = std::max(ppt, 16);
@@ -376,24 +388,27 @@
     return ppt;
 }
 
-cudaError_t launch_squeeze_bound(SqueezeParams P, bool squeeze, int c2, cudaStream_t st)
+cudaError_t launch_squeeze_bound(SqueezeParams P, bool squeeze, bool store, int c2, cudaStream_t st)
 {
     if (!P.n_ind || !P.n_pieces) return cudaSuccess;
-    P.pieces_per_task = squeeze_pieces_per_task(P.n_ind, P.n_pieces);
+    if (!squeeze) store = false;
+    if (c2 <= 0 && !(squeeze && store)) return cudaErrorInvalidValue;
+    if (squeeze && !store && P.partial) return cudaErrorInvalidValue;
+    const int ctas_per_sm = store ? kSqCtasPerSm : kSqCtasPerSmNoTile;
+    P.pieces_per_task = squeeze_pieces_per_task(P.n_ind, P.n_pieces, ctas_per_sm * kSqWarps);
     P.n_col_tasks = (P.n_pieces + P.pieces_per_task - 1) / P.pieces_per_task;
     const int n_rg = (P.n_ind + 31) / 32;
     const long long n_tasks = (long long)n_rg * P.n_col_tasks;
     long long grid = (n_tasks + kSqWarps - 1) / kSqWarps;
-    if (grid > 148ll * 4 * 8) grid = 148ll * 4 * 8;
-    const size_t smem = (size_t)kSqWarps * kSqWarpBytes;
-    if (c2 <= 0) {
-        if (!squeeze) return cudaErrorInvalidValue;
-        return launch_sq_t<true, false, 2, 1, false>(P, (unsigned)grid, smem, st);
-    }
-    if (P.partial) return squeeze ? launch_sq_partial<true>(P, c2, (unsigned)grid, smem, st) : launch_sq_partial<false>(P, c2, (unsigned)grid, smem, st);
-    if (P.lag == 1) return squeeze ? launch_sq_c2<true, 1>(P, c2, (unsigned)grid, smem, st) : launch_sq_c2<false, 1>(P, c2, (unsigned)grid, smem, st);
-    if (P.lag == 2) return squeeze ? launch_sq_c2<true, 2>(P, c2, (unsigned)grid, smem, st) : launch_sq_c2<false, 2>(P, c2, (unsigned)grid, smem, st);
-    return cudaErrorInvalidValue;
+    if (grid > 148ll * ctas_per_sm * 8) grid = 148ll * ctas_per_sm * 8;
+    const unsigned g = (unsigned)grid;
+    const size_t smem = (size_t)kSqWarps * (store ? kSqWarpBytes : kSqWarpBytesNoTile);
+    if (c2 <= 0) return launch_sq_t<true, true, false, 2, 1, false>(P, g, smem, st);
+    if (P.partial) return squeeze ? launch_sq_partial<true, true>(P, c2, g, smem, st) : launch_sq_partial<false, false>(P, c2, g, smem, st);
+    if (P.lag != 1 && P.lag != 2) return cudaErrorInvalidValue;
+    if (!squeeze) return P.lag == 1 ? launch_sq_c2<false, false, 1>(P, c2, g, smem, st) : launch_sq_c2<false, false, 2>(P, c2, g, smem, st);
+    if (!store) return P.lag == 1 ? launch_sq_c2<true, false, 1>(P, c2, g, smem, st) : launch_sq_c2<true, false, 2>(P, c2, g, smem, st);
+    return P.lag == 1 ? launch_sq_c2<true, true, 1>(P, c2, g, smem, st) : launch_sq_c2<true, true, 2>(P, c2, g, smem, st);
 }
 
 __global__ void __launch_bounds__(256)
diff --git a/garlic_b200/csrc/walk.cuh b/garlic_b200/csrc/walk.cuh
--- a/garlic_b200/csrc/walk.cuh
+++ b/garlic_b200/csrc/walk.cuh
@@ -24,6 +24,7 @@
 template <int SRC>
 struct LaneCtx {
     const uint64_t* row;
+    int row_base;
     const char* tile;
     int tile_lo;
     const double* freq;
@@ -218,12 +219,13 @@
 
 template <int SRC, bool ROH, bool DUMP>
 GHD void walk_item(const WalkParams& P, const Item& it, int k_slot, bool active, uint32_t* ring, int rstride,
-                   const char* tile, int tile_lo, int ind_in = -1)
+                   const char* tile, int tile_lo, int ind_in = -1, const uint64_t* row = nullptr, int row_base = 0)
 {
     const int W = P.W;
     const int ind = ind_in >= 0 ? ind_in : (P.ind_list ? P.ind_list[k_slot] : k_slot);
     LaneCtx<SRC> C;
-    C.row = P.geno + (int64_t)ind * P.row_words;
+    C.row = row ? row : P.geno + (int64_t)ind * P.row_words;
+    C.row_base = row ? row_base : 0;
     C.tile = tile;
     C.tile_lo = tile_lo;
     C.freq = P.freq;
@@ -234,7 +236,7 @@
     double win = 0.0;
     for (int i = 0; i < W; ++i) {
         const int s = it.w0 + i;
-        const int g = (int)(C.row[s >> 5] >> (2 * (s & 31))) & 3;
+        const int g = (int)(C.row[(s >> 5) - C.row_base] >> (2 * (s & 31))) & 3;
         win += C.aval(s, g);
     }
     LaneState S;
@@ -252,8 +254,8 @@
 
     const int M = it.own_hi - 1 - it.w0;
     const int sa = 2 * ((it.w0 + W) & 31), sb = 2 * (it.w0 & 31);
-    const uint64_t* pa = C.row + ((it.w0 + W) >> 5);
-    const uint64_t* pb = C.row + (it.w0 >> 5);
+    const uint64_t* pa = C.row + (((it.w0 + W) >> 5) - C.row_base);
+    const uint64_t* pb = C.row + ((it.w0 >> 5) - C.row_base);
     uint64_t a_lo = pa[0], b_lo = pb[0];
     uint64_t a_hi = pa[1], b_hi = pb[1];
     pa += 2; pb += 2;
```

Result: faster. 1374 billion (median of 6 runs) (+11.0%).
